# iqbal-lab-org/gramtools

Hardware: AMD Instinct MI355X
Metric: 150bp reads quasimapped/sec (whole node); bit-exact coverage (higher is better)
Workload: dtype u32

## Files before the change

gramtools_amd/csrc/gmx_capi.cpp:

```cpp
#include <atomic>
#include <algorithm>
#include <array>
#include <cmath>
#include <cstdlib>
#include <cstring>
#include <map>
#include <new>
#include <stdexcept>
#include <system_error>
#include <string>
#include <thread>
#include <vector>

#include "gmx_core.h"
#include "gmx_internal.h"

static std::atomic<uint64_t> g_index_serial{1};
struct gmx_index {
  gmx::HostIndex h;
  const uint64_t serial = g_index_serial.fetch_add(1);
};

static thread_local std::string g_error;
void gmx_set_error(const std::string &msg) noexcept {
// ... 250 lines not shown
    ++n;
  }
  return (int64_t)n;
} GMX_GUARD_INT("gmx_index_per_base_layout")

int gmx_index_allele_base_layout(const gmx_index *ix, uint32_t *pb_off, uint32_t *len) try {
  const auto &h = ix->h;
  if (h.is_nested) {
    gmx_set_error("allele_base_non_nested is empty by convention for nested PRGs");
    return GMX_EINVAL;
  }
  for (size_t s = 0; s < h.sites.size(); ++s) {
    const GmxSite &site = h.sites[s];
    const GmxNode &entry = h.nodes[site.entry_node];
    for (uint32_t a = 0; a < site.n_alleles; ++a) {
      uint32_t tgt = h.edges[entry.edge_begin + a];
      uint32_t slot = h.l_allele_off[s] + a;
      if (tgt == site.exit_node) {
        pb_off[slot] = 0;
        len[slot] = 0;
      } else {
        pb_off[slot] = h.l_cov_off[tgt];
        len[slot] = h.nodes[tgt].seq_len;
      }
    }
  }
  return GMX_OK;
} GMX_GUARD_INT("gmx_index_allele_base_layout")

static std::vector<uint32_t> bubble_order(const gmx::HostIndex &h) {
  std::vector<uint32_t> order(h.sites.size());
  for (uint32_t i = 0; i < order.size(); ++i) order[i] = i;
  std::sort(order.begin(), order.end(), [&](uint32_t a, uint32_t b) {
    if (h.site_ref_pos[a] != h.site_ref_pos[b]) return h.site_ref_pos[a] > h.site_ref_pos[b];
    return a > b;
  });
  return order;
}

int gmx_index_bubble_order(const gmx_index *ix, uint32_t *out) try {
  auto o = bubble_order(ix->h);
  for (size_t i = 0; i < o.size(); ++i) out[i] = 5 + 2 * o[i];
  return GMX_OK;
} GMX_GUARD_INT("gmx_index_bubble_order")

int gmx_compute_coverage_depth(const gmx_index *ix, const uint32_t *per_base_raw, const uint32_t *grouped_raw,
                               const uint32_t *glog, uint64_t n_log, gmx_depth_stats *out) try {
  const gmx::HostIndex &h = ix->h;
  std::vector<std::map<int32_t, uint16_t>> hap(h.sites.size());
  std::vector<std::map<std::vector<int32_t>, uint16_t>> logged(h.sites.size());
  for (uint64_t i = 0; i < n_log;) {
    if (glog[i] == 0xFFFFFFFFu) {
      ++i;
      continue;
    }
    if (i + 2 > n_log) break;
    const uint32_t s = glog[i], n = glog[i + 1] & ~GMX_LOG_COUNTED;
    const uint64_t head = (glog[i + 1] & GMX_LOG_COUNTED) ? 4 : 2;
    if (s >= h.sites.size() || i + head + n > n_log) {
      gmx_set_error("corrupt grouped log");
      return GMX_EINVAL;
    }
    const uint64_t count = head == 4 ? ((uint64_t)glog[i + 2] | ((uint64_t)glog[i + 3] << 32)) : 1;
    std::vector<int32_t> ids(glog + i + head, glog + i + head + n);
    logged[s][ids] = (uint16_t)(logged[s][ids] + count);
    i += head + n;
  }
  for (size_t s = 0; s < h.sites.size(); ++s) {
    const GmxSite &site = h.sites[s];
    if (h.l_grouped_off[s] != GMX_GROUPED_LOG) {
      uint32_t nm = (1u << site.n_alleles) - 1u;
      for (uint32_t m = 0; m < nm; ++m) {
        uint32_t tot = grouped_raw[h.l_grouped_off[s] + m];
        if (!tot) continue;
        uint16_t c = (uint16_t)(tot & 0xFFFFu);
        for (uint32_t a = 0; a < site.n_alleles; ++a)
          if (((m + 1) >> a) & 1u) hap[s][(int32_t)a] = (uint16_t)(hap[s][(int32_t)a] + c);
      }
    }
    for (auto &e : logged[s])
      for (auto a : e.first) hap[s][a] = (uint16_t)(hap[s][a] + e.second);
  }
  auto max_hap = [&](size_t s) -> std::pair<int32_t, uint16_t> {
    std::pair<int32_t, uint16_t> best{0, 0};
    bool any = false;
    for (auto &e : hap[s])
      if (!any || e.second > best.second) {
        best = {e.first, e.second};
        any = true;
      }
    return best;
  };
  std::vector<double> coverages;
  double total = 0;
  uint64_t no_cov = 0;
  for (uint32_t s : bubble_order(h)) {
    const GmxSite &site = h.sites[s];
    if (site.parent_site != 0) continue;
    auto mx = max_hap(s);
    uint16_t allele_cov = mx.second;
    double sum = 0;
    uint64_t n_bases = 0;
    uint32_t cur = site.entry_node;
    size_t guard = 0;
    while (cur != site.exit_node) {
      if (++guard > h.nodes.size() + 8) {
        gmx_set_error("coverage graph walk does not terminate");
        return GMX_EINVAL;
      }
      const GmxNode &nd = h.nodes[cur];
      uint32_t ne = h.nodes[cur + 1].edge_begin - nd.edge_begin;
      if (ne > 1 && nd.seq_len == 0) {
        auto m2 = max_hap((nd.site - 5) / 2);
        if (m2.first < 0 || (uint32_t)m2.first >= ne) {
          gmx_set_error("haplogroup out of range");
          return GMX_EINVAL;
        }
        cur = h.edges[nd.edge_begin + (uint32_t)m2.first];
        continue;
      }
      if (nd.seq_len > 0 && nd.cov_off != GMX_NO_COV)
        for (uint32_t i = 0; i < nd.seq_len; ++i) {
          uint32_t v = per_base_raw[h.l_cov_off[cur] + i];
          sum += (double)(v > 65535u ? 65535u : v);
          ++n_bases;
        }
      cur = h.edges[nd.edge_begin];
    }
    double site_cov = n_bases ? sum / (double)n_bases : (double)allele_cov;
    total += site_cov;
    coverages.push_back(site_cov);
    if (allele_cov == 0) no_cov++;
  }
  double mean = total / (double)coverages.size();
  double tv = 0;
  for (double c : coverages) tv += std::pow(c - mean, 2);
  out->mean_cov_depth = mean;
  out->variance_cov_depth = tv / (double)coverages.size();
  out->num_sites_noCov = no_cov;
  out->num_sites_total = coverages.size();
  return GMX_OK;
} GMX_GUARD_INT("gmx_compute_coverage_depth")

int gmx_debug_suffix_array_u16(const uint16_t *text, uint64_t n, uint16_t *out) try {
  try {
    gmx::debug_suffix_array_u16(text, (size_t)n, out);
    return GMX_OK;
  } catch (std::exception const &ex) {
    gmx_set_error(ex.what());
    return GMX_EINVAL;
  }
} GMX_GUARD_INT("gmx_debug_suffix_array_u16")

int gmx_index_copy_sa(const gmx_index *ix, uint32_t *out) try {
  memcpy(out, ix->h.sa.data(), ix->h.sa.size() * 4);
  return GMX_OK;
} GMX_GUARD_INT("gmx_index_copy_sa")
int gmx_index_copy_bwt(const gmx_index *ix, uint32_t *out) try {
  if (ix->h.bwt.empty()) {
    gmx_set_error("this index was built without its introspection tables (GMX_INDEX_INTROSPECTION=1 keeps them)");
    return GMX_EINVAL;
  }
  memcpy(out, ix->h.bwt.data(), ix->h.bwt.size() * 4);
  return GMX_OK;
} GMX_GUARD_INT("gmx_index_copy_bwt")
uint32_t gmx_index_rank(const gmx_index *ix, uint32_t upper, uint32_t base) try {
  if (base < 1 || base > 4) return 0;
  GmxIndexView v = ix->h.view();
  return gmx_rank(v, upper, base);
} GMX_GUARD_ZERO("gmx_index_rank")
int gmx_index_copy_pos_info(const gmx_index *ix, int64_t *out) try {
  const auto &h = ix->h;
  if (h.pos_target.size() != h.prg.size()) {
    gmx_set_error("this index was built without its introspection tables (GMX_INDEX_INTROSPECTION=1 keeps them)");
    return GMX_EINVAL;
  }
  for (size_t p = 0; p < h.prg.size(); ++p) {
    const GmxNode &nd = h.nodes[h.pos_node[p]];
    out[5 * p + 0] = nd.site;
    out[5 * p + 1] = nd.allele;
    out[5 * p + 2] = h.prg[p] <= 4 ? (int64_t)p - nd.first_pos : 0;
    out[5 * p + 3] = h.pos_target[p].first;
    out[5 * p + 4] = h.pos_target[p].second;
  }
  return GMX_OK;
} GMX_GUARD_INT("gmx_index_copy_pos_info")
int64_t gmx_index_copy_target_map(const gmx_index *ix, int64_t *out, uint64_t cap) try {
  std::vector<int64_t> v{(int64_t)ix->h.target_map.size()};
  for (auto &e : ix->h.target_map) {
    v.push_back(e.first);
    v.push_back((int64_t)e.second.size());
    for (auto &t : e.second) {
      v.push_back(t.id);
      v.push_back(t.deletion_allele);
    }
  }
  if (v.size() > cap) return -(int64_t)v.size();
  std::copy(v.begin(), v.end(), out);
  return (int64_t)v.size();
} GMX_GUARD_INT("gmx_index_copy_target_map")
int64_t gmx_index_seed_states(const gmx_index *ix, const uint8_t *kmer, int64_t *out, uint64_t cap) try {
  return gmx_index_seed_states_k(ix, kmer, ix->h.kmer_size, out, cap);
} GMX_GUARD_INT("gmx_index_seed_states")
int64_t gmx_index_seed_states_k(const gmx_index *ix, const uint8_t *kmer, uint32_t len, int64_t *out, uint64_t cap) try {
  const auto &h = ix->h;
  if (len == 0 || (len != h.kmer_size && len != h.kmer_size2)) return GMX_EINVAL;
  uint32_t code = 0;
  for (uint32_t j = 0; j < len; ++j) {
    if (kmer[j] < 1 || kmer[j] > 4) return GMX_EINVAL;
    code |= (uint32_t)(kmer[j] - 1) << (2 * j);
  }
  auto v = gmx::seed_states_of(h, code, len != h.kmer_size);
  if (v.size() > cap) return -(int64_t)v.size();
  std::copy(v.begin(), v.end(), out);
  return (int64_t)v.size();
} GMX_GUARD_INT("gmx_index_seed_states_k")
int64_t gmx_index_jump_states(const gmx_index *ix, uint32_t lo, uint32_t hi, int64_t *out, uint64_t cap) try {
  const auto &h = ix->h;
  GmxIndexView v = h.view();
  ProbeCtx ctx;
  const GmxRankBlock b = v.blocks[lo >> GMX_BLK_SHIFT];
  gmx_marker_pass(v, lo, hi, GMX_NIL, GMX_NIL, b, ctx);
  std::vector<int64_t> r{(int64_t)ctx.n};
  for (uint32_t s = 0; s < ctx.n; ++s) {
    r.push_back(ctx.st[s].lo);
    r.push_back(ctx.st[s].hi);
    std::vector<std::pair<uint32_t, int32_t>> tmp;
    for (uint32_t x = ctx.st[s].tvd; x != GMX_NIL; x = ctx.arena[x].next) tmp.push_back({ctx.arena[x].site, ctx.arena[x].allele});
    r.push_back((int64_t)tmp.size());
    for (size_t i = tmp.size(); i-- > 0;) {
      r.push_back(tmp[i].first);
      r.push_back(tmp[i].second);
    }
    tmp.clear();
    for (uint32_t x = ctx.st[s].tvg; x != GMX_NIL; x = ctx.arena[x].next) tmp.push_back({ctx.arena[x].site, -1});
    r.push_back((int64_t)tmp.size());
    for (size_t i = tmp.size(); i-- > 0;) {
      r.push_back(tmp[i].first);
      r.push_back(-1);
    }
  }
  if (r.size() > cap) return -(int64_t)r.size();
  std::copy(r.begin(), r.end(), out);
  return (int64_t)r.size();
} GMX_GUARD_INT("gmx_index_jump_states")

int gmx_master_seeds(uint32_t master_seed, const uint64_t *reads_per_file, uint64_t n_files, uint32_t *out) try {
  uint32_t mt[624];
  mt[0] = master_seed;
  for (int i = 1; i < 624; ++i) mt[i] = 1812433253u * (mt[i - 1] ^ (mt[i - 1] >> 30)) + (uint32_t)i;
  int idx = 624;
  auto next = [&]() {
    if (idx >= 624) {
      for (int i = 0; i < 624; ++i) {
        uint32_t y = (mt[i] & 0x80000000u) | (mt[(i + 1) % 624] & 0x7fffffffu);
        mt[i] = mt[(i + 397) % 624] ^ (y >> 1) ^ ((y & 1u) ? 0x9908b0dfu : 0u);
      }
      idx = 0;
    }
    uint32_t y = mt[idx++];
    y ^= (y >> 11);
    y ^= (y << 7) & 0x9d2c5680u;
    y ^= (y << 15) & 0xefc60000u;
    y ^= (y >> 18);
    return y;
  };
  uint64_t o = 0;
  for (uint64_t f = 0; f < n_files; ++f)
    for (uint64_t start = 0; start < reads_per_file[f]; start += 5000)
      for (uint64_t i = 0; i < 5000; ++i) {
        uint32_t s = next();
        if (start + i < reads_per_file[f]) out[o++] = s;
      }
  return GMX_OK;
} GMX_GUARD_INT("gmx_master_seeds")

uint64_t gmx_packed_pairs(const uint64_t *offsets, uint32_t uniform_len, uint64_t n_reads) try {
  if (uniform_len) return n_reads * (uint64_t)((uniform_len + 31u) / 32u);
  if (!offsets) return 0;
  return ((offsets[n_reads] >> 5) - (offsets[0] >> 5)) + n_reads;
} GMX_GUARD_ZERO("gmx_packed_pairs")

namespace {
inline void pack8(uint64_t x, uint32_t &lo, uint32_t &hi, uint64_t &bad) {
  const uint64_t y = x - 0x0101010101010101ull;
  bad |= (y & ~x & 0x8080808080808080ull) | (y & 0xFCFCFCFCFCFCFCFCull);
  lo = (uint32_t)(((y & 0x0101010101010101ull) * 0x0102040810204080ull) >> 56);
  hi = (uint32_t)((((y >> 1) & 0x0101010101010101ull) * 0x0102040810204080ull) >> 56);
}
inline bool pack_read(const uint8_t *p, uint32_t len, uint64_t *out) {
  uint64_t bad = 0;
  uint32_t i = 0, pair = 0;
  for (; i + 32 <= len; i += 32, ++pair) {
    uint32_t lo = 0, hi = 0;
    for (int j = 0; j < 4; ++j) {
      uint64_t x;
      memcpy(&x, p + i + 8 * j, 8);
      uint32_t l, h;
      pack8(x, l, h, bad);
      lo |= l << (8 * j);
      hi |= h << (8 * j);
    }
    out[pair] = (uint64_t)lo | ((uint64_t)hi << 32);
  }
  if (i < len) {
    uint32_t lo = 0, hi = 0;
// ... 161 lines not shown
```

gramtools_amd/csrc/gmx_engine_cover_kernels.h:

```cpp
#pragma once
struct CoverAcc {
  uint32_t *acc;
  uint32_t *log;
  uint32_t *log_cursor;
  uint32_t log_cap;
  uint32_t *scratch_big;
  uint32_t n_lanes_big;
  int rng_mode;
  uint32_t max_candidates;
  uint32_t log_sites;
  uint32_t *heap;
  uint64_t heap_words;
  const uint32_t *status;
  uint32_t n_tasks;
  unsigned long long *stats;
  uint32_t rev_off;
  __device__ __forceinline__ uint32_t off_of(uint32_t task) const { return (task & 1u) ? rev_off : 0u; }
};

#define GMX_LOG_PAD 0xFFFFFFFFu
#ifdef GMX_LOOP_STATS
__device__ unsigned long long gmx_cover_stats[6 * 16];
__device__ unsigned long long gmx_coop_stats[6 * 8];
extern "C" int gmx_debug_coop_stats(unsigned long long *out, int reset) {
// ... 825 lines not shown
  if (!done) o.single_rest_list[atomicAdd(&o.counters[GMX_CNT_SINGLE_REST * GMX_CNT_STRIDE], 1u)] = (uint32_t)rec_idx;
}
__global__ void __launch_bounds__(GMX_BLOCK) gmx_cover_single_rest_kernel(GmxIndexView ix, BatchView b, SearchOut o, CoverAcc acc) {
  const uint32_t n = o.counters[GMX_CNT_SINGLE_REST * GMX_CNT_STRIDE];
  for (uint32_t i = blockIdx.x * GMX_BLOCK + threadIdx.x; i < n; i += gridDim.x * GMX_BLOCK)
    gmx_cover_single_rec<false>(ix, o, acc, o.single_rest_list[i], o.cover_general_list, 8u);
}

__global__ void gmx_log_replay_setup_kernel(SearchOut o, const uint32_t *retry_huge_in) {
  uint32_t *c = o.counters;
  const uint32_t n_entries = c[GMX_CNT_LOG_RETRY * GMX_CNT_STRIDE], n_recs = c[GMX_CNT_LOG_RETRY_RECS * GMX_CNT_STRIDE],
                 n_huge = c[GMX_CNT_LOG_RETRY_HUGE * GMX_CNT_STRIDE];
  for (uint32_t i = threadIdx.x; i < n_huge; i += blockDim.x) o.huge_list[i] = retry_huge_in[i];
  __syncthreads();
  if (threadIdx.x == 0) {
    c[4 * GMX_CNT_STRIDE] = n_entries;
    c[GMX_CNT_REPLAY_RECS * GMX_CNT_STRIDE] = n_recs;
    c[11 * GMX_CNT_STRIDE] = n_huge;
    c[15 * GMX_CNT_STRIDE] = 0;
    c[14 * GMX_CNT_STRIDE] = 0;
    c[GMX_CNT_LOG_RETRY * GMX_CNT_STRIDE] = 0;
    c[GMX_CNT_LOG_RETRY_RECS * GMX_CNT_STRIDE] = 0;
    c[GMX_CNT_LOG_RETRY_HUGE * GMX_CNT_STRIDE] = 0;
  }
}
template <bool NESTED>
__global__ void __launch_bounds__(GMX_BLOCK) gmx_cover_single_replay_kernel(GmxIndexView ix, BatchView b, SearchOut o, CoverAcc acc,
                                                                            const uint32_t *recs_in) {
  const uint32_t n = o.counters[GMX_CNT_REPLAY_RECS * GMX_CNT_STRIDE];
  for (uint32_t i = blockIdx.x * GMX_BLOCK + threadIdx.x; i < n; i += gridDim.x * GMX_BLOCK)
    gmx_cover_single_rec<NESTED>(ix, o, acc, recs_in[i], o.cover_overflow_list, 4u);
}

__global__ void gmx_stats_limbs_kernel(unsigned long long *stats, uint32_t *limbs, int recombine) {
  const uint32_t t = threadIdx.x;
  if (!recombine) {
    if (t < 20) limbs[t] = (uint32_t)((stats[t >> 2] >> (16 * (t & 3))) & 0xFFFFull);
    else if (t < 32) limbs[t] = 0;
  } else if (t < 5) {
    unsigned long long v = 0;
    for (int l = 3; l >= 0; --l) v = (v << 16) + limbs[4 * t + l];
    stats[t] = v;
  }
}

#define GMX_PACK_READS 128
#define GMX_PACK_IN_BYTES (24 * 1024)
#define GMX_PACK_OUT_PAIRS (GMX_PACK_IN_BYTES / 32 + GMX_PACK_READS + 8)
typedef uint32_t __attribute__((aligned(1))) gmx_u32_unaligned;
__device__ __forceinline__ void pack4(uint32_t x, uint32_t &lo, uint32_t &hi, uint32_t &bad) {
  uint32_t y = x - 0x01010101u;
  bad |= ((y & ~x & 0x80808080u) | (y & 0xFCFCFCFCu));
  lo = (((y & 0x01010101u) * 0x01020408u) >> 24) & 0xFu;
  hi = ((((y >> 1) & 0x01010101u) * 0x01020408u) >> 24) & 0xFu;
}
__device__ __forceinline__ uint2 pack_tail(const uint8_t *p, uint32_t rem, uint32_t &bad) {
  uint2 out = make_uint2(0, 0);
  for (uint32_t j = 0; j < rem; ++j) {
    uint32_t x = p[j];
    if (x < 1 || x > 4) bad = 1;
    out.x |= ((x - 1u) & 1u) << j;
    out.y |= (((x - 1u) >> 1) & 1u) << j;
  }
  return out;
}
#define GMX_PACK_THREADS (2 * GMX_PACK_READS)
__global__ void __launch_bounds__(GMX_PACK_THREADS) gmx_pack_kernel(BatchView b, uint8_t *skip, uint2 *packed, uint32_t *counters,
                                                                    uint32_t *zero, uint32_t zero_words) {
  __shared__ uint4 in4[GMX_PACK_IN_BYTES / 16 + 2];
  __shared__ uint2 outp[GMX_PACK_OUT_PAIRS];
  if (blockIdx.x == 0)
    for (uint32_t i = threadIdx.x; i < GMX_N_COUNTERS * GMX_CNT_STRIDE; i += GMX_PACK_THREADS) counters[i] = 0;
  for (uint32_t i = blockIdx.x * GMX_PACK_THREADS + threadIdx.x; i < zero_words; i += gridDim.x * GMX_PACK_THREADS) zero[i] = 0;
  const uint32_t r0 = blockIdx.x * GMX_PACK_READS;
  const uint32_t r1 = min(r0 + GMX_PACK_READS, b.n_reads);
  const uint32_t read = r0 + (threadIdx.x >> 1), half = threadIdx.x & 1u;
  const uint64_t s0 = b.offsets[r0], s1 = b.offsets[r1];
  const uintptr_t g0 = reinterpret_cast<uintptr_t>(b.reads + s0);
  const uint32_t shift = (uint32_t)(g0 & 15u);
  const uint64_t span = (s1 - s0) + shift;
  if (span <= GMX_PACK_IN_BYTES) {
    const uint4 *src = reinterpret_cast<const uint4 *>(g0 - shift);
    const uint32_t n16 = (uint32_t)((span + 15) >> 4);
    {
      uint32_t i = threadIdx.x;
      for (; i + 2 * GMX_PACK_THREADS < n16; i += 3 * GMX_PACK_THREADS) {
        const uint4 v0 = src[i], v1 = src[i + GMX_PACK_THREADS], v2 = src[i + 2 * GMX_PACK_THREADS];
        in4[i] = v0;
        in4[i + GMX_PACK_THREADS] = v1;
        in4[i + 2 * GMX_PACK_THREADS] = v2;
      }
      for (; i < n16; i += GMX_PACK_THREADS) in4[i] = src[i];
    }
    const uint64_t po0 = pack_off(b, r0);
    const uint32_t n_out = (uint32_t)(pack_off(b, r1) - po0);
    for (uint32_t i = threadIdx.x; i < n_out; i += GMX_PACK_THREADS) outp[i] = make_uint2(0, 0);
    __syncthreads();
    if (read < r1) {
      const uint64_t s = b.offsets[read];
      const uint32_t len = (uint32_t)(b.offsets[read + 1] - s);
      const uint32_t q = shift + (uint32_t)(s - s0);
      const uint32_t *w = reinterpret_cast<const uint32_t *>(in4);
      const uint8_t *bytes = reinterpret_cast<const uint8_t *>(in4);
      uint2 *out = outp + (uint32_t)(pack_off(b, read) - po0);
      const uint32_t full = len >> 5, first_half = (full + 1u) >> 1;
      const uint32_t c0 = half ? first_half : 0u, c1 = half ? full : first_half;
      uint32_t idx = (q >> 2) + 8u * c0;
      const uint32_t sh = q & 3u;
      uint32_t bad = 0;
      uint32_t carry = w[idx];
      for (uint32_t c = c0; c < c1; ++c) {
        uint2 pair = make_uint2(0, 0);
#pragma unroll
        for (int j = 0; j < 8; ++j) {
          uint32_t nxt = w[++idx], lo, hi;
          pack4(__builtin_amdgcn_alignbyte(nxt, carry, sh), lo, hi, bad);
          pair.x |= lo << (4 * j);
          pair.y |= hi << (4 * j);
          carry = nxt;
        }
        out[c] = pair;
      }
      const uint32_t rem = len & 31u;
      if (half && rem) out[full] = pack_tail(bytes + q + full * 32, rem, bad);
      bad |= (uint32_t)__shfl_xor((int)bad, 1);
      if (!half) skip[read] = bad ? 1 : 0;
    }
    __syncthreads();
    for (uint32_t i = threadIdx.x; i < n_out; i += GMX_PACK_THREADS) packed[po0 + i] = outp[i];
    return;
  }
  if (read >= r1 || half) return;
  uint64_t s = b.offsets[read], e = b.offsets[read + 1];
  uint32_t len = (uint32_t)(e - s);
  const uint8_t *p = b.reads + s;
  uint2 *out = packed + pack_off(b, read);
  uint32_t bad = 0;
  uint32_t full = len >> 5;
  for (uint32_t c = 0; c < full; ++c) {
    uint2 pair = make_uint2(0, 0);
#pragma unroll
    for (int j = 0; j < 8; ++j) {
      uint32_t lo, hi;
      pack4(*reinterpret_cast<const gmx_u32_unaligned *>(p + c * 32 + j * 4), lo, hi, bad);
      pair.x |= lo << (4 * j);
      pair.y |= hi << (4 * j);
    }
    out[c] = pair;
  }
  uint32_t rem = len & 31u;
  if (rem) out[full] = pack_tail(p + full * 32, rem, bad);
  skip[read] = bad ? 1 : 0;
}
```

gramtools_amd/csrc/gmx_engine_debug.h:

```cpp

struct GmxDebugPools {
  GmxFinalState *states = nullptr;
  uint32_t *stack = nullptr;
  GmxPathNode *arena = nullptr;
  uint32_t *result = nullptr;
  uint32_t *in = nullptr;
  uint2 *planes = nullptr;
  uint32_t cap_states = 0, cap_nodes = 0, cap_in = 0, cap_pairs = 0;
};

__global__ void __launch_bounds__(64) gmx_debug_search_kernel(GmxIndexView ix, BatchView b, const uint32_t *in, uint32_t from, uint32_t stop,
                                                              uint32_t mode, uint32_t from_seed_table, BigOut g, uint32_t *result) {
  const bool active = threadIdx.x == 0;
  BigCtx ctx;
  ctx.sp = 0;
  ctx.cap = g.max_states;
  ctx.stack = g.stack;
  ctx.arena = g.arena;
  ctx.arena_n = 0;
  ctx.arena_cap = g.max_path_nodes;
  ctx.status = GMX_TASK_MAPPED;
  ctx.out = g.states;
  ctx.n_out = 0;
  ctx.out_cap = g.max_states;
// ... 17 lines not shown
        const uint32_t lo = p[0], hi = p[1], nt = p[2], ng = p[3];
        p += 4;
        uint32_t tvd = GMX_NIL, tvg = GMX_NIL;
        bool ok = true;
        for (uint32_t j = 0; j < nt; ++j, p += 2)
          if (ok) ok = (tvd = ctx.arena_new(p[0], (int32_t)p[1], tvd)) != GMX_NIL;
        for (uint32_t j = 0; j < ng; ++j, ++p)
          if (ok) ok = (tvg = ctx.arena_new(p[0], -1, tvg)) != GMX_NIL;
        if (!ok || !ctx.push(lo, hi, tvd, tvg, from, mode)) ctx.fail(GMX_TASK_OVERFLOW);
      }
    }
    run = ctx.status == GMX_TASK_MAPPED;
  }
  GmxLane ln;
  dfs_run_wave<2, false>(ix, ctx, r, stop, run, 0, ln);
  if (active) {
    result[0] = ctx.status;
    result[1] = ctx.n_out;
    result[2] = ctx.arena_n;
  }
}

__global__ void gmx_debug_items_kernel(GmxIndexView ix, const GmxFinalState *finals, uint32_t n_final, uint32_t *out, uint32_t cap_items) {
  if (blockIdx.x != 0 || threadIdx.x != 0) return;
  uint32_t n_items = 0, n_nonvar = 0;
  uint32_t *items = out + 2, *nonvar = out + 2 + 6 * (size_t)cap_items;
  const bool ok = gmx_final_items(
      ix, finals, n_final,
      [&](uint32_t lo, uint32_t hi, uint32_t tvd, uint32_t tvg, uint32_t es, int32_t ea) -> bool {
        if (n_items >= cap_items) return false;
        uint32_t *it = items + 6 * (size_t)n_items++;
        it[0] = lo, it[1] = hi, it[2] = tvd, it[3] = tvg, it[4] = es, it[5] = (uint32_t)ea;
        return true;
      },
      [&](uint32_t i, uint32_t) {
        if (n_nonvar < cap_items) nonvar[n_nonvar] = i;
        ++n_nonvar;
      });
  out[0] = ok ? n_items : 0xFFFFFFFFu;
  out[1] = n_nonvar;
}

namespace {

struct DebugWriter {
  uint32_t *out;
  uint64_t cap, n = 0;
  void put(uint32_t w) {
    if (out && n < cap) out[n] = w;
    ++n;
  }
};

int debug_isa(gmx_engine *e) {
  if (!e->debug_isa.empty()) return GMX_OK;
  std::vector<uint32_t> sa(e->dview.n);
  HIP_TRY(hipMemcpy(sa.data(), e->dview.sa, sa.size() * sizeof(uint32_t), hipMemcpyDeviceToHost));
  e->debug_isa.assign(sa.size(), 0u);
  for (size_t i = 0; i < sa.size(); ++i)
    if (sa[i] < sa.size()) e->debug_isa[sa[i]] = (uint32_t)i;
  return GMX_OK;
}

template <class NodeAt>
int debug_put_state(gmx_engine *e, DebugWriter &w, const GmxFinalState &st, NodeAt node) {
  uint32_t lo = st.lo, hi = st.hi;
  if (hi == GMX_TEXT_MARK) {
    if (lo >= e->debug_isa.size()) {
      gmx_set_error("debug states: text-form state outside the PRG");
      return GMX_EREF;
    }
    lo = hi = e->debug_isa[lo];
  }
  std::vector<std::pair<uint32_t, int32_t>> tvd;
  std::vector<uint32_t> tvg;
  for (uint32_t h = st.traversed; h != GMX_NIL;) {
    GmxPathNode nd;
    int rc = node(h, nd);
    if (rc) return rc;
    tvd.emplace_back(nd.site, nd.allele);
    h = nd.next;
    if (tvd.size() > (1u << 20)) {
      gmx_set_error("debug states: path list does not end");
      return GMX_EREF;
    }
  }
  for (uint32_t h = st.traversing; h != GMX_NIL;) {
    if (gmx_h_inline(h)) {
      tvg.push_back(5u + 2u * (h & ~GMX_INLINE_FLAG));
      break;
    }
    GmxPathNode nd;
    int rc = node(h, nd);
    if (rc) return rc;
    tvg.push_back(nd.site);
    h = nd.next;
    if (tvg.size() > (1u << 20)) {
      gmx_set_error("debug states: path list does not end");
      return GMX_EREF;
    }
  }
  w.put(lo);
  w.put(hi);
  w.put((uint32_t)tvd.size());
  w.put((uint32_t)tvg.size());
  for (size_t i = tvd.size(); i-- > 0;) {
    w.put(tvd[i].first);
    w.put((uint32_t)tvd[i].second);
  }
  for (size_t i = tvg.size(); i-- > 0;) w.put(tvg[i]);
  return GMX_OK;
}

int debug_pools(gmx_engine *e, GmxDebugPools &p, uint32_t n_in_words, uint32_t n_pairs) {
  const uint32_t S = std::max<uint32_t>(e->big.max_states, 64u), N = std::max<uint32_t>(e->big.max_path_nodes, 64u);
  int rc;
  if ((rc = e->alloc(&p.states, S, false))) return rc;
  if ((rc = e->alloc(&p.stack, (size_t)S * GMX_STACK_WORDS, false))) return rc;
  if ((rc = e->alloc(&p.arena, N, false))) return rc;
  if ((rc = e->alloc(&p.result, 4, true))) return rc;
  if ((rc = e->alloc(&p.in, std::max<uint32_t>(n_in_words, 1u), false))) return rc;
  if ((rc = e->alloc(&p.planes, n_pairs + 16, true))) return rc;
  p.cap_states = S;
  p.cap_nodes = N;
  return GMX_OK;
}
void debug_pools_free(gmx_engine *e, GmxDebugPools &p) {
  e->release(p.states);
  e->release(p.stack);
  e->release(p.arena);
  e->release(p.result);
  e->release(p.in);
  e->release(p.planes);
}

}

extern "C" {

int gmx_engine_debug_keep_states(gmx_engine *e, int on) try {
  if (!e) {
    gmx_set_error("null engine");
    return GMX_EINVAL;
  }
  e->keep_states = on != 0;
  return GMX_OK;
} GMX_GUARD_INT("gmx_engine_debug_keep_states")

int gmx_debug_final_states(gmx_engine *e, uint64_t task, uint32_t *out, uint64_t cap_words, uint64_t *n_words, int *tier) try {
  if (!e || !n_words) {
    gmx_set_error("gmx_debug_final_states: null argument");
    return GMX_EINVAL;
  }
  if (!e->keep_states || task >= 2 * e->keep_reads) {
    gmx_set_error("gmx_debug_final_states: no such task in the last batch (gmx_engine_debug_keep_states first)");
    return GMX_EINVAL;
  }
  HIP_TRY(hipSetDevice(e->opts.device));
  HIP_TRY(hipDeviceSynchronize());
  int rc = debug_isa(e);
  if (rc) return rc;
  uint32_t raw[GMX_N_COUNTERS * GMX_CNT_STRIDE];
  HIP_TRY(hipMemcpy(raw, e->d_counters, sizeof(raw), hipMemcpyDeviceToHost));
  auto c = [&](int i) { return raw[i * GMX_CNT_STRIDE]; };
  DebugWriter w{out, cap_words};
  {
    const uint32_t n_huge = c(11);
    std::vector<uint32_t> huge(n_huge);
    if (n_huge) HIP_TRY(hipMemcpy(huge.data(), e->d_huge, n_huge * sizeof(uint32_t), hipMemcpyDeviceToHost));
    for (uint32_t t : huge)
      if (t == task) {
        gmx_set_error("gmx_debug_final_states: the task was searched by the last tier, which keeps no states");
        return GMX_ECAP;
      }
  }
  const uint32_t used = (uint32_t)std::min<uint64_t>((uint64_t)c(1) + c(9) + c(29), e->big.max_slots);
  if (used) {
    std::vector<uint32_t> owner(used), nf(used), over(std::min<uint32_t>(c(1), used));
    HIP_TRY(hipMemcpy(owner.data(), e->big.task_of_slot, used * sizeof(uint32_t), hipMemcpyDeviceToHost));
    HIP_TRY(hipMemcpy(nf.data(), e->big.n_final, used * sizeof(uint32_t), hipMemcpyDeviceToHost));
    if (!over.empty()) HIP_TRY(hipMemcpy(over.data(), e->d_overflow, over.size() * sizeof(uint32_t), hipMemcpyDeviceToHost));
    bool in_slots = false;
    for (uint32_t s = used; s-- > 0;) {
      const bool first_q = s < over.size();
      if (first_q && (over[s] & ~GMX_INST_FLAG) != task) continue;
      if (!first_q && owner[s] != task) continue;
      in_slots = true;
      if (first_q && owner[s] != task) continue;
      if (nf[s] == 0) continue;
      const bool inst = first_q && (over[s] & GMX_INST_FLAG) != 0;
      const uint32_t n = nf[s];
      std::vector<GmxFinalState> st(n);
      if (inst) {
        uint32_t first = 0, width = 0;
        HIP_TRY(hipMemcpy(&first, e->d_inst_first + s, 4, hipMemcpyDeviceToHost));
        HIP_TRY(hipMemcpy(&width, e->d_inst_width + s, 4, hipMemcpyDeviceToHost));
        if (n > width * GMX_INST_STATES) continue;
        HIP_TRY(hipMemcpy(st.data(), e->d_inst_states + (size_t)first * GMX_INST_STATES, n * sizeof(GmxFinalState), hipMemcpyDeviceToHost));
        const GmxPathNode *arena = e->d_inst_arena + (size_t)first * GMX_FAST_ARENA;
        w.put(n);
        for (uint32_t i = 0; i < n; ++i) {
          rc = debug_put_state(e, w, st[i], [&](uint32_t h, GmxPathNode &nd) {
            HIP_TRY(hipMemcpy(&nd, arena + h, sizeof(nd), hipMemcpyDeviceToHost));
            return GMX_OK;
          });
          if (rc) return rc;
        }
        if (tier) *tier = 2;
      } else {
        if (n > e->big.max_states) continue;
        HIP_TRY(hipMemcpy(st.data(), e->big.states + (size_t)s * e->big.max_states, n * sizeof(GmxFinalState), hipMemcpyDeviceToHost));
        const GmxPathNode *arena = e->big.arena + (size_t)s * e->big.max_path_nodes;
        w.put(n);
        for (uint32_t i = 0; i < n; ++i) {
          rc = debug_put_state(e, w, st[i], [&](uint32_t h, GmxPathNode &nd) {
            HIP_TRY(hipMemcpy(&nd, arena + h, sizeof(nd), hipMemcpyDeviceToHost));
            return GMX_OK;
          });
          if (rc) return rc;
        }
        if (tier) *tier = 1;
      }
      *n_words = w.n;
      return w.n > cap_words && out ? GMX_ECAP : GMX_OK;
    }
    if (in_slots) {
      w.put(0);
      if (tier) *tier = 1;
      *n_words = w.n;
      return GMX_OK;
    }
  }
  uint32_t packed = 0;
  HIP_TRY(hipMemcpy(&packed, e->d_n_final + task, 4, hipMemcpyDeviceToHost));
  const uint32_t n = std::min<uint32_t>(packed & 0xFFu, GMX_FAST_STATES);
  std::vector<GmxFinalState> st(n);
  if (n) HIP_TRY(hipMemcpy(st.data(), e->d_finals + (size_t)task * GMX_FAST_STATES, n * sizeof(GmxFinalState), hipMemcpyDeviceToHost));
  const GmxPathNode *arena = e->d_arena + task;
  w.put(n);
  for (uint32_t i = 0; i < n; ++i) {
    rc = debug_put_state(e, w, st[i], [&](uint32_t h, GmxPathNode &nd) {
      HIP_TRY(hipMemcpy(&nd, arena + h, sizeof(nd), hipMemcpyDeviceToHost));
      return GMX_OK;
    });
    if (rc) return rc;
  }
  if (tier) *tier = 0;
  *n_words = w.n;
  return w.n > cap_words && out ? GMX_ECAP : GMX_OK;
} GMX_GUARD_INT("gmx_debug_final_states")

int gmx_debug_search(gmx_engine *e, const uint8_t *read, uint32_t read_len, int from_seed_table, const uint32_t *states, uint64_t n_state_words,
                     uint32_t from, uint32_t stop, int lf_only, uint32_t *out, uint64_t cap_words, uint64_t *n_words) try {
  if (!e || !read || !n_words || read_len == 0 || (!from_seed_table && (!states || n_state_words == 0 || from > read_len || stop > from))) {
    gmx_set_error("gmx_debug_search: bad argument");
    return GMX_EINVAL;
  }
  for (uint32_t i = 0; i < read_len; ++i)
    if (read[i] < 1 || read[i] > 4) {
      gmx_set_error("gmx_debug_search: the read must hold bases 1..4");
      return GMX_EINVAL;
    }
  if (from_seed_table && read_len < e->dview.kmer_size) {
    gmx_set_error("gmx_debug_search: read shorter than the k-mer size");
    return GMX_EINVAL;
  }
  HIP_TRY(hipSetDevice(e->opts.device));
  HIP_TRY(hipDeviceSynchronize());
  int rc = debug_isa(e);
  if (rc) return rc;
  const uint32_t n_pairs = (read_len + 31u) / 32u;
  GmxDebugPools p;
  if ((rc = debug_pools(e, p, (uint32_t)n_state_words, n_pairs))) return rc;
  std::vector<uint2> planes(n_pairs + 16, make_uint2(0, 0));
  for (uint32_t i = 0; i < read_len; ++i) {
    const uint32_t code = read[i] - 1u;
    planes[i >> 5].x |= (code & 1u) << (i & 31u);
    planes[i >> 5].y |= (code >> 1) << (i & 31u);
  }
  HIP_TRY(hipMemcpy(p.planes, planes.data(), planes.size() * sizeof(uint2), hipMemcpyHostToDevice));
  if (!from_seed_table) HIP_TRY(hipMemcpy(p.in, states, n_state_words * sizeof(uint32_t), hipMemcpyHostToDevice));
  BatchView b{};
  b.packed = p.planes;
  b.n_reads = 1;
  b.forward_only = 1;
  b.uniform_len = read_len;
  b.pairs_per_read = n_pairs;
  BigOut g{};
  g.states = p.states;
  g.stack = p.stack;
  g.arena = p.arena;
  g.max_states = p.cap_states;
  g.max_path_nodes = p.cap_nodes;
  g.max_slots = 1;
  const size_t big_lds = (size_t)GMX_BIG_LDS_DEPTH * GMX_STACK_WORDS * 64 * sizeof(uint32_t);
  hipLaunchKernelGGL(gmx_debug_search_kernel, dim3(1), dim3(64), big_lds, 0, e->dview, b, p.in, from, stop,
                     lf_only ? GMX_MODE_LF : GMX_MODE_STATE, from_seed_table ? 1u : 0u, g, p.result);
  HIP_TRY(hipGetLastError());
  HIP_TRY(hipDeviceSynchronize());
  uint32_t res[3] = {0, 0, 0};
  HIP_TRY(hipMemcpy(res, p.result, sizeof(res), hipMemcpyDeviceToHost));
  if (res[0] != GMX_TASK_MAPPED) {
    debug_pools_free(e, p);
    gmx_set_error(res[0] == GMX_TASK_OVERFLOW ? "gmx_debug_search: the states exceed the engine's large-capacity pools (gmx_engine_opts.max_states / max_path_nodes)"
                                              : "gmx_debug_search: the search reports a condition on which the reference throws");
    return res[0] == GMX_TASK_OVERFLOW ? GMX_ECAP : GMX_EREF;
  }
  const uint32_t n = res[1];
  std::vector<GmxFinalState> st(n);
  std::vector<GmxPathNode> arena(res[2]);
  if (n) HIP_TRY(hipMemcpy(st.data(), p.states, n * sizeof(GmxFinalState), hipMemcpyDeviceToHost));
  if (res[2]) HIP_TRY(hipMemcpy(arena.data(), p.arena, res[2] * sizeof(GmxPathNode), hipMemcpyDeviceToHost));
  debug_pools_free(e, p);
  DebugWriter w{out, cap_words};
  w.put(n);
  for (uint32_t i = 0; i < n; ++i) {
    rc = debug_put_state(e, w, st[i], [&](uint32_t h, GmxPathNode &nd) {
      if (h >= arena.size()) {
        gmx_set_error("gmx_debug_search: path handle outside the arena");
        return GMX_EREF;
      }
      nd = arena[h];
      return GMX_OK;
    });
    if (rc) return rc;
  }
  *n_words = w.n;
  return w.n > cap_words && out ? GMX_ECAP : GMX_OK;
} GMX_GUARD_INT("gmx_debug_search")

int gmx_debug_encapsulate(gmx_engine *e, const uint32_t *states, uint64_t n_state_words, uint32_t *out, uint64_t cap_words, uint64_t *n_words,
                          uint32_t *nonvariant_sa, uint64_t cap_nonvariant, uint64_t *n_nonvariant) try {
  if (!e || !states || n_state_words == 0 || !n_words || !n_nonvariant) {
    gmx_set_error("gmx_debug_encapsulate: bad argument");
    return GMX_EINVAL;
  }
  HIP_TRY(hipSetDevice(e->opts.device));
  HIP_TRY(hipDeviceSynchronize());
  std::vector<GmxFinalState> st;
  std::vector<GmxPathNode> arena;
  const uint32_t *p = states, *end = states + n_state_words;
  const uint32_t ns = *p++;
  uint64_t positions = 0;
  for (uint32_t s = 0; s < ns; ++s) {
    if (p + 4 > end || p + 4 + 2 * (uint64_t)p[2] + p[3] > end) {
      gmx_set_error("gmx_debug_encapsulate: malformed state words");
      return GMX_EINVAL;
    }
    const uint32_t lo = p[0], hi = p[1], nt = p[2], ng = p[3];
    p += 4;
    if (lo > hi || hi >= e->dview.n) {
      gmx_set_error("gmx_debug_encapsulate: interval outside the suffix array");
      return GMX_EINVAL;
    }
    uint32_t tvd = GMX_NIL, tvg = GMX_NIL;
    for (uint32_t j = 0; j < nt; ++j, p += 2) {
      arena.push_back(GmxPathNode{p[0], (int32_t)p[1], tvd});
      tvd = (uint32_t)arena.size() - 1;
    }
    for (uint32_t j = 0; j < ng; ++j, ++p) {
      arena.push_back(GmxPathNode{p[0], -1, tvg});
      tvg = (uint32_t)arena.size() - 1;
    }
    st.push_back(GmxFinalState{lo, hi, tvd, tvg});
    positions += (uint64_t)hi - lo + 1;
  }
  if (positions > (1u << 24)) {
    gmx_set_error("gmx_debug_encapsulate: more than 2^24 positions");
    return GMX_EINVAL;
  }
  const uint32_t cap_items = (uint32_t)std::max<uint64_t>(positions + ns, 1);
  GmxFinalState *d_st = nullptr;
  uint32_t *d_out = nullptr;
  int rc;
  if ((rc = e->alloc(&d_st, st.size(), false))) return rc;
  if ((rc = e->alloc(&d_out, 2 + 7 * (size_t)cap_items, true))) return rc;
  if (!st.empty()) HIP_TRY(hipMemcpy(d_st, st.data(), st.size() * sizeof(GmxFinalState), hipMemcpyHostToDevice));
  hipLaunchKernelGGL(gmx_debug_items_kernel, dim3(1), dim3(64), 0, 0, e->dview, d_st, (uint32_t)st.size(), d_out, cap_items);
  HIP_TRY(hipGetLastError());
  HIP_TRY(hipDeviceSynchronize());
  std::vector<uint32_t> res(2 + 7 * (size_t)cap_items);
  HIP_TRY(hipMemcpy(res.data(), d_out, res.size() * sizeof(uint32_t), hipMemcpyDeviceToHost));
  e->release(d_st);
  e->release(d_out);
  if (res[0] == 0xFFFFFFFFu || res[1] > cap_items) {
    gmx_set_error("gmx_debug_encapsulate: item buffer exceeded");
    return GMX_EREF;
  }
  DebugWriter w{out, cap_words};
  w.put(res[0]);
  for (uint32_t i = 0; i < res[0]; ++i) {
    const uint32_t *it = res.data() + 2 + 6 * (size_t)i;
    GmxFinalState f{it[0], it[1], it[2], it[3]};
    if (it[4] != 0) {
      w.put(f.lo);
      w.put(f.lo);
      w.put(1);
      w.put(0);
      w.put(it[4]);
      w.put(it[5]);
      continue;
    }
    rc = debug_put_state(e, w, f, [&](uint32_t h, GmxPathNode &nd) {
      if (h >= arena.size()) {
        gmx_set_error("gmx_debug_encapsulate: path handle outside the arena");
        return GMX_EREF;
      }
      nd = arena[h];
      return GMX_OK;
    });
    if (rc) return rc;
  }
  *n_words = w.n;
  *n_nonvariant = res[1];
  for (uint32_t i = 0; i < res[1] && nonvariant_sa && i < cap_nonvariant; ++i) nonvariant_sa[i] = res[2 + 6 * (size_t)cap_items + i];
  return (w.n > cap_words && out) || (nonvariant_sa && res[1] > cap_nonvariant) ? GMX_ECAP : GMX_OK;
} GMX_GUARD_INT("gmx_debug_encapsulate")

}
```

gramtools_amd/csrc/gmx_engine_host.h:

```cpp
#pragma once
#define HIP_TRY(expr)                                                                      \
  do {                                                                                     \
    hipError_t _e = (expr);                                                                \
    if (_e != hipSuccess) {                                                                \
      gmx_set_error(std::string(#expr) + ": " + hipGetErrorString(_e));                    \
      return GMX_EHIP;                                                                     \
    }                                                                                      \
  } while (0)

enum : int { GMX_TK_SEED = 0, GMX_TK_FILTER0, GMX_TK_FILTER1, GMX_TK_SINGLE, GMX_TK_EXTEND2, GMX_TK_UNPACK, GMX_TK_N };
static_assert(GMX_TK_N <= GMX_TIMED_KERNELS, "gmx_timing::kernel_ms holds GMX_TIMED_KERNELS entries");

struct GmxReadLog {
  const uint32_t stride;
  bool on = false;
  uint32_t *d = nullptr;
  uint64_t cap = 0, count = 0;

  uint64_t used() const { return (count * stride + 3) & ~3ull; }

  int reserve(uint64_t n_more) {
    const uint64_t need = (count + n_more) * stride;
    if (need <= cap) return GMX_OK;
    const uint64_t grown = (std::max<uint64_t>(need + need / 2, 1u << 20) + 3) & ~3ull;
    uint32_t *q = nullptr;
    HIP_TRY(hipDeviceSynchronize());
    HIP_TRY(hipMalloc((void **)&q, grown));
    hipError_t err = hipMemset(q, 0, grown);
    if (err == hipSuccess && count) err = hipMemcpy(q, d, used(), hipMemcpyDeviceToDevice);
    if (err != hipSuccess) {
      (void)hipFree(q);
      HIP_TRY(err);
    }
    release();
    d = q;
    cap = grown;
    return GMX_OK;
  }
  int clear(const hipStream_t *stream) {
    if (count) HIP_TRY(stream ? hipMemsetAsync(d, 0, used(), *stream) : hipMemset(d, 0, used()));
    count = 0;
    return GMX_OK;
  }
  uint64_t claim(uint64_t n) {
    const uint64_t base = count;
    count += n;
    return base;
  }
  void release() {
    if (d) (void)hipFree(d);
    d = nullptr;
    cap = 0;
  }
};

struct gmx_engine {
  gmx_engine_opts opts;
  GmxIndexView dview;
  std::vector<void *> allocs;
  uint64_t index_bytes = 0;
  uint32_t *d_fused = nullptr, *d_limbs = nullptr;
  size_t n_fused = 0, n_acc = 0;
  bool record_strands = false;
  uint32_t max_candidates = 0;
  bool recorded = false;
  std::vector<uint32_t> phys_allele, phys_pb, phys_grouped;
  std::vector<uint32_t> hit_fix;
  unsigned long long *d_stats = nullptr;
  uint32_t *d_error = nullptr;
  uint32_t *d_log = nullptr, *d_log_cursor = nullptr;
  uint32_t log_cap = 0;
  uint32_t n_allele = 0, n_pb = 0, n_grouped = 0;
  uint64_t cap_reads = 0;
  uint8_t *d_skip = nullptr;
  uint2 *d_packed = nullptr;
  uint64_t cap_packed = 0;
  uint32_t *d_status = nullptr, *d_n_final = nullptr, *d_mapped = nullptr, *d_overflow = nullptr, *d_counters = nullptr;
  uint32_t *d_general_rest = nullptr;
  uint32_t *d_single_rest = nullptr;
  bool cover_jump = false;
  uint32_t *d_task_lists = nullptr;
  GmxSeed *d_alive_seed = nullptr;
  uint32_t *d_alive = nullptr, *d_dead = nullptr, *d_dead2 = nullptr;
  uint64_t *d_seed_cursor = nullptr;
  bool seed_cursor = false;
  GmxFinalState *d_finals = nullptr;
  GmxPathNode *d_arena = nullptr;
  GmxCoverRec *d_cover_recs = nullptr;
  BigOut big{};
  uint32_t *d_scratch_big = nullptr, *d_cover_overflow = nullptr;
  uint32_t cover_big_lanes = 0;
  uint32_t *d_big_mapped = nullptr, *d_cover_general = nullptr, *d_cover_mid = nullptr, *d_overflow2 = nullptr;
  uint32_t *d_huge = nullptr, *d_cover_huge = nullptr, *d_huge_retry = nullptr;
  uint32_t *d_inst_list = nullptr, *d_inst_sa = nullptr, *d_inst_remaining = nullptr, *d_inst_mapped = nullptr;
  uint32_t inst_cap = 0;
  GmxPathNode *d_inst_arena = nullptr;
  GmxFinalState *d_inst_states = nullptr;
  uint32_t *d_inst_first = nullptr, *d_inst_width = nullptr;
  uint32_t *d_inst_serial = nullptr, *d_general_serial = nullptr, *d_big_serial = nullptr, *d_overflow3 = nullptr;
  bool coop = true;
  uint32_t *d_heap = nullptr;
  uint64_t heap_words = 0;
  bool log_sites = false;
  std::map<std::vector<uint32_t>, std::array<uint64_t, 2>> log_counts;
  uint32_t *h_log_state = nullptr;
  hipEvent_t ev_log_state = nullptr;
  bool log_state_pending = false;
  uint32_t *d_log_retry[2] = {nullptr, nullptr}, *d_log_retry_recs[2] = {nullptr, nullptr}, *d_log_retry_huge[2] = {nullptr, nullptr};
  int log_retry_side = 0;
  BatchView last_b{};
  SearchOut last_o{};
  CoverAcc last_acc{};
  size_t last_big_lds = 0;
  uint64_t log_replays = 0, log_replayed_entries = 0;
  uint64_t log_known = 0;
  uint64_t log_reads_since = 0;
  bool reset_pending = false;
  hipStream_t reset_stream = nullptr;
  hipStream_t side2_stream = nullptr;
  hipEvent_t ev_fork2 = nullptr, ev_side1 = nullptr, ev_filter = nullptr;
  hipStream_t side_stream = nullptr;
  hipEvent_t ev_fork = nullptr, ev_join = nullptr;
  hipEvent_t ev_wait = nullptr;
  struct GmxDeviceIndex *shared_index = nullptr;
  uint32_t filter_lds_words = 0;
  const uint32_t *d_kmer_planar = nullptr;
  const uint32_t *d_absent = nullptr;
  uint32_t n_absent = 0;
  bool use_absent = false;
  uint32_t n_cus = 256;
  uint32_t probe_iters = GMX_PROBE_ITERS;
  uint32_t extend_cap = 0;
  uint32_t extend_budget = 8;
  bool seeds_in_place = false;
  gmx_engine *twin = nullptr;
  gmx_engine *owner = nullptr;
  bool is_twin = false, twin_off = false;
  GmxReadLog outcomes{1}, positions{16};
  uint64_t reset_epoch = 0;
  hipStream_t main_stream = nullptr;
  uint32_t twin_toggle = 0;
  hipEvent_t ev_zeroed = nullptr, ev_twin_done = nullptr;
  uint64_t zero_epoch = 0, seen_zero_epoch = 0;
  bool twin_in_flight = false;
  bool last_on_twin = false;
  uint32_t extend_passes = 1;
  uint32_t extend_budget2[GMX_EXTRA_PASSES] = {24, 96, 0};
  GmxParked *d_park2 = nullptr;
  uint32_t *d_park2_n = nullptr;
  bool keep_states = false;
  uint64_t keep_reads = 0;
  std::vector<uint32_t> debug_isa;
  uint32_t fuse = 1;
  uint8_t *d_reads = nullptr;
  uint64_t *d_offsets = nullptr;
  uint32_t *d_seeds = nullptr;
  uint64_t cap_bases = 0, cap_stage_reads = 0;
  struct StageSlot {
    uint8_t *d_reads = nullptr;
    uint64_t *d_offsets = nullptr, *h_offsets = nullptr;
    uint32_t *d_seeds = nullptr, *h_seeds = nullptr;
    uint64_t cap_bases = 0, cap_reads = 0;
    hipEvent_t copied = nullptr, done = nullptr;
    bool busy = false;
  } stage[2];
  hipStream_t copy_stream = nullptr;
  hipStream_t copy_stream2 = nullptr;
  uint32_t copy_toggle = 0;
  hipStream_t last_stream = nullptr;
  struct PackSlot {
    uint2 *d_planes = nullptr;
    uint64_t *d_offsets = nullptr;
    uint32_t *d_seeds = nullptr;
    uint8_t *d_skip = nullptr;
    uint64_t cap_pairs = 0, cap_reads = 0;
    hipEvent_t copied = nullptr, done = nullptr;
    bool busy = false;
  } pslot[3];
  uint32_t pslot_next = 0;
  void release(void *q) {
    if (!q) return;
    for (size_t i = 0; i < allocs.size(); ++i)
      if (allocs[i] == q) {
        allocs[i] = allocs.back();
        allocs.pop_back();
        (void)hipFree(q);
        return;
      }
  }
  bool timing = false;
  struct EvTriple { hipEvent_t s, a, b, c; uint64_t reads; hipEvent_t k[GMX_TIMED_KERNELS][2]; uint32_t timed; };
  std::vector<EvTriple> pending;
  double search_ms = 0, cover_ms = 0;
  uint64_t search_launches = 0, cover_launches = 0, timed_reads = 0;
  double kernel_ms[GMX_TIMED_KERNELS] = {0};
  uint64_t kernel_launches[GMX_TIMED_KERNELS] = {0};

  template <class T>
  int alloc(T **p, size_t count, bool zero) {
    void *q = nullptr;
    size_t bytes = std::max<size_t>(count, 1) * sizeof(T);
    allocs.reserve(allocs.size() + 1);
    HIP_TRY(hipMalloc(&q, bytes));
    if (zero) HIP_TRY(hipMemset(q, 0, bytes));
    allocs.push_back(q);
    *p = (T *)q;
    return GMX_OK;
  }
  template <class T, class A>
  int upload(const T **dst, const std::vector<T, A> &src) {
    T *q = nullptr;
    int rc = alloc(&q, src.size(), false);
    if (rc) return rc;
    if (!src.empty()) HIP_TRY(hipMemcpy(q, src.data(), src.size() * sizeof(T), hipMemcpyHostToDevice));
    index_bytes += src.size() * sizeof(T);
    *dst = q;
    return GMX_OK;
  }
  int upload(const uint32_t **dst, const gmx::WordBuf &src) {
    uint32_t *q = nullptr;
    int rc = alloc(&q, src.size(), false);
    if (rc) return rc;
    const size_t piece = (size_t)1 << 28;
    for (size_t at = 0; at < src.size(); at += piece)
      HIP_TRY(hipMemcpy(q + at, src.data() + at, std::min(piece, src.size() - at) * sizeof(uint32_t), hipMemcpyHostToDevice));
    index_bytes += src.size() * sizeof(uint32_t);
    *dst = q;
    return GMX_OK;
  }
};

static hipError_t gmx_event_wait(hipEvent_t ev) {
  static const bool spin = getenv("GMX_WAIT_SPIN") != nullptr;
  if (spin) return hipEventSynchronize(ev);
  const auto t0 = std::chrono::steady_clock::now();
  for (bool napping = false;;) {
    const hipError_t q = hipEventQuery(ev);
    if (q != hipErrorNotReady) return q;
    (void)hipGetLastError();
    if (!napping) {
      napping = std::chrono::steady_clock::now() - t0 > std::chrono::microseconds(60);
      continue;
    }
    struct timespec ts = {0, 50 * 1000};
    nanosleep(&ts, nullptr);
  }
}

static int gmx_quiesce(gmx_engine *e) {
  if (!e->ev_wait) HIP_TRY(hipEventCreateWithFlags(&e->ev_wait, hipEventDisableTiming | hipEventBlockingSync));
  hipStream_t streams[5] = {e->last_stream, e->copy_stream, e->side_stream, e->side2_stream, e->copy_stream2};
  for (int i = 0; i < 5; ++i) {
    if (i > 0 && !streams[i]) continue;
    bool seen = false;
    for (int j = 0; j < i; ++j) seen = seen || streams[j] == streams[i];
    if (seen) continue;
    HIP_TRY(hipEventRecord(e->ev_wait, streams[i]));
    HIP_TRY(gmx_event_wait(e->ev_wait));
  }
  return GMX_OK;
}

static int note_zeroed(gmx_engine *e, hipStream_t stream) {
  if (!e->twin) return GMX_OK;
  if (!e->ev_zeroed) HIP_TRY(hipEventCreateWithFlags(&e->ev_zeroed, hipEventDisableTiming));
  HIP_TRY(hipEventRecord(e->ev_zeroed, stream));
  ++e->zero_epoch;
  return GMX_OK;
}
static int twin_join(gmx_engine *e, hipStream_t stream) {
  gmx_engine *tw = e->twin;
  if (!tw || !e->twin_in_flight) return GMX_OK;
  if (!e->ev_twin_done) HIP_TRY(hipEventCreateWithFlags(&e->ev_twin_done, hipEventDisableTiming));
  HIP_TRY(hipEventRecord(e->ev_twin_done, tw->main_stream));
  HIP_TRY(hipStreamWaitEvent(stream, e->ev_twin_done, 0));
  return GMX_OK;
}
static int flush_reset(gmx_engine *e) {
  if (!e->reset_pending) return GMX_OK;
  e->reset_pending = false;
  HIP_TRY(hipMemsetAsync(e->d_fused, 0, (e->n_fused + 32) * 4, e->reset_stream));
  return note_zeroed(e, e->reset_stream);
}

static int log_settle(gmx_engine *e);
static int gmx_log_drain(gmx_engine *e, uint64_t keep_below) {
  int frc = flush_reset(e);
  if (frc) return frc;
  HIP_TRY(hipDeviceSynchronize());
  uint32_t used = 0;
  HIP_TRY(hipMemcpy(&used, e->d_log_cursor, 4, hipMemcpyDeviceToHost));
  used = std::min(used, e->log_cap);
  e->log_reads_since = 0;
  e->log_known = used;
  if (used <= keep_below) return GMX_OK;
  std::vector<uint32_t> w(used);
  HIP_TRY(hipMemcpy(w.data(), e->d_log, (size_t)used * 4, hipMemcpyDeviceToHost));
  std::vector<uint32_t> key;
  for (size_t i = 0; i < w.size();) {
    if (w[i] == GMX_LOG_PAD) {
      ++i;
      continue;
    }
    const size_t n_ids = i + 2 > w.size() ? 0 : (size_t)(w[i + 1] & ~GMX_LOG_REVERSE);
    if (i + 2 > w.size() || i + 2 + n_ids > w.size()) {
      gmx_set_error("grouped-allele-count log: malformed record at word " + std::to_string(i) + " of " + std::to_string(w.size()));
      return GMX_EREF;
    }
    if ((w[i + 1] & GMX_LOG_REVERSE) && !(e->owner ? e->owner : e)->record_strands) {
      gmx_set_error("grouped-allele-count log: a reverse-complement record at word " + std::to_string(i) + " of an engine that does not record per strand");
      return GMX_EREF;
    }
    key.assign(1, w[i]);
    key.insert(key.end(), w.begin() + i + 2, w.begin() + i + 2 + n_ids);
    e->log_counts[key][(w[i + 1] & GMX_LOG_REVERSE) ? 1 : 0] += 1;
    i += 2 + n_ids;
  }
  HIP_TRY(hipMemset(e->d_log_cursor, 0, 4));
  e->log_known = 0;
  return GMX_OK;
}

template <class Env, int LIST>
static void launch_cover_lds(gmx_engine *e, hipStream_t stream, const BatchView &b, const SearchOut &o, const CoverAcc &acc,
                             bool after_coop = false) {
  static const uint32_t lanes_env = getenv("GMX_COVER_LANES") ? (uint32_t)atoi(getenv("GMX_COVER_LANES")) : 0u;
  const uint32_t lanes = lanes_env ? std::min(lanes_env, gmx_cover_lds_lanes<Env>()) : gmx_cover_lds_lanes<Env>();
  const size_t lds = (size_t)GmxScratchFixed<Env>::total * lanes * sizeof(uint32_t);
  const uint32_t per_cu = std::min<uint32_t>((uint32_t)(160 * 1024 / lds), 32u);
  hipLaunchKernelGGL((gmx_cover_kernel<Env, LIST>), dim3(e->n_cus * per_cu), dim3(64), lds, stream, e->dview, b, o, e->big,
                     acc, lanes, after_coop ? 1u : 0u);
}

template <int LIST>
static void launch_cover_coop(gmx_engine *e, hipStream_t stream, const BatchView &b, const SearchOut &o, const CoverAcc &acc) {
  const size_t lds = (size_t)gmx_coop_lds_words<LIST>() * sizeof(uint32_t);
  const uint32_t per_cu = std::min<uint32_t>((uint32_t)(160 * 1024 / lds), 16u);
  hipLaunchKernelGGL((gmx_cover_coop_kernel<LIST>), dim3(e->n_cus * per_cu), dim3(64), lds, stream, e->dview, b, o, e->big, acc);
}

extern "C" {

void gmx_engine_default_opts(gmx_engine_opts *o) try {
  o->device = 0;
  o->rng_mode = GMX_RNG_LEMIRE;
  o->max_states = 1024;
  o->max_path_nodes = 2048;
  o->max_batch_reads = 4u << 20;
  o->forward_only = 0;
  o->huge_heap_bytes = 512ull << 20;
  o->log_cap_words = 0;
} GMX_GUARD_VOID("gmx_engine_default_opts")

static int ensure_batch_capacity(gmx_engine *e, uint64_t n_reads, bool launching = false) {
  if (launching) {
    gmx_engine *own = e->owner ? e->owner : e;
    for (GmxReadLog *log : {&own->outcomes, &own->positions})
      if (log->on) {
        const int lrc = log->reserve(n_reads);
        if (lrc) return lrc;
      }
  }
  if (n_reads <= e->cap_reads) return GMX_OK;
  uint64_t cap = std::max<uint64_t>(e->cap_reads ? n_reads + n_reads / 8 : n_reads, 1024);
  uint64_t n_tasks = cap * 2;
  int rc;
  if ((rc = e->alloc(&e->d_skip, cap, true))) return rc;
  if ((rc = e->alloc(&e->d_status, n_tasks, false))) return rc;
  if ((rc = e->alloc(&e->d_n_final, n_tasks, false))) return rc;
  if ((rc = e->alloc(&e->d_cover_recs, n_tasks * GMX_REGIONS, false))) return rc;
  if ((rc = e->alloc(&e->d_mapped, n_tasks * GMX_REGIONS, false))) return rc;
  if ((rc = e->alloc(&e->d_task_lists, (size_t)GMX_TL_N * n_tasks, false))) return rc;
  e->d_overflow = e->d_task_lists + (size_t)GMX_TL_OVERFLOW * n_tasks;
  e->d_overflow2 = e->d_task_lists + (size_t)GMX_TL_OVERFLOW2 * n_tasks;
  e->d_alive = e->d_task_lists + (size_t)GMX_TL_ALIVE * n_tasks;
  e->d_dead = e->d_task_lists + (size_t)GMX_TL_DEAD * n_tasks;
  e->d_dead2 = e->d_task_lists + (size_t)GMX_TL_DEAD2 * n_tasks;
  e->d_cover_general = e->d_task_lists + (size_t)GMX_TL_GENERAL * n_tasks;
  if ((rc = e->alloc(&e->d_cover_overflow, n_tasks, false))) return rc;
  if ((rc = e->alloc(&e->d_general_rest, n_tasks, false))) return rc;
  if ((rc = e->alloc(&e->d_single_rest, n_tasks, false))) return rc;
  if ((rc = e->alloc(&e->d_park2, (size_t)n_tasks * GMX_STACK_DEPTH, false))) return rc;
  if ((rc = e->alloc(&e->d_park2_n, n_tasks, false))) return rc;
  if (e->log_sites)
    for (int side = 0; side < 2; ++side) {
      if ((rc = e->alloc(&e->d_log_retry[side], n_tasks, false))) return rc;
      if ((rc = e->alloc(&e->d_log_retry_recs[side], n_tasks, false))) return rc;
      if ((rc = e->alloc(&e->d_log_retry_huge[side], n_tasks, false))) return rc;
    }
  if ((rc = e->alloc(&e->d_cover_mid, n_tasks, false))) return rc;
  if ((rc = e->alloc(&e->d_seed_cursor, n_tasks, false))) return rc;
  if ((rc = e->alloc(&e->d_finals, n_tasks * GMX_FAST_STATES, false))) return rc;
  if ((rc = e->alloc(&e->d_arena, n_tasks * GMX_FAST_ARENA, false))) return rc;
  if ((rc = e->alloc(&e->d_alive_seed, n_tasks, false))) return rc;
  if ((rc = e->alloc(&e->d_huge, n_tasks, false))) return rc;
  if ((rc = e->alloc(&e->d_cover_huge, n_tasks, false))) return rc;
  if ((rc = e->alloc(&e->d_huge_retry, 2 * n_tasks, false))) return rc;
  e->big.max_slots = (uint32_t)std::min<uint64_t>(n_tasks, std::min<uint64_t>(std::max<uint64_t>(n_tasks / 16, 4096), 262144));
  if ((rc = e->alloc(&e->big.states, (size_t)e->big.max_slots * e->big.max_states, false))) return rc;
  if ((rc = e->alloc(&e->big.stack, (size_t)e->big.max_slots * e->big.max_states * GMX_STACK_WORDS, false))) return rc;
  if ((rc = e->alloc(&e->big.arena, (size_t)e->big.max_slots * e->big.max_path_nodes, false))) return rc;
  if ((rc = e->alloc(&e->big.n_final, e->big.max_slots, false))) return rc;
  if ((rc = e->alloc(&e->big.task_of_slot, e->big.max_slots, false))) return rc;
  if ((rc = e->alloc(&e->d_big_mapped, e->big.max_slots, false))) return rc;
  e->inst_cap = (uint32_t)std::min<uint64_t>(n_tasks, 1u << 23);
  if ((rc = e->alloc(&e->d_inst_list, e->inst_cap, false))) return rc;
  if ((rc = e->alloc(&e->d_inst_sa, e->inst_cap, false))) return rc;
  if ((rc = e->alloc(&e->d_inst_remaining, e->big.max_slots, false))) return rc;
  if ((rc = e->alloc(&e->d_inst_mapped, e->big.max_slots, false))) return rc;
  if ((rc = e->alloc(&e->d_inst_first, e->big.max_slots, false))) return rc;
  if ((rc = e->alloc(&e->d_inst_width, e->big.max_slots, false))) return rc;
  if ((rc = e->alloc(&e->d_inst_serial, e->big.max_slots, false))) return rc;
  if ((rc = e->alloc(&e->d_general_serial, n_tasks, false))) return rc;
  if ((rc = e->alloc(&e->d_big_serial, e->big.max_slots, false))) return rc;
  if ((rc = e->alloc(&e->d_overflow3, 2 * n_tasks, false))) return rc;
  if ((rc = e->alloc(&e->d_inst_arena, (size_t)e->inst_cap * GMX_FAST_ARENA, false))) return rc;
  if ((rc = e->alloc(&e->d_inst_states, (size_t)e->inst_cap * GMX_INST_STATES, false))) return rc;
  e->cap_reads = cap;
  return GMX_OK;
}

struct GmxDeviceIndex {
  uint64_t serial = 0;
  int device = 0;
  GmxIndexView view{};
  std::vector<void *> allocs;
  uint64_t bytes = 0;
  int refs = 0;
};
static std::mutex g_dev_index_mu;
static std::vector<GmxDeviceIndex *> g_dev_indexes;
static void gmx_dev_index_release(GmxDeviceIndex *d) {
  if (!d) return;
  std::lock_guard<std::mutex> lk(g_dev_index_mu);
  if (--d->refs > 0) return;
  for (void *p : d->allocs) (void)hipFree(p);
  g_dev_indexes.erase(std::remove(g_dev_indexes.begin(), g_dev_indexes.end(), d), g_dev_indexes.end());
  delete d;
}

static int engine_create(const gmx_index *ixh, const gmx_engine_opts *opts_in, gmx_engine *primary, gmx_engine **out);
static int set_record_strands(gmx_engine *e, bool on);
int gmx_engine_create(const gmx_index *ixh, const gmx_engine_opts *opts_in, gmx_engine **out) try {
  int rc = engine_create(ixh, opts_in, nullptr, out);
  if (rc) return rc;
  gmx_engine *e = *out;
  if (const char *ro = getenv("GMX_RECORD_OUTCOMES")) e->outcomes.on = atoi(ro) != 0;
  if (const char *rp = getenv("GMX_RECORD_POSITIONS")) e->positions.on = atoi(rp) != 0;
  const gmx::HostIndex &h = gmx_index_host(ixh);
  const bool can = !e->log_sites && e->shared_index && !getenv("GMX_NO_INDEX_SHARE");
  bool want = can && (h.is_nested || e->index_bytes >= (2ull << 30));
  if (const char *tw = getenv("GMX_TWIN")) want = can && atoi(tw) != 0;
  if (want) {
    gmx_engine *t = nullptr;
    if (engine_create(ixh, &e->opts, e, &t) == GMX_OK) {
      e->twin = t;
      t->owner = e;
    } else {
      (void)hipGetLastError();
    }
  }
  if (const char *rs = getenv("GMX_RECORD_STRANDS"))
    if (atoi(rs) != 0 && (rc = set_record_strands(e, true))) {
      gmx_engine_destroy(e);
      *out = nullptr;
      return rc;
    }
  if (const char *mc = getenv("GMX_MAX_CANDIDATES")) e->max_candidates = (uint32_t)strtoul(mc, nullptr, 10);
  return GMX_OK;
} GMX_GUARD_INT("gmx_engine_create")

static int engine_create(const gmx_index *ixh, const gmx_engine_opts *opts_in, gmx_engine *primary, gmx_engine **out) {
  if (!ixh || !out) {
    gmx_set_error("gmx_engine_create: null argument");
    return GMX_EINVAL;
  }
  gmx_engine_opts opts;
  if (opts_in)
    opts = *opts_in;
  else
    gmx_engine_default_opts(&opts);
  if (opts.max_states == 0) opts.max_states = 1024;
  if (opts.max_path_nodes == 0) opts.max_path_nodes = 2048;
  if (opts.max_batch_reads == 0) opts.max_batch_reads = 4u << 20;
  if (opts.huge_heap_bytes == 0) opts.huge_heap_bytes = 512ull << 20;
  if (const char *hb = getenv("GMX_HUGE_HEAP_BYTES")) opts.huge_heap_bytes = strtoull(hb, nullptr, 10);
  opts.huge_heap_bytes = std::max<uint64_t>(opts.huge_heap_bytes, 64 * 1024);
  int ndev = 0;
  if (hipGetDeviceCount(&ndev) != hipSuccess || ndev <= 0) {
    gmx_set_error("no HIP device available: the quasimap engine has no CPU fallback");
    return GMX_ENODEV;
  }
  if (opts.device < 0 || opts.device >= ndev) {
    gmx_set_error("device ordinal out of range");
    return GMX_ENODEV;
  }
  HIP_TRY(hipSetDevice(opts.device));
  const gmx::HostIndex &h = gmx_index_host(ixh);
  if (h.kmer_size == 0) {
    gmx_set_error("the index was built without a k-mer seed table (kmer_size = 0)");
    return GMX_EINVAL;
  }
  gmx_engine *e = new gmx_engine();
  e->opts = opts;
  GmxIndexView v = h.view();
  int rc = 0;
  {
// ... 100 lines not shown
      e->n_cus = (uint32_t)prop.multiProcessorCount;
    const size_t words = h.kmer_bitmap.size();
    if (!getenv("GMX_FORCE_ABSENT_FILTER") && words >= 4 && words % 4 == 0 && words * 4 <= 128 * 1024 &&
        hipFuncSetAttribute(reinterpret_cast<const void *>(gmx_filter_lds_kernel), hipFuncAttributeMaxDynamicSharedMemorySize,
                            (int)(words * 4)) == hipSuccess)
      e->filter_lds_words = (uint32_t)words;
    (void)hipGetLastError();
    if (primary) {
      e->filter_lds_words = primary->filter_lds_words;
      e->d_kmer_planar = primary->d_kmer_planar;
      e->d_absent = primary->d_absent;
      e->n_absent = primary->n_absent;
      e->use_absent = primary->use_absent;
    } else if (e->filter_lds_words) {
      const uint32_t k = h.kmer_size;
      std::vector<uint32_t> planar(words, 0);
      for (uint64_t code = 0; code < (1ull << (2 * k)); ++code) {
        if (!((h.kmer_bitmap[code >> 5] >> (code & 31)) & 1u)) continue;
        uint32_t lo = 0, hi = 0;
        for (uint32_t j = 0; j < k; ++j) {
          const uint32_t base = (uint32_t)(code >> (2 * j)) & 3u;
          lo |= (base & 1u) << j;
          hi |= (base >> 1) << j;
        }
        const uint32_t p = (hi << k) | lo;
        planar[p >> 5] |= 1u << (p & 31);
      }
      rc |= e->upload(&e->d_kmer_planar, planar);
    } else if (!getenv("GMX_NO_ABSENT_FILTER")) {
      const uint64_t n_k = 1ull << (2 * h.kmer_size);
      if (n_k - std::min<uint64_t>(n_k, h.n_seed_kmers_present) <= GMX_ABSENT_MAX) {
        std::vector<uint32_t> absent;
        for (size_t w = 0; w < words && absent.size() <= GMX_ABSENT_MAX; ++w) {
          uint32_t zeros = ~h.kmer_bitmap[w];
          while (zeros) {
            const uint64_t code = (uint64_t)w * 32 + (uint32_t)__builtin_ctz(zeros);
            zeros &= zeros - 1;
            if (code < n_k) absent.push_back((uint32_t)code);
          }
        }
        if (absent.size() <= GMX_ABSENT_MAX) {
          e->n_absent = (uint32_t)absent.size();
          e->use_absent = true;
          if (absent.empty()) absent.push_back(0);
          rc |= e->upload(&e->d_absent, absent);
        }
      }
    }
  }
  if (const char *pi = getenv("GMX_PROBE_ITERS")) e->probe_iters = (uint32_t)std::max(0, atoi(pi));
  if (getenv("GMX_NO_FUSE")) e->fuse = 0;
  if (const char *eb = getenv("GMX_EXTEND_BUDGET")) e->extend_budget = (uint32_t)std::max(0, atoi(eb));
  e->extend_cap = 0u;
  if (const char *ec = getenv("GMX_EXTEND_CAP")) e->extend_cap = (uint32_t)std::max(0, atoi(ec));
  e->extend_passes = 1u;
  e->extend_budget2[0] = 24;
  e->extend_budget2[1] = 96;
  if (const char *ep = getenv("GMX_EXTEND_PASSES")) {
    e->extend_passes = 1;
    for (const char *q = ep; *q && e->extend_passes < GMX_EXTRA_PASSES;) {
      e->extend_budget2[e->extend_passes - 1] = (uint32_t)std::max(1l, strtol(q, const_cast<char **>(&q), 10));
      ++e->extend_passes;
      if (*q == ',') ++q; else break;
    }
  }
  if (getenv("GMX_NO_COOP")) e->coop = false;
  e->seed_cursor = h.n_seed_states_large * 10 > h.n_seed_states;
  if (const char *sc = getenv("GMX_SEED_CURSOR")) e->seed_cursor = atoi(sc) != 0;
  if (primary) {
    e->seed_cursor = primary->seed_cursor;
    e->dview.sa_ctx = primary->dview.sa_ctx;
    e->dview.seed_side = primary->dview.seed_side;
  }
  if (!primary && e->seed_cursor && !rc && !getenv("GMX_NO_SA_CTX")) {
    uint32_t *sc = nullptr;
    if (e->alloc(&sc, h.sa.size(), false) == GMX_OK) {
      hipLaunchKernelGGL(gmx_sa_ctx_kernel, dim3(8192), dim3(256), 0, nullptr, e->dview.sa, e->dview.text, (uint64_t)h.sa.size(), sc);
      if (hipDeviceSynchronize() == hipSuccess) {
        e->dview.sa_ctx = sc;
        e->index_bytes += h.sa.size() * sizeof(uint32_t);
      }
    } else {
      (void)hipGetLastError();
    }
  }
  if (!primary && e->seed_cursor && !rc && !getenv("GMX_NO_SEED_SIDE") && h.seed_words.size() > 1) {
    uint32_t *side = nullptr;
    const size_t n_side = h.seed_words.size() / 4 + 2;
    if (e->alloc(&side, n_side, false) == GMX_OK) {
      hipLaunchKernelGGL(gmx_seed_side_kernel, dim3(8192), dim3(256), 0, nullptr, e->dview.seeds, (uint64_t)h.seeds.size(), e->dview.seed_words,
                         e->dview.seed_shift, side);
      if (h.kmer_size2)
        hipLaunchKernelGGL(gmx_seed_side_kernel, dim3(8192), dim3(256), 0, nullptr, e->dview.seeds2, (uint64_t)h.seeds2.size(), e->dview.seed_words,
                           e->dview.seed_shift, side);
      if (hipDeviceSynchronize() == hipSuccess) {
        e->dview.seed_side = side;
        e->index_bytes += n_side * sizeof(uint32_t);
      }
    } else {
      (void)hipGetLastError();
    }
  }
  auto make_stream = [&](hipStream_t *st) -> bool {
    int least = 0, greatest = 0;
    bool want_prio = h.is_nested;
    if (const char *tp = getenv("GMX_TWIN_PRIORITY")) want_prio = atoi(tp) != 0;
    const bool prio = primary && want_prio && hipDeviceGetStreamPriorityRange(&least, &greatest) == hipSuccess && least != greatest;
    (void)hipGetLastError();
    return (prio ? hipStreamCreateWithPriority(st, hipStreamNonBlocking, greatest) : hipStreamCreateWithFlags(st, hipStreamNonBlocking)) == hipSuccess;
  };
  rc |= !make_stream(&e->side_stream);
  rc |= !make_stream(&e->side2_stream);
  rc |= hipEventCreateWithFlags(&e->ev_fork2, hipEventDisableTiming) != hipSuccess;
  rc |= hipEventCreateWithFlags(&e->ev_side1, hipEventDisableTiming) != hipSuccess;
  rc |= hipEventCreateWithFlags(&e->ev_filter, hipEventDisableTiming) != hipSuccess;
  rc |= hipEventCreateWithFlags(&e->ev_fork, hipEventDisableTiming) != hipSuccess;
  rc |= hipEventCreateWithFlags(&e->ev_join, hipEventDisableTiming) != hipSuccess;
  e->cover_big_lanes = 64 * 32;
  rc |= e->alloc(&e->d_scratch_big, (size_t)GmxScratchFixed<CoverEnvBig>::total * e->cover_big_lanes, false);
  if (primary) {
    e->is_twin = true;
    rc |= !make_stream(&e->main_stream);
    e->last_stream = e->main_stream;
  }
  if (rc) {
    gmx_engine_destroy(e);
    return GMX_EHIP;
  }
  *out = e;
  return GMX_OK;
}

void gmx_engine_destroy(gmx_engine *e) try {
  if (!e) return;
  (void)hipSetDevice(e->opts.device);
  (void)hipDeviceSynchronize();
  if (e->twin) gmx_engine_destroy(e->twin);
  e->twin = nullptr;
  if (e->main_stream) (void)hipStreamDestroy(e->main_stream);
  if (e->ev_zeroed) (void)hipEventDestroy(e->ev_zeroed);
  if (e->ev_twin_done) (void)hipEventDestroy(e->ev_twin_done);
  if (e->side_stream) (void)hipStreamDestroy(e->side_stream);
  if (e->side2_stream) (void)hipStreamDestroy(e->side2_stream);
  if (e->ev_fork2) (void)hipEventDestroy(e->ev_fork2);
  if (e->ev_side1) (void)hipEventDestroy(e->ev_side1);
  if (e->ev_filter) (void)hipEventDestroy(e->ev_filter);
  if (e->ev_fork) (void)hipEventDestroy(e->ev_fork);
  if (e->ev_join) (void)hipEventDestroy(e->ev_join);
  if (e->ev_wait) (void)hipEventDestroy(e->ev_wait);
  if (e->copy_stream) (void)hipStreamDestroy(e->copy_stream);
  if (e->copy_stream2) (void)hipStreamDestroy(e->copy_stream2);
  if (e->h_log_state) (void)hipHostFree(e->h_log_state);
  if (e->ev_log_state) (void)hipEventDestroy(e->ev_log_state);
  for (auto &sl : e->pslot) {
    if (sl.copied) (void)hipEventDestroy(sl.copied);
    if (sl.done) (void)hipEventDestroy(sl.done);
  }
  for (auto &sl : e->stage) {
    if (sl.copied) (void)hipEventDestroy(sl.copied);
    if (sl.done) (void)hipEventDestroy(sl.done);
    if (sl.h_offsets) (void)hipHostFree(sl.h_offsets);
    if (sl.h_seeds) (void)hipHostFree(sl.h_seeds);
  }
  for (void *p : e->allocs) (void)hipFree(p);
  e->outcomes.release();
  e->positions.release();
  gmx_dev_index_release(e->shared_index);
  delete e;
} GMX_GUARD_VOID("gmx_engine_destroy")

int gmx_engine_reset(gmx_engine *e) try {
  HIP_TRY(hipSetDevice(e->opts.device));
  e->reset_pending = false;
  HIP_TRY(hipDeviceSynchronize());
  HIP_TRY(hipMemset(e->d_fused, 0, (e->n_fused + 32) * 4));
  HIP_TRY(hipMemset(e->d_error, 0, 8));
  HIP_TRY(hipMemset(e->d_counters, 0, GMX_N_COUNTERS * GMX_CNT_STRIDE * 4));
  if (e->twin) {
    HIP_TRY(hipMemset(e->twin->d_error, 0, 8));
    HIP_TRY(hipMemset(e->twin->d_counters, 0, GMX_N_COUNTERS * GMX_CNT_STRIDE * 4));
    e->twin_in_flight = false;
  }
  int lrc = e->outcomes.clear(nullptr);
  if (lrc || (lrc = e->positions.clear(nullptr))) return lrc;
  ++e->reset_epoch;
  e->log_counts.clear();
  e->log_known = e->log_reads_since = 0;
  e->log_state_pending = false;
  e->recorded = false;
  return GMX_OK;
} GMX_GUARD_INT("gmx_engine_reset")

int gmx_engine_reset_async(gmx_engine *e, void *hip_stream) try {
  HIP_TRY(hipSetDevice(e->opts.device));
  hipStream_t st = (hipStream_t)hip_stream;
  int frc = flush_reset(e);
  if (frc) return frc;
  if ((frc = twin_join(e, st))) return frc;
  e->twin_in_flight = false;
  if ((frc = e->outcomes.clear(&st)) || (frc = e->positions.clear(&st))) return frc;
  ++e->reset_epoch;
  e->reset_pending = true;
  e->reset_stream = st;
  e->log_counts.clear();
  e->log_known = e->log_reads_since = 0;
  e->log_state_pending = false;
  e->recorded = false;
  return GMX_OK;
} GMX_GUARD_INT("gmx_engine_reset_async")

static bool gmx_ab_no_filter() {
  static const bool off = getenv("GMX_AB_NO_FILTER") != nullptr;
  return off;
}
static void launch_filter(gmx_engine *e, hipStream_t st, dim3 task_grid, const BatchView &b, const SearchOut &o, int pass,
                          hipEvent_t t0 = nullptr, hipEvent_t t1 = nullptr) {
  if (gmx_ab_no_filter()) return;
  if (e->filter_lds_words)
    hipExtLaunchKernelGGL(gmx_filter_lds_kernel, dim3(e->n_cus), dim3(GMX_FILTER_LDS_THREADS), e->filter_lds_words * 4,
                          st, t0, t1, 0u, e->dview, b, o, e->d_kmer_planar, e->filter_lds_words, pass);
  else if (e->use_absent)
    hipExtLaunchKernelGGL(gmx_filter_absent_kernel, task_grid, dim3(GMX_BLOCK), 0, st, t0, t1, 0u, e->dview, b, o, e->d_absent, e->n_absent, pass);
  else
    hipExtLaunchKernelGGL(gmx_filter_kernel, task_grid, dim3(GMX_BLOCK), 0, st, t0, t1, 0u, e->dview, b, o, pass);
}

static int log_state_enqueue(gmx_engine *e, hipStream_t stream) {
  if (!e->h_log_state) {
    HIP_TRY(hipHostMalloc(reinterpret_cast<void **>(&e->h_log_state), 4 * sizeof(uint32_t), hipHostMallocDefault));
    HIP_TRY(hipEventCreateWithFlags(&e->ev_log_state, hipEventDisableTiming));
  }
  HIP_TRY(hipMemcpyAsync(e->h_log_state + 0, e->d_log_cursor, 4, hipMemcpyDeviceToHost, stream));
  HIP_TRY(hipMemcpyAsync(e->h_log_state + 1, e->d_counters + GMX_CNT_LOG_RETRY * GMX_CNT_STRIDE, 4, hipMemcpyDeviceToHost, stream));
  HIP_TRY(hipMemcpyAsync(e->h_log_state + 2, e->d_counters + GMX_CNT_LOG_RETRY_RECS * GMX_CNT_STRIDE, 4, hipMemcpyDeviceToHost, stream));
  HIP_TRY(hipMemcpyAsync(e->h_log_state + 3, e->d_counters + GMX_CNT_LOG_RETRY_HUGE * GMX_CNT_STRIDE, 4, hipMemcpyDeviceToHost, stream));
  HIP_TRY(hipEventRecord(e->ev_log_state, stream));
  e->log_state_pending = true;
  return GMX_OK;
}

static int launch_log_replay(gmx_engine *e, hipStream_t stream) {
  const int in = e->log_retry_side, out = in ^ 1;
  SearchOut o = e->last_o;
  o.log_retry_list = e->d_log_retry[out];
  o.log_retry_recs = e->d_log_retry_recs[out];
  o.log_retry_huge = e->d_log_retry_huge[out];
  o.cover_overflow_list = e->d_log_retry[in];
  hipLaunchKernelGGL(gmx_log_replay_setup_kernel, dim3(1), dim3(1024), 0, stream, o, e->d_log_retry_huge[in]);
  if (e->dview.is_nested)
    hipLaunchKernelGGL(gmx_cover_single_replay_kernel<true>, dim3(e->n_cus * 4), dim3(GMX_BLOCK), 0, stream, e->dview, e->last_b, o, e->last_acc,
                     e->d_log_retry_recs[in]);
  else
    hipLaunchKernelGGL(gmx_cover_single_replay_kernel<false>, dim3(e->n_cus * 4), dim3(GMX_BLOCK), 0, stream, e->dview, e->last_b, o, e->last_acc,
                     e->d_log_retry_recs[in]);
  hipLaunchKernelGGL((gmx_cover_kernel<CoverEnvBig, 1>), dim3(e->cover_big_lanes / 64), dim3(64), e->last_big_lds, stream, e->dview,
                     e->last_b, o, e->big, e->last_acc, 64u, 0u);
  HIP_TRY(hipGetLastError());
  e->log_retry_side = out;
  e->last_o.log_retry_list = o.log_retry_list;
  e->last_o.log_retry_recs = o.log_retry_recs;
  e->last_o.log_retry_huge = o.log_retry_huge;
  return log_state_enqueue(e, stream);
}

static int log_settle(gmx_engine *e) {
  if (!e->log_state_pending) return GMX_OK;
  uint64_t before = ~0ull;
  for (int round = 0;; ++round) {
    HIP_TRY(hipEventSynchronize(e->ev_log_state));
    e->log_state_pending = false;
    const uint32_t used = std::min(e->h_log_state[0], e->log_cap);
    const uint64_t retries = (uint64_t)e->h_log_state[1] + e->h_log_state[2] + e->h_log_state[3];
    if (retries == 0) {
      if (used > e->log_cap / 2) return gmx_log_drain(e, 0);
      e->log_known = used;
      return GMX_OK;
    }
    if (round > 0 && retries >= before) {
      HIP_TRY(hipDeviceSynchronize());
      const uint32_t err[2] = {GMX_TASK_LOGFULL, 0};
      HIP_TRY(hipMemcpy(e->d_error, err, 8, hipMemcpyHostToDevice));
      return GMX_OK;
    }
    before = retries;
    int rc = gmx_log_drain(e, 0);
    if (rc) return rc;
    e->log_replays++;
    e->log_replayed_entries += retries;
    if ((rc = launch_log_replay(e, e->last_stream))) return rc;
  }
}

struct BatchInput {
  const uint8_t *d_reads = nullptr;
  const uint64_t *d_offsets = nullptr;
  const uint32_t *d_seeds = nullptr;
  const uint2 *d_planes = nullptr;
  const uint8_t *d_skip = nullptr;
  const uint32_t *d_twobit = nullptr;
  uint32_t twobit_base0 = 0;
  uint32_t uniform_len = 0;
  uint64_t n_reads = 0, total_bases = 0;
};

__global__ void gmx_batch_begin_kernel(uint32_t *counters, uint32_t *zero, uint32_t zero_words) {
  if (blockIdx.x == 0)
    for (uint32_t i = threadIdx.x; i < GMX_N_COUNTERS * GMX_CNT_STRIDE; i += blockDim.x) counters[i] = 0;
  for (uint32_t i = blockIdx.x * blockDim.x + threadIdx.x; i < zero_words; i += gridDim.x * blockDim.x) zero[i] = 0;
}

__device__ __forceinline__ uint32_t gmx_even_bits(unsigned long long x) {
  x &= 0x5555555555555555ull;
  x = (x | (x >> 1)) & 0x3333333333333333ull;
  x = (x | (x >> 2)) & 0x0F0F0F0F0F0F0F0Full;
  x = (x | (x >> 4)) & 0x00FF00FF00FF00FFull;
  x = (x | (x >> 8)) & 0x0000FFFF0000FFFFull;
  x = (x | (x >> 16)) & 0x00000000FFFFFFFFull;
  return (uint32_t)x;
}
__global__ void __launch_bounds__(256) gmx_unpack2_kernel(BatchView b, const uint32_t *stream, uint32_t base0, uint2 *packed) {
  const uint32_t ppr_uniform = b.pairs_per_read;
  for (uint64_t t = blockIdx.x * (uint64_t)blockDim.x + threadIdx.x;; t += (uint64_t)gridDim.x * blockDim.x) {
    uint32_t read, pair;
    uint64_t first_base;
    uint32_t len;
    if (b.uniform_len) {
      read = (uint32_t)(t / ppr_uniform);
      if (read >= b.n_reads) break;
      pair = (uint32_t)(t - (uint64_t)read * ppr_uniform);
      first_base = (uint64_t)read * b.uniform_len;
      len = b.uniform_len;
    } else {
      read = (uint32_t)t;
      if (read >= b.n_reads) break;
      pair = 0;
      first_base = b.offsets[read] - b.offsets[0];
      len = (uint32_t)(b.offsets[read + 1] - b.offsets[read]);
    }
    uint2 *out = packed + pack_off(b, read);
    const uint32_t n_pairs = b.uniform_len ? pair + 1 : (len + 31u) / 32u;
    for (uint32_t p = pair; p < n_pairs; ++p) {
      const uint64_t j = base0 + first_base + 32ull * p;
      const uint64_t w = j >> 4;
      const uint32_t sh = (uint32_t)(j & 15u) * 2u;
      const uint32_t w0 = stream[w], w1 = stream[w + 1], w2 = stream[w + 2];
      const unsigned long long bits = (unsigned long long)__builtin_amdgcn_alignbit(w1, w0, sh) |
                                      ((unsigned long long)__builtin_amdgcn_alignbit(w2, w1, sh) << 32);
      out[p] = make_uint2(gmx_even_bits(bits), gmx_even_bits(bits >> 1));
    }
  }
}

static int launch_batch(gmx_engine *e, const BatchInput &in, hipStream_t stream) {
  const uint64_t n_reads = in.n_reads, total_bases = in.total_bases;
  if (n_reads == 0) return GMX_OK;
  if (n_reads > (0x7fffffffull / GMX_FAST_ARENA) / 2) {
    gmx_set_error("batch too large: at most 44 M reads per launch (lower gmx_engine_opts.max_batch_reads)");
    return GMX_EINVAL;
  }
  int rc = e->log_sites ? log_settle(e) : GMX_OK;
  if (rc) return rc;
  if ((rc = ensure_batch_capacity(e, n_reads, true))) return rc;
  const bool fold_reset = e->reset_pending && e->reset_stream == stream;
  if (e->reset_pending && !fold_reset && (rc = flush_reset(e))) return rc;
  e->reset_pending = false;
  if (!in.d_planes) {
    uint64_t need = total_bases / 32 + n_reads + 16;
    if (need > e->cap_packed) {
      rc = e->alloc(&e->d_packed, need, false);
      if (rc) return rc;
      e->cap_packed = need;
    }
  }
  BatchView b{in.d_reads, in.d_offsets, in.d_seeds, (in.d_planes || in.d_twobit) ? in.d_skip : e->d_skip, in.d_planes ? in.d_planes : e->d_packed,
              (uint32_t)n_reads, (uint32_t)(e->opts.forward_only ? 1 : 0), in.uniform_len, (in.uniform_len + 31u) / 32u,
              e->keep_states ? 1u : 0u};
  const uint32_t region_inv = (uint32_t)std::min<uint64_t>(0xFFFFFFFFull, (((uint64_t)GMX_REGIONS << 32) + e->dview.n_prg - 1) / std::max<uint32_t>(e->dview.n_prg, 1u));
  SearchOut o{};
  o.status = e->d_status;
  o.n_final = e->d_n_final;
  o.finals = e->d_finals;
  o.arena = e->d_arena;
  o.cover_recs = e->d_cover_recs;
  o.cover_rec_task = e->d_mapped;
  o.region_cap = (uint32_t)(e->cap_reads * 2);
  o.region_inv = region_inv;
  o.task_lists = e->d_task_lists;
  o.list_stride = (uint32_t)(e->cap_reads * 2);
  o.overflow_list = e->d_overflow;
  o.overflow2_list = e->d_overflow2;
  o.cover_overflow_list = e->d_cover_overflow;
  o.big_mapped_list = e->d_big_mapped;
  o.cover_mid_list = e->d_cover_mid;
  o.cover_general_list = e->d_cover_general;
  o.alive_list = e->d_alive;
  o.dead_list = e->d_dead;
  o.dead2_list = e->d_dead2;
  o.seed_cursor = e->d_seed_cursor;
  o.error = e->d_error;
  o.counters = e->d_counters;
  o.alive_seed = e->d_alive_seed;
  o.huge_list = e->d_huge;
  o.cover_huge_list = e->d_cover_huge;
  o.huge_retry = e->d_huge_retry;
  o.arena_stride = (uint32_t)(e->cap_reads * 2);
  o.inst_list = e->d_inst_list;
  o.inst_sa = e->d_inst_sa;
  o.inst_remaining = e->d_inst_remaining;
  o.inst_cap = e->inst_cap;
  o.inst_slots = !getenv("GMX_NO_INST") ? e->big.max_slots : 0u;
  o.slot_n_final = e->big.n_final;
  o.slot_task = e->big.task_of_slot;
  o.inst_mapped_list = e->d_inst_mapped;
  o.inst_arena = e->d_inst_arena;
  o.inst_states = e->d_inst_states;
  o.inst_first = e->d_inst_first;
  o.inst_remaining_width = e->d_inst_width;
  o.inst_serial_list = e->d_inst_serial;
  o.general_serial_list = e->d_general_serial;
  o.big_serial_list = e->d_big_serial;
  o.overflow3_list = e->d_overflow3;
  o.split_twice = getenv("GMX_NO_SPLIT2") ? 0u : 1u;
  o.general_rest_list = e->d_general_rest;
  o.single_rest_list = e->d_single_rest;
  o.park2 = e->d_park2;
  o.park2_n = e->d_park2_n;
  o.log_retry_list = e->d_log_retry[e->log_retry_side];
  o.log_retry_recs = e->d_log_retry_recs[e->log_retry_side];
  o.log_retry_huge = e->d_log_retry_huge[e->log_retry_side];
  o.stats = e->d_stats;
  {
    gmx_engine *own = e->owner ? e->owner : e;
    own->recorded = true;
    if (own->outcomes.on) {
      o.outcomes = own->outcomes.d;
      o.outcome_base = own->outcomes.claim(n_reads);
    }
    if (own->positions.on) {
      o.positions = reinterpret_cast<uint2 *>(own->positions.d);
      o.position_base = own->positions.claim(n_reads);
    }
  }
  uint32_t n_tasks = (uint32_t)n_reads * 2;
  if (e->keep_states) {
    HIP_TRY(hipMemsetAsync(e->d_n_final, 0, (size_t)n_tasks * sizeof(uint32_t), stream));
    e->keep_reads = n_reads;
  }
  gmx_engine::EvTriple ev{};
  if (e->timing) {
    HIP_TRY(hipEventCreate(&ev.s));
    HIP_TRY(hipEventCreate(&ev.a));
    HIP_TRY(hipEventCreate(&ev.b));
    HIP_TRY(hipEventCreate(&ev.c));
    for (int k = 0; k < GMX_TK_N; ++k) {
      HIP_TRY(hipEventCreate(&ev.k[k][0]));
      HIP_TRY(hipEventCreate(&ev.k[k][1]));
    }
    ev.reads = n_reads;
    HIP_TRY(hipEventRecord(ev.s, stream));
  }
  auto t_ev = [&](int k, int side) -> hipEvent_t {
    if (!e->timing) return nullptr;
    ev.timed |= 1u << k;
    return ev.k[k][side];
  };
  if (in.d_planes || in.d_twobit) {
    hipLaunchKernelGGL(gmx_batch_begin_kernel, dim3(fold_reset ? 256 : 1), dim3(1024), 0, stream, e->d_counters,
                       fold_reset ? e->d_fused : nullptr, fold_reset ? (uint32_t)(e->n_fused + 32) : 0u);
    if (in.d_twobit) {
      const uint64_t threads = in.uniform_len ? n_reads * ((in.uniform_len + 31u) / 32u) : n_reads;
      hipExtLaunchKernelGGL(gmx_unpack2_kernel, dim3((unsigned)std::min<uint64_t>((threads + 255) / 256, 1u << 20)), dim3(256), 0, stream,
                            t_ev(GMX_TK_UNPACK, 0), t_ev(GMX_TK_UNPACK, 1), 0u, b, in.d_twobit, in.twobit_base0, e->d_packed);
    }
  } else
    hipLaunchKernelGGL(gmx_pack_kernel, dim3((unsigned)((n_reads + GMX_PACK_READS - 1) / GMX_PACK_READS)), dim3(GMX_PACK_THREADS), 0, stream, b,
                       e->d_skip, e->d_packed, e->d_counters, fold_reset ? e->d_fused : nullptr, fold_reset ? (uint32_t)(e->n_fused + 32) : 0u);
  if (fold_reset && (rc = note_zeroed(e, stream))) return rc;
  size_t lds = (size_t)GMX_STACK_DEPTH * GMX_STACK_WORDS * GMX_BLOCK * sizeof(uint32_t);
  const size_t big_lds = (size_t)GMX_BIG_LDS_DEPTH * GMX_STACK_WORDS * 64 * sizeof(uint32_t);
  dim3 task_grid((n_tasks + GMX_BLOCK - 1) / GMX_BLOCK);
  const bool seeded = e->dview.kmer_size2 != 0 && !getenv("GMX_NO_SEEDED");
  if (seeded)
    hipExtLaunchKernelGGL(gmx_seed_kernel, dim3((n_tasks + GMX_SEED_THREADS * GMX_SEED_CHUNKS - 1) / (GMX_SEED_THREADS * GMX_SEED_CHUNKS)), dim3(GMX_SEED_THREADS), 0, stream,
                          t_ev(GMX_TK_SEED, 0), t_ev(GMX_TK_SEED, 1), 0u, e->dview, b, o);
  else if (e->seed_cursor)
    hipExtLaunchKernelGGL(gmx_probe_kernel<true>, task_grid, dim3(GMX_BLOCK), (uint32_t)lds, stream, t_ev(GMX_TK_SEED, 0), t_ev(GMX_TK_SEED, 1), 0u, e->dview, b, o,
                          e->probe_iters);
  else
    hipExtLaunchKernelGGL(gmx_probe_kernel<false>, task_grid, dim3(GMX_BLOCK), (uint32_t)lds, stream, t_ev(GMX_TK_SEED, 0), t_ev(GMX_TK_SEED, 1), 0u, e->dview, b, o,
                          e->probe_iters);
  HIP_TRY(hipEventRecord(e->ev_fork, stream));
  HIP_TRY(hipStreamWaitEvent(e->side_stream, e->ev_fork, 0));
  CoverAcc acc{e->d_fused, e->d_log, e->d_log_cursor, e->log_cap, e->d_scratch_big, e->cover_big_lanes, e->opts.rng_mode,
               (e->owner ? e->owner : e)->max_candidates, e->log_sites ? 1u : 0u, e->d_heap, e->heap_words, e->d_status, (uint32_t)n_reads * 2u, e->d_stats,
               (e->owner ? e->owner : e)->record_strands ? (uint32_t)e->n_acc : 0u};
  if (seeded) {
    HIP_TRY(hipStreamWaitEvent(e->side2_stream, e->ev_fork, 0));
    const InstPools pools{0};
    hipLaunchKernelGGL(gmx_extend_inst_kernel, dim3(e->n_cus * 2), dim3(GMX_BLOCK), lds, e->side2_stream, e->dview, b, o, pools);
    if (e->coop) launch_cover_coop<5>(e, e->side2_stream, b, o, acc);
    launch_cover_lds<CoverEnvMid, 5>(e, e->side2_stream, b, o, acc, e->coop);
    hipLaunchKernelGGL(gmx_search_split_kernel, dim3(4096), dim3(64), big_lds, e->side2_stream, e->dview, b, o, e->big, 0);
    launch_cover_lds<CoverEnvMid, 4>(e, e->side2_stream, b, o, acc);
  } else {
    hipLaunchKernelGGL(gmx_search_big_kernel, dim3(1024), dim3(64), big_lds, e->side_stream, e->dview, b, o, e->big, 0);
  }
  HIP_TRY(hipEventRecord(e->ev_side1, e->side_stream));
  if (!gmx_ab_no_filter()) launch_filter(e, e->side_stream, task_grid, b, o, 0, t_ev(GMX_TK_FILTER0, 0), t_ev(GMX_TK_FILTER0, 1));
  hipEvent_t k0 = e->timing ? ev.a : nullptr, k1 = e->timing ? ev.b : nullptr;
  const uint32_t budget = e->extend_budget;
  if (seeded && e->seed_cursor)
    hipExtLaunchKernelGGL((gmx_extend_kernel<true, 1>), task_grid, dim3(GMX_BLOCK), (uint32_t)lds, stream, k0, k1, 0u, e->dview, b, o, e->fuse, budget, 0u);
  else if (seeded)
    hipExtLaunchKernelGGL((gmx_extend_kernel<false, 1>), task_grid, dim3(GMX_BLOCK), (uint32_t)lds, stream, k0, k1, 0u, e->dview, b, o, e->fuse, budget, 0u);
  else if (e->seed_cursor)
    hipExtLaunchKernelGGL((gmx_extend_kernel<true, 0>), task_grid, dim3(GMX_BLOCK), (uint32_t)lds, stream, k0, k1, 0u, e->dview, b, o, e->fuse, budget, 0u);
  else
    hipExtLaunchKernelGGL((gmx_extend_kernel<false, 0>), task_grid, dim3(GMX_BLOCK), (uint32_t)lds, stream, k0, k1, 0u, e->dview, b, o, e->fuse, budget, 0u);
  if (budget) {
    for (uint32_t pass = 0; pass < e->extend_passes; ++pass) {
      const bool last = pass + 1 >= e->extend_passes;
      const uint32_t budget2 = last ? e->extend_cap : e->extend_budget2[pass];
      const uint32_t pass_arg = pass | (last && e->extend_cap ? 0x80000000u : 0u);
      hipEvent_t p0 = pass == 0 ? t_ev(GMX_TK_EXTEND2, 0) : nullptr, p1 = pass == 0 ? t_ev(GMX_TK_EXTEND2, 1) : nullptr;
      if (e->seed_cursor)
        hipExtLaunchKernelGGL((gmx_extend_kernel<true, 2>), task_grid, dim3(GMX_BLOCK), (uint32_t)lds, stream, p0, p1, 0u, e->dview, b, o, e->fuse, budget2, pass_arg);
      else
        hipExtLaunchKernelGGL((gmx_extend_kernel<false, 2>), task_grid, dim3(GMX_BLOCK), (uint32_t)lds, stream, p0, p1, 0u, e->dview, b, o, e->fuse, budget2, pass_arg);
    }
  }
  HIP_TRY(hipEventRecord(e->ev_fork2, stream));
  HIP_TRY(hipStreamWaitEvent(e->side2_stream, e->ev_fork2, 0));
  HIP_TRY(hipStreamWaitEvent(e->side2_stream, e->ev_side1, 0));
  if (!gmx_ab_no_filter()) launch_filter(e, e->side2_stream, task_grid, b, o, 1, t_ev(GMX_TK_FILTER1, 0), t_ev(GMX_TK_FILTER1, 1));
  static const bool split2 = getenv("GMX_NO_SPLIT2") == nullptr;
  if (split2) hipLaunchKernelGGL(gmx_search_split_kernel, dim3(1024), dim3(64), big_lds, e->side2_stream, e->dview, b, o, e->big, 1);
  hipLaunchKernelGGL(gmx_search_big_kernel, dim3(1024), dim3(64), big_lds, e->side2_stream, e->dview, b, o, e->big, split2 ? 2 : 1);
  if (e->coop) launch_cover_coop<2>(e, e->side2_stream, b, o, acc);
  launch_cover_lds<CoverEnvMid, 2>(e, e->side2_stream, b, o, acc, e->coop);
  const bool general_on_side = !e->dview.is_nested;
  HIP_TRY(hipStreamWaitEvent(e->side_stream, e->ev_fork2, 0));
  const size_t one_lds = (size_t)4 * GMX_WIDE_LOCI * GMX_ONE_THREADS * sizeof(uint32_t);
  const bool one = !getenv("GMX_NO_COVER_ONE");
  auto launch_one = [&](hipStream_t st) {
    hipLaunchKernelGGL(gmx_cover_one_kernel, dim3(e->n_cus * 4), dim3(GMX_ONE_THREADS), one_lds, st, e->dview, b, o, e->big, acc, one ? 1u : 0u);
  };
  if (general_on_side) {
    launch_one(e->side_stream);
    if (e->coop) launch_cover_coop<3>(e, e->side_stream, b, o, acc);
    launch_cover_lds<CoverEnvLds, 3>(e, e->side_stream, b, o, acc, e->coop);
    launch_cover_lds<CoverEnv, 0>(e, e->side_stream, b, o, acc);
  }
  HIP_TRY(hipEventRecord(e->ev_filter, e->side_stream));
  if (e->dview.is_nested) {
    hipExtLaunchKernelGGL(gmx_cover_single_kernel<true>, dim3(task_grid.x * GMX_REGIONS), dim3(GMX_BLOCK), 0, stream, t_ev(GMX_TK_SINGLE, 0), t_ev(GMX_TK_SINGLE, 1), 0u,
                          e->dview, b, o, acc);
  } else if (e->cover_jump) {
    hipExtLaunchKernelGGL(gmx_cover_jump_kernel, dim3(task_grid.x * GMX_REGIONS), dim3(GMX_BLOCK), (uint32_t)(GMX_STAGE_MAX * GMX_BLOCK * sizeof(uint32_t)), stream,
                          t_ev(GMX_TK_SINGLE, 0), t_ev(GMX_TK_SINGLE, 1), 0u, e->dview, b, o, acc);
    hipLaunchKernelGGL(gmx_cover_single_rest_kernel, dim3(e->n_cus * 2), dim3(GMX_BLOCK), 0, stream, e->dview, b, o, acc);
  } else {
    hipExtLaunchKernelGGL(gmx_cover_single_kernel<false>, dim3(task_grid.x * GMX_REGIONS), dim3(GMX_BLOCK), 0, stream, t_ev(GMX_TK_SINGLE, 0), t_ev(GMX_TK_SINGLE, 1), 0u,
                          e->dview, b, o, acc);
  }
  hipStream_t last = general_on_side ? e->side2_stream : stream;
  if (!general_on_side) {
    launch_one(stream);
    if (e->coop) launch_cover_coop<3>(e, stream, b, o, acc);
    launch_cover_lds<CoverEnvLds, 3>(e, stream, b, o, acc, e->coop);
    launch_cover_lds<CoverEnv, 0>(e, stream, b, o, acc);
    HIP_TRY(hipEventRecord(e->ev_join, e->side2_stream));
    HIP_TRY(hipStreamWaitEvent(stream, e->ev_join, 0));
  }
  HIP_TRY(hipStreamWaitEvent(last, e->ev_filter, 0));
  hipLaunchKernelGGL((gmx_cover_kernel<CoverEnvBig, 1>), dim3(e->cover_big_lanes / 64), dim3(64), big_lds, last, e->dview,
                     b, o, e->big, acc, 64u, 0u);
  if (general_on_side) {
    HIP_TRY(hipEventRecord(e->ev_join, e->side2_stream));
    HIP_TRY(hipStreamWaitEvent(stream, e->ev_join, 0));
  }
  if (e->timing) {
    HIP_TRY(hipEventRecord(ev.c, stream));
    e->pending.push_back(ev);
  }
  HIP_TRY(hipGetLastError());
  e->last_stream = stream;
  if (e->log_sites) {
    e->last_b = b;
    e->last_o = o;
    e->last_acc = acc;
    e->last_big_lds = big_lds;
    if ((rc = log_state_enqueue(e, stream))) return rc;
  }
  return GMX_OK;
}

int gmx_map_reads_device(gmx_engine *e, const uint8_t *d_reads, const uint64_t *d_offsets, const uint32_t *d_seeds,
                         uint64_t n_reads, uint64_t total_bases, void *hip_stream) try {
  if (!e) {
    gmx_set_error("null engine");
    return GMX_EINVAL;
  }
  HIP_TRY(hipSetDevice(e->opts.device));
  hipStream_t stream = (hipStream_t)hip_stream;
  uint64_t done = 0;
  while (done < n_reads) {
    uint64_t n = std::min<uint64_t>(e->opts.max_batch_reads, n_reads - done);
    BatchInput in;
    in.d_reads = d_reads;
    in.d_offsets = d_offsets + done;
    in.d_seeds = d_seeds + done;
    in.n_reads = n;
    in.total_bases = total_bases;
    int rc = launch_batch(e, in, stream);
    if (rc) return rc;
    done += n;
  }
  if (e->log_sites) return log_settle(e);
  return GMX_OK;
} GMX_GUARD_INT("gmx_map_reads_device")

static bool gmx_is_pinned(const void *p) {
  hipPointerAttribute_t at;
  if (hipPointerGetAttributes(&at, p) != hipSuccess) {
    (void)hipGetLastError();
    return false;
  }
  return at.type == hipMemoryTypeHost;
}

static int map_reads_host_pipelined(gmx_engine *e, const uint8_t *reads, const uint64_t *offsets, const uint32_t *seeds,
                                    uint64_t n_reads, uint64_t chunk) {
  if (!e->copy_stream) HIP_TRY(hipStreamCreateWithFlags(&e->copy_stream, hipStreamNonBlocking));
  const uint64_t first = offsets[0], total = offsets[n_reads] - first;
  const bool registered = !gmx_is_pinned(reads + first) &&
                          hipHostRegister(const_cast<uint8_t *>(reads + first), total, hipHostRegisterDefault) == hipSuccess;
  (void)hipGetLastError();
  int rc = GMX_OK;
  auto hip_ok = [&](hipError_t err, const char *what) {
    if (err == hipSuccess) return true;
    gmx_set_error(std::string(what) + ": " + hipGetErrorString(err));
    rc = GMX_EHIP;
    return false;
  };
  uint64_t done = 0;
  try {
  for (uint32_t i = 0; done < n_reads && rc == GMX_OK; ++i) {
    gmx_engine::StageSlot &sl = e->stage[i & 1];
    const uint64_t n = std::min<uint64_t>(chunk, n_reads - done);
    const uint64_t b0 = offsets[done], bases = offsets[done + n] - b0;
    if (sl.busy) {
      if (!hip_ok(gmx_event_wait(sl.done), "hipEventSynchronize")) break;
      sl.busy = false;
    }
    if (!sl.copied) {
      if (!hip_ok(hipEventCreateWithFlags(&sl.copied, hipEventDisableTiming | hipEventBlockingSync), "hipEventCreate") ||
          !hip_ok(hipEventCreateWithFlags(&sl.done, hipEventDisableTiming | hipEventBlockingSync), "hipEventCreate"))
        break;
    }
    if (bases > sl.cap_bases) {
      const uint64_t cb = std::max<uint64_t>(bases + bases / 8, 1 << 16);
      e->release(sl.d_reads);
      sl.d_reads = nullptr;
      sl.cap_bases = 0;
      if ((rc = e->alloc(&sl.d_reads, cb + 16, false))) break;
      sl.cap_bases = cb;
    }
    if (n > sl.cap_reads) {
      const uint64_t cr = std::max<uint64_t>(n, 1024);
      e->release(sl.d_offsets);
      e->release(sl.d_seeds);
      sl.d_offsets = nullptr;
      sl.d_seeds = nullptr;
      sl.cap_reads = 0;
      if ((rc = e->alloc(&sl.d_offsets, cr + 1, false)) || (rc = e->alloc(&sl.d_seeds, cr, false))) break;
      if (sl.h_offsets) (void)hipHostFree(sl.h_offsets);
      if (sl.h_seeds) (void)hipHostFree(sl.h_seeds);
      sl.h_offsets = nullptr;
      sl.h_seeds = nullptr;
      if (!hip_ok(hipHostMalloc(reinterpret_cast<void **>(&sl.h_offsets), (cr + 1) * sizeof(uint64_t), hipHostMallocDefault), "hipHostMalloc") ||
          !hip_ok(hipHostMalloc(reinterpret_cast<void **>(&sl.h_seeds), cr * sizeof(uint32_t), hipHostMallocDefault), "hipHostMalloc"))
        break;
      sl.cap_reads = cr;
    }
    for (uint64_t j = 0; j <= n; ++j) sl.h_offsets[j] = offsets[done + j] - b0;
    memcpy(sl.h_seeds, seeds + done, n * sizeof(uint32_t));
    if (!hip_ok(hipMemcpyAsync(sl.d_reads, reads + b0, bases, hipMemcpyHostToDevice, e->copy_stream), "hipMemcpyAsync(reads)") ||
        !hip_ok(hipMemcpyAsync(sl.d_offsets, sl.h_offsets, (n + 1) * sizeof(uint64_t), hipMemcpyHostToDevice, e->copy_stream), "hipMemcpyAsync(offsets)") ||
        !hip_ok(hipMemcpyAsync(sl.d_seeds, sl.h_seeds, n * sizeof(uint32_t), hipMemcpyHostToDevice, e->copy_stream), "hipMemcpyAsync(seeds)") ||
        !hip_ok(hipEventRecord(sl.copied, e->copy_stream), "hipEventRecord") ||
        !hip_ok(hipStreamWaitEvent(nullptr, sl.copied, 0), "hipStreamWaitEvent"))
      break;
    {
      BatchInput in;
      in.d_reads = sl.d_reads;
      in.d_offsets = sl.d_offsets;
      in.d_seeds = sl.d_seeds;
      in.n_reads = n;
      in.total_bases = bases;
      rc = launch_batch(e, in, nullptr);
    }
    if (rc) break;
    if (!hip_ok(hipEventRecord(sl.done, nullptr), "hipEventRecord")) break;
    sl.busy = true;
    done += n;
  }
  } catch (...) {
    rc = gmx_guard_catch("gmx_map_reads_host");
  }
  (void)hipStreamSynchronize(e->copy_stream);
  (void)hipDeviceSynchronize();
  e->stage[0].busy = e->stage[1].busy = false;
  if (registered) (void)hipHostUnregister(const_cast<uint8_t *>(reads + first));
  (void)hipGetLastError();
  return rc ? rc : gmx_engine_sync(e);
}

static uint64_t gmx_feed_chunk(const gmx_engine *e);
int gmx_map_reads_host(gmx_engine *e, const uint8_t *reads, const uint64_t *offsets, const uint32_t *seeds,
                       uint64_t n_reads) try {
  if (!e) {
    gmx_set_error("null engine");
    return GMX_EINVAL;
  }
  if (n_reads == 0) return GMX_OK;
  HIP_TRY(hipSetDevice(e->opts.device));
  {
    const uint64_t chunk = gmx_feed_chunk(e);
    if (n_reads > chunk && !getenv("GMX_HOST_SERIAL")) return map_reads_host_pipelined(e, reads, offsets, seeds, n_reads, chunk);
  }
  uint64_t done = 0;
  while (done < n_reads) {
    uint64_t n = std::min<uint64_t>(e->opts.max_batch_reads, n_reads - done);
    uint64_t b0 = offsets[done], b1 = offsets[done + n];
    uint64_t bases = b1 - b0;
    if (bases > e->cap_bases) {
      uint64_t cb = std::max<uint64_t>(bases, 1 << 16);
      int rc = e->alloc(&e->d_reads, cb + 16, false);
      if (rc) return rc;
      e->cap_bases = cb;
    }
    if (n > e->cap_stage_reads) {
      uint64_t cr = std::max<uint64_t>(n, 1024);
      int rc = e->alloc(&e->d_offsets, cr + 1, false);
      if (rc) return rc;
      rc = e->alloc(&e->d_seeds, cr, false);
      if (rc) return rc;
      e->cap_stage_reads = cr;
    }
    std::vector<uint64_t> rel(n + 1);
    for (uint64_t i = 0; i <= n; ++i) rel[i] = offsets[done + i] - b0;
    HIP_TRY(hipMemcpy(e->d_reads, reads + b0, bases, hipMemcpyHostToDevice));
    HIP_TRY(hipMemcpy(e->d_offsets, rel.data(), (n + 1) * sizeof(uint64_t), hipMemcpyHostToDevice));
    HIP_TRY(hipMemcpy(e->d_seeds, seeds + done, n * sizeof(uint32_t), hipMemcpyHostToDevice));
    BatchInput in;
    in.d_reads = e->d_reads;
    in.d_offsets = e->d_offsets;
    in.d_seeds = e->d_seeds;
    in.n_reads = n;
    in.total_bases = bases;
    int rc = launch_batch(e, in, nullptr);
    if (rc) return rc;
    HIP_TRY(hipStreamSynchronize(nullptr));
    if (e->log_sites && (rc = log_settle(e))) return rc;
    done += n;
  }
  return gmx_engine_sync(e);
} GMX_GUARD_INT("gmx_map_reads_host")

struct BatchTarget {
  gmx_engine *eng;
  hipStream_t stream;
};
static int pick_target(gmx_engine *e, BatchTarget *out) {
  out->eng = e;
  out->stream = nullptr;
  e->last_on_twin = false;
  gmx_engine *tw = e->twin;
  if (!tw || e->twin_off || e->keep_states) return GMX_OK;
  if (e->reset_pending) {
    e->twin_toggle = 1;
    return GMX_OK;
  }
  if ((e->twin_toggle++ & 1u) == 0) return GMX_OK;
  if (tw->seen_zero_epoch != e->zero_epoch) {
    HIP_TRY(hipStreamWaitEvent(tw->main_stream, e->ev_zeroed, 0));
    tw->seen_zero_epoch = e->zero_epoch;
  }
  tw->timing = e->timing;
  out->eng = tw;
  out->stream = tw->main_stream;
  e->twin_in_flight = true;
  e->last_on_twin = true;
  return GMX_OK;
}

static int map_reads_packed_impl(gmx_engine *e, const uint64_t *planes, bool twobit, const uint64_t *offsets, uint32_t uniform_len,
                                 const uint32_t *seeds, const uint8_t *skip, uint64_t n_reads) {
  if (!e || !planes || !seeds || (!offsets && !uniform_len)) {
    gmx_set_error("gmx_map_reads_packed_host / gmx_map_reads_2bit_host: null argument (offsets may be null only with uniform_len)");
    return GMX_EINVAL;
  }
  if (n_reads == 0) return GMX_OK;
  HIP_TRY(hipSetDevice(e->opts.device));
  if (!e->copy_stream) HIP_TRY(hipStreamCreateWithFlags(&e->copy_stream, hipStreamNonBlocking));
  static const bool two_copy_streams = getenv("GMX_TWO_COPY_STREAMS") != nullptr;
  if (two_copy_streams && !e->copy_stream2) HIP_TRY(hipStreamCreateWithFlags(&e->copy_stream2, hipStreamNonBlocking));
  const uint32_t ppr = (uniform_len + 31u) / 32u;
  auto base_at = [&](uint64_t r) -> uint64_t { return uniform_len ? r * uniform_len : offsets[r] - offsets[0]; };
  auto pair_at = [&](uint64_t r) -> uint64_t {
    if (twobit) return (base_at(r) + 31) >> 5;
    return uniform_len ? r * ppr : ((offsets[r] >> 5) - (offsets[0] >> 5)) + r;
  };
  struct Reg { const void *p; bool on; };
  Reg regs[4] = {{planes, false}, {offsets, false}, {seeds, false}, {skip, false}};
  const uint64_t reg_bytes[4] = {pair_at(n_reads) * 8, (n_reads + 1) * 8, n_reads * 4, n_reads};
  bool all_pinned = true;
  for (int i = 0; i < 4; ++i) {
    if (!regs[i].p || gmx_is_pinned(regs[i].p)) continue;
    regs[i].on = hipHostRegister(const_cast<void *>(regs[i].p), reg_bytes[i], hipHostRegisterDefault) == hipSuccess;
    (void)hipGetLastError();
    all_pinned = false;
  }
  const uint32_t *d_seeds_host = nullptr;
  if (e->seeds_in_place && gmx_is_pinned(seeds)) {
    void *dp = nullptr;
    if (hipHostGetDevicePointer(&dp, const_cast<uint32_t *>(seeds), 0) == hipSuccess && dp) d_seeds_host = static_cast<const uint32_t *>(dp);
    else (void)hipGetLastError();
  }
  const uint64_t chunk = gmx_feed_chunk(e);
  int rc = GMX_OK;
  auto hip_ok = [&](hipError_t err, const char *what) {
    if (err == hipSuccess) return true;
    gmx_set_error(std::string(what) + ": " + hipGetErrorString(err));
    rc = GMX_EHIP;
    return false;
  };
  try {
  for (uint64_t done = 0; done < n_reads && rc == GMX_OK;) {
    gmx_engine::PackSlot &sl = e->pslot[e->pslot_next];
    e->pslot_next = (e->pslot_next + 1) % 3;
    const uint64_t n = std::min<uint64_t>(chunk, n_reads - done);
    uint64_t p0 = pair_at(done), pairs = pair_at(done + n) - p0;
    uint32_t twobit_base0 = 0;
    if (twobit) {
      const uint64_t b0 = base_at(done), b1 = base_at(done + n);
      p0 = b0 >> 5;
      pairs = ((b1 + 31) >> 5) - p0;
      twobit_base0 = (uint32_t)(b0 & 31u);
    }
    if (sl.busy) {
      if (!hip_ok(gmx_event_wait(sl.done), "hipEventSynchronize")) break;
      sl.busy = false;
    }
    if (!sl.copied) {
      if (!hip_ok(hipEventCreateWithFlags(&sl.copied, hipEventDisableTiming | hipEventBlockingSync), "hipEventCreate") ||
          !hip_ok(hipEventCreateWithFlags(&sl.done, hipEventDisableTiming | hipEventBlockingSync), "hipEventCreate"))
        break;
    }
    if (pairs + 16 > sl.cap_pairs) {
      const uint64_t cp = pairs + pairs / 8 + 64;
      e->release(sl.d_planes);
      sl.d_planes = nullptr;
      sl.cap_pairs = 0;
      if ((rc = e->alloc(&sl.d_planes, cp, false))) break;
      sl.cap_pairs = cp;
    }
    if (n > sl.cap_reads) {
      const uint64_t cr = std::max<uint64_t>(n, 1024);
      e->release(sl.d_offsets);
      e->release(sl.d_seeds);
      e->release(sl.d_skip);
      sl.d_offsets = nullptr;
      sl.d_seeds = nullptr;
      sl.d_skip = nullptr;
      sl.cap_reads = 0;
      if ((rc = e->alloc(&sl.d_offsets, cr + 1, false)) || (rc = e->alloc(&sl.d_seeds, cr, false)) || (rc = e->alloc(&sl.d_skip, cr, false))) break;
      sl.cap_reads = cr;
    }
    const hipStream_t cs = two_copy_streams && ((e->copy_toggle++) & 1u) ? e->copy_stream2 : e->copy_stream;
    if (!hip_ok(hipMemcpyAsync(sl.d_planes, planes + p0, pairs * 8, hipMemcpyHostToDevice, cs), "hipMemcpyAsync(planes)")) break;
    if (!uniform_len &&
        !hip_ok(hipMemcpyAsync(sl.d_offsets, offsets + done, (n + 1) * 8, hipMemcpyHostToDevice, cs), "hipMemcpyAsync(offsets)"))
      break;
    if (!d_seeds_host &&
        !hip_ok(hipMemcpyAsync(sl.d_seeds, seeds + done, n * 4, hipMemcpyHostToDevice, cs), "hipMemcpyAsync(seeds)"))
      break;
    if (skip && !hip_ok(hipMemcpyAsync(sl.d_skip, skip + done, n, hipMemcpyHostToDevice, cs), "hipMemcpyAsync(skip)")) break;
    BatchTarget tg;
    if ((rc = pick_target(e, &tg))) break;
    if (!hip_ok(hipEventRecord(sl.copied, cs), "hipEventRecord") ||
        !hip_ok(hipStreamWaitEvent(tg.stream, sl.copied, 0), "hipStreamWaitEvent"))
      break;
    BatchInput in;
    in.d_offsets = uniform_len ? nullptr : sl.d_offsets;
    in.d_seeds = d_seeds_host ? d_seeds_host + done : sl.d_seeds;
    in.d_planes = twobit ? nullptr : sl.d_planes;
    in.d_twobit = twobit ? reinterpret_cast<const uint32_t *>(sl.d_planes) : nullptr;
    in.twobit_base0 = twobit_base0;
    in.d_skip = skip ? sl.d_skip : nullptr;
    in.uniform_len = uniform_len;
    in.n_reads = n;
    in.total_bases = uniform_len ? n * (uint64_t)uniform_len : offsets[done + n] - offsets[done];
    if ((rc = launch_batch(tg.eng, in, tg.stream))) break;
    if (!hip_ok(hipEventRecord(sl.done, tg.stream), "hipEventRecord")) break;
    sl.busy = true;
    done += n;
  }
  } catch (...) {
    rc = gmx_guard_catch(twobit ? "gmx_map_reads_2bit_host" : "gmx_map_reads_packed_host");
  }
  if (rc != GMX_OK || !all_pinned) {
    (void)hipStreamSynchronize(e->copy_stream);
    if (e->copy_stream2) (void)hipStreamSynchronize(e->copy_stream2);
    if (rc != GMX_OK) {
      (void)hipDeviceSynchronize();
      for (auto &sl : e->pslot) sl.busy = false;
    }
  }
  for (int i = 0; i < 4; ++i)
    if (regs[i].on) (void)hipHostUnregister(const_cast<void *>(regs[i].p));
  (void)hipGetLastError();
  return rc;
}

int gmx_map_reads_packed_host(gmx_engine *e, const uint64_t *planes, const uint64_t *offsets, uint32_t uniform_len,
                              const uint32_t *seeds, const uint8_t *skip, uint64_t n_reads) try {
  return map_reads_packed_impl(e, planes, false, offsets, uniform_len, seeds, skip, n_reads);
} GMX_GUARD_INT("gmx_map_reads_packed_host")

static uint64_t gmx_feed_chunk(const gmx_engine *e) {
  static const char *env = getenv("GMX_FEED_CHUNK");
  if (env) return std::max<uint64_t>(1, std::min<uint64_t>(e->opts.max_batch_reads, strtoull(env, nullptr, 10)));
  return e->opts.max_batch_reads;
}

int gmx_map_reads_packed_device(gmx_engine *e, const uint64_t *d_planes, const uint64_t *d_offsets, uint32_t uniform_len,
                                const uint32_t *seeds, const uint8_t *d_skip, uint64_t n_reads) try {
  if (!e || !d_planes || !seeds || (!d_offsets && !uniform_len)) {
    gmx_set_error("gmx_map_reads_packed_device: null argument (d_offsets may be null only with uniform_len)");
    return GMX_EINVAL;
  }
  if (n_reads == 0) return GMX_OK;
  HIP_TRY(hipSetDevice(e->opts.device));
  const uint32_t *d_seeds = seeds;
  if (gmx_is_pinned(seeds)) {
    void *dp = nullptr;
    if (hipHostGetDevicePointer(&dp, const_cast<uint32_t *>(seeds), 0) != hipSuccess || !dp) {
      (void)hipGetLastError();
      gmx_set_error("gmx_map_reads_packed_device: the page-locked seeds have no device address");
      return GMX_EHIP;
    }
    d_seeds = static_cast<const uint32_t *>(dp);
  }
  const uint64_t chunk = gmx_feed_chunk(e);
  if (!uniform_len && n_reads > chunk) {
    gmx_set_error("gmx_map_reads_packed_device: with d_offsets a call takes at most 2^20 reads (and at most max_batch_reads)");
    return GMX_EINVAL;
  }
  const uint64_t ppr = (uniform_len + 31u) / 32u;
  for (uint64_t done = 0; done < n_reads;) {
    const uint64_t n = std::min<uint64_t>(chunk, n_reads - done);
    BatchInput in;
    in.d_planes = reinterpret_cast<const uint2 *>(d_planes + done * ppr);
    in.d_offsets = uniform_len ? nullptr : d_offsets;
    in.d_seeds = d_seeds + done;
    in.d_skip = d_skip ? d_skip + done : nullptr;
    in.uniform_len = uniform_len;
    in.n_reads = n;
    in.total_bases = uniform_len ? n * (uint64_t)uniform_len : 0;
    BatchTarget tg;
    int rc = pick_target(e, &tg);
    if (rc) return rc;
    if ((rc = launch_batch(tg.eng, in, tg.stream))) return rc;
    done += n;
  }
  return GMX_OK;
} GMX_GUARD_INT("gmx_map_reads_packed_device")

int gmx_map_reads_2bit_host(gmx_engine *e, const uint64_t *stream, const uint64_t *offsets, uint32_t uniform_len, const uint32_t *seeds,
                            const uint8_t *skip, uint64_t n_reads) try {
  return map_reads_packed_impl(e, stream, true, offsets, uniform_len, seeds, skip, n_reads);
} GMX_GUARD_INT("gmx_map_reads_2bit_host")

void *gmx_engine_second_stream(gmx_engine *e) { return e && e->twin ? (void *)e->twin->main_stream : nullptr; }

int gmx_engine_seeds_in_place(gmx_engine *e, int on) try {
  if (!e) {
    gmx_set_error("null engine");
    return GMX_EINVAL;
  }
  e->seeds_in_place = on != 0;
  return GMX_OK;
} GMX_GUARD_INT("gmx_engine_seeds_in_place")

int gmx_engine_sync_uploads(gmx_engine *e) try {
  if (!e) {
    gmx_set_error("null engine");
    return GMX_EINVAL;
  }
  HIP_TRY(hipSetDevice(e->opts.device));
  if (e->copy_stream) {
    if (!e->ev_wait) HIP_TRY(hipEventCreateWithFlags(&e->ev_wait, hipEventDisableTiming | hipEventBlockingSync));
    HIP_TRY(hipEventRecord(e->ev_wait, e->copy_stream));
    HIP_TRY(gmx_event_wait(e->ev_wait));
  }
  if (e->copy_stream2) {
    if (!e->ev_wait) HIP_TRY(hipEventCreateWithFlags(&e->ev_wait, hipEventDisableTiming | hipEventBlockingSync));
    HIP_TRY(hipEventRecord(e->ev_wait, e->copy_stream2));
    HIP_TRY(gmx_event_wait(e->ev_wait));
  }
  return GMX_OK;
} GMX_GUARD_INT("gmx_engine_sync_uploads")

static std::mutex g_host_mu;
struct HostBlock {
  uint64_t bytes;
  bool pinned;
};
static std::map<void *, HostBlock> g_host_live;
static std::vector<std::pair<void *, uint64_t>> g_host_spare;
void *gmx_host_alloc(uint64_t bytes) try {
  bytes = std::max<uint64_t>(bytes, 1);
  {
    std::lock_guard<std::mutex> lk(g_host_mu);
    size_t best = g_host_spare.size();
    for (size_t i = 0; i < g_host_spare.size(); ++i)
      if (g_host_spare[i].second >= bytes && g_host_spare[i].second <= 2 * bytes + (1u << 20) &&
          (best == g_host_spare.size() || g_host_spare[i].second < g_host_spare[best].second))
        best = i;
    if (best != g_host_spare.size()) {
      void *p = g_host_spare[best].first;
      g_host_live[p] = HostBlock{g_host_spare[best].second, true};
      g_host_spare.erase(g_host_spare.begin() + (long)best);
      return p;
    }
  }
  void *p = nullptr;
  static const unsigned alloc_flags = getenv("GMX_HOST_ALLOC_FLAGS") ? (unsigned)strtoul(getenv("GMX_HOST_ALLOC_FLAGS"), nullptr, 0) : hipHostMallocDefault;
  bool pinned = hipHostMalloc(&p, bytes, alloc_flags) == hipSuccess && p;
  if (!pinned) {
    (void)hipGetLastError();
    p = malloc(bytes);
  }
  if (p) {
    std::lock_guard<std::mutex> lk(g_host_mu);
    g_host_live[p] = HostBlock{bytes, pinned};
  }
  return p;
} GMX_GUARD_PTR("gmx_host_alloc")
void gmx_host_free(void *p) try {
  if (!p) return;
  HostBlock blk{0, false};
  {
    std::lock_guard<std::mutex> lk(g_host_mu);
    auto it = g_host_live.find(p);
    if (it == g_host_live.end()) return;
    blk = it->second;
    g_host_live.erase(it);
    if (blk.pinned && blk.bytes >= (1u << 20) && g_host_spare.size() < 16) {
      g_host_spare.emplace_back(p, blk.bytes);
      return;
    }
  }
  if (blk.pinned)
    (void)hipHostFree(p);
  else
    free(p);
} GMX_GUARD_VOID("gmx_host_free")

int gmx_engine_reserve(gmx_engine *e, uint64_t n_reads, uint64_t n_bases) try {
  if (!e) {
    gmx_set_error("null engine");
    return GMX_EINVAL;
  }
  HIP_TRY(hipSetDevice(e->opts.device));
  n_reads = std::min<uint64_t>(n_reads, e->opts.max_batch_reads);
  int rc = ensure_batch_capacity(e, n_reads);
  if (rc) return rc;
  const uint64_t need = n_bases / 32 + n_reads + 16;
  if (need > e->cap_packed) {
    if ((rc = e->alloc(&e->d_packed, need, false))) return rc;
    e->cap_packed = need;
  }
  if (n_bases > e->cap_bases) {
    if ((rc = e->alloc(&e->d_reads, n_bases + 16, false))) return rc;
    e->cap_bases = n_bases;
  }
  if (n_reads > e->cap_stage_reads) {
    if ((rc = e->alloc(&e->d_offsets, n_reads + 1, false)) || (rc = e->alloc(&e->d_seeds, n_reads, false))) return rc;
    e->cap_stage_reads = n_reads;
  }
  return GMX_OK;
} GMX_GUARD_INT("gmx_engine_reserve")

int gmx_engine_reserve_packed(gmx_engine *e, uint64_t n_reads, uint64_t n_pairs) try {
  if (!e) {
    gmx_set_error("null engine");
    return GMX_EINVAL;
  }
  HIP_TRY(hipSetDevice(e->opts.device));
  n_reads = std::min<uint64_t>(n_reads, gmx_feed_chunk(e));
  int rc = ensure_batch_capacity(e, n_reads);
  if (rc) return rc;
  if (e->twin && (rc = ensure_batch_capacity(e->twin, n_reads))) return rc;
  if (!e->copy_stream) HIP_TRY(hipStreamCreateWithFlags(&e->copy_stream, hipStreamNonBlocking));
  for (auto &sl : e->pslot) {
    if (sl.busy) continue;
    if (!sl.copied) {
      HIP_TRY(hipEventCreateWithFlags(&sl.copied, hipEventDisableTiming | hipEventBlockingSync));
      HIP_TRY(hipEventCreateWithFlags(&sl.done, hipEventDisableTiming | hipEventBlockingSync));
    }
    if (n_pairs + 16 > sl.cap_pairs) {
      e->release(sl.d_planes);
      sl.d_planes = nullptr;
      sl.cap_pairs = 0;
      if ((rc = e->alloc(&sl.d_planes, n_pairs + 64, false))) return rc;
      sl.cap_pairs = n_pairs + 64;
    }
    if (n_reads > sl.cap_reads) {
      e->release(sl.d_offsets);
      e->release(sl.d_seeds);
      e->release(sl.d_skip);
      sl.d_offsets = nullptr;
      sl.d_seeds = nullptr;
      sl.d_skip = nullptr;
      sl.cap_reads = 0;
      if ((rc = e->alloc(&sl.d_offsets, n_reads + 1, false)) || (rc = e->alloc(&sl.d_seeds, n_reads, false)) ||
          (rc = e->alloc(&sl.d_skip, n_reads, false)))
        return rc;
      sl.cap_reads = n_reads;
    }
  }
  return GMX_OK;
} GMX_GUARD_INT("gmx_engine_reserve_packed")

int gmx_engine_sync(gmx_engine *e) try {
  HIP_TRY(hipSetDevice(e->opts.device));
  {
    int frc = flush_reset(e);
    if (frc) return frc;
    if ((frc = log_settle(e))) return frc;
  }
  {
    int qrc = gmx_quiesce(e);
    if (qrc) return qrc;
    if (e->twin && (qrc = gmx_quiesce(e->twin))) return qrc;
    e->twin_in_flight = false;
  }
  HIP_TRY(hipStreamSynchronize(e->last_stream));
  HIP_TRY(hipDeviceSynchronize());
  uint32_t c[4] = {0, 0, 0, 0};
  HIP_TRY(hipMemcpy(c + 2, e->d_error, 8, hipMemcpyDeviceToHost));
  if (c[2] == 0 && e->twin) {
    HIP_TRY(hipMemcpy(c + 2, e->twin->d_error, 8, hipMemcpyDeviceToHost));
    if (c[2] != 0) HIP_TRY(hipMemset(e->twin->d_error, 0, 8));
  }
  if (c[2] != 0) {
    HIP_TRY(hipMemset(e->d_error, 0, 8));
    char msg[256];
    if (c[2] == GMX_TASK_LOGFULL) {
      snprintf(msg, sizeof(msg),
               "a read's records exceed the whole grouped-allele-count log (sites without dense group counters; %u words): "
               "nothing of it was recorded: raise gmx_engine_opts.log_cap_words",
               e->log_cap);
      gmx_set_error(msg);
      return GMX_ECAP;
    }
    if (c[2] == GMX_TASK_OVERFLOW) {
      snprintf(msg, sizeof(msg),
               "read %u (orientation %u) needs more memory for its search states or its mapping instances than the whole "
               "last-tier heap holds (%llu bytes); nothing of this read was recorded: raise gmx_engine_opts.huge_heap_bytes "
               "(GMX_HUGE_HEAP_BYTES)",
               c[3] >> 1, c[3] & 1, (unsigned long long)e->heap_words * 4);
      gmx_set_error(msg);
      return GMX_ECAP;
    }
    snprintf(msg, sizeof(msg),
             "read %u (orientation %u): inconsistent variant path (the reference throws/asserts here: a site "
             "traversed twice or an exit that does not match the entered site)",
             c[3] >> 1, c[3] & 1);
    gmx_set_error(msg);
    return GMX_EREF;
  }
  return GMX_OK;
} GMX_GUARD_INT("gmx_engine_sync")

int gmx_engine_enable_timing(gmx_engine *e, int on) try {
  e->timing = on != 0;
  if (e->twin) e->twin->timing = e->timing;
  return GMX_OK;
} GMX_GUARD_INT("gmx_engine_enable_timing")

int gmx_engine_timing(gmx_engine *e, gmx_timing *out) try {
  HIP_TRY(hipSetDevice(e->opts.device));
  if (e->twin) {
    e->pending.insert(e->pending.end(), e->twin->pending.begin(), e->twin->pending.end());
    e->twin->pending.clear();
  }
  for (auto &ev : e->pending) {
    HIP_TRY(hipEventSynchronize(ev.c));
    float ms0 = 0, ms1 = 0, ms2 = 0;
    HIP_TRY(hipEventElapsedTime(&ms0, ev.s, ev.a));
    HIP_TRY(hipEventElapsedTime(&ms1, ev.a, ev.b));
    HIP_TRY(hipEventElapsedTime(&ms2, ev.b, ev.c));
    e->search_ms += ms1;
    e->cover_ms += ms0 + ms2;
    e->search_launches++;
    e->cover_launches++;
    e->timed_reads += ev.reads;
    for (int k = 0; k < GMX_TK_N; ++k) {
      if (ev.timed & (1u << k)) {
        float ms = 0;
        HIP_TRY(hipEventSynchronize(ev.k[k][1]));
        HIP_TRY(hipEventElapsedTime(&ms, ev.k[k][0], ev.k[k][1]));
        e->kernel_ms[k] += ms;
        e->kernel_launches[k]++;
      }
      (void)hipEventDestroy(ev.k[k][0]);
      (void)hipEventDestroy(ev.k[k][1]);
    }
    (void)hipEventDestroy(ev.s);
    (void)hipEventDestroy(ev.a);
    (void)hipEventDestroy(ev.b);
    (void)hipEventDestroy(ev.c);
  }
  e->pending.clear();
  out->search_ms = e->search_ms;
  out->search_launches = e->search_launches;
  out->cover_ms = e->cover_ms;
  out->cover_launches = e->cover_launches;
  out->reads = e->timed_reads;
  for (int k = 0; k < GMX_TIMED_KERNELS; ++k) {
    out->kernel_ms[k] = e->kernel_ms[k];
    out->kernel_launches[k] = e->kernel_launches[k];
    e->kernel_ms[k] = 0;
    e->kernel_launches[k] = 0;
  }
  e->search_ms = e->cover_ms = 0;
  e->search_launches = e->cover_launches = e->timed_reads = 0;
  return GMX_OK;
} GMX_GUARD_INT("gmx_engine_timing")

int gmx_engine_queue_counts(gmx_engine *e, gmx_queue_counts *out) try {
  HIP_TRY(hipSetDevice(e->opts.device));
  HIP_TRY(hipDeviceSynchronize());
  uint32_t raw[GMX_N_COUNTERS * GMX_CNT_STRIDE];
  HIP_TRY(hipMemcpy(raw, (e->twin && e->last_on_twin ? e->twin : e)->d_counters, sizeof(raw), hipMemcpyDeviceToHost));
  auto c = [&](int i) { return (uint64_t)raw[i * GMX_CNT_STRIDE]; };
  out->mapped = 0;
  for (int r = 0; r < GMX_REGIONS; ++r) out->mapped += c(16 + r);
  out->mapped += c(8);
  out->alive = c(5);
  out->dead = c(6) + c(12);
  out->overflow_probe = c(1);
  out->overflow_extend = c(9);
  out->big_mapped = c(7);
  out->cover_general = c(8);
  out->cover_mid = c(13);
  out->cover_overflow = c(4);
  out->seed_cursor = e->seed_cursor ? 1 : 0;
  out->inst_mapped = c(25);
  out->huge_search = c(11);
  out->huge_cover = c(15);
  out->log_replays = e->log_replays;
  out->log_replayed_entries = e->log_replayed_entries;
  out->overflow_split = c(29);
  return GMX_OK;
} GMX_GUARD_INT("gmx_engine_queue_counts")

int gmx_coverage_device(gmx_engine *e, gmx_device_coverage *out) try {
  {
    int frc = flush_reset(e);
    if (frc) return frc;
  }
  if (e->twin && e->twin_in_flight) {
    int qrc = gmx_quiesce(e->twin);
    if (qrc) return qrc;
    e->twin_in_flight = false;
  }
  out->allele_sum = out->per_base = out->grouped = nullptr;
  out->n_allele_sum = e->n_allele;
  out->n_per_base = e->n_pb;
  out->n_grouped = e->n_grouped;
  out->stats = e->d_stats;
  out->n_stats = 5;
  out->fused = e->d_fused;
  out->n_fused = e->n_fused;
  return GMX_OK;
} GMX_GUARD_INT("gmx_coverage_device")

int gmx_coverage_reduce_begin(gmx_engine *e, void *hip_stream) try {
  if (!e) {
    gmx_set_error("null engine");
    return GMX_EINVAL;
  }
  {
    int frc = flush_reset(e);
    if (frc) return frc;
    if ((frc = log_settle(e))) return frc;
  }
  HIP_TRY(hipSetDevice(e->opts.device));
  {
    int trc = twin_join(e, (hipStream_t)hip_stream);
    if (trc) return trc;
  }
  e->recorded = true;
  hipLaunchKernelGGL(gmx_stats_limbs_kernel, dim3(1), dim3(64), 0, (hipStream_t)hip_stream, e->d_stats, e->d_limbs, 0);
  HIP_TRY(hipGetLastError());
  return GMX_OK;
} GMX_GUARD_INT("gmx_coverage_reduce_begin")

int gmx_coverage_reduce_end(gmx_engine *e, void *hip_stream) try {
  if (!e) {
    gmx_set_error("null engine");
    return GMX_EINVAL;
  }
  {
    int frc = flush_reset(e);
    if (frc) return frc;
  }
  HIP_TRY(hipSetDevice(e->opts.device));
  hipLaunchKernelGGL(gmx_stats_limbs_kernel, dim3(1), dim3(64), 0, (hipStream_t)hip_stream, e->d_stats, e->d_limbs, 1);
  HIP_TRY(hipGetLastError());
  return GMX_OK;
} GMX_GUARD_INT("gmx_coverage_reduce_end")

static void gather_block(const gmx_engine *e, const uint32_t *block, uint32_t *allele_sum, uint32_t *per_base, uint32_t *grouped) {
  if (allele_sum) for (size_t i = 0; i < e->phys_allele.size(); ++i) allele_sum[i] += block[e->phys_allele[i]];
  if (per_base) for (size_t i = 0; i < e->phys_pb.size(); ++i) per_base[i] += block[e->phys_pb[i]];
  if (grouped) for (size_t i = 0; i < e->phys_grouped.size(); ++i) grouped[i] += block[e->phys_grouped[i]];
  for (size_t i = 0; i + 3 < e->hit_fix.size(); i += 4) {
    const uint32_t hits = block[e->hit_fix[i]];
    if (allele_sum) allele_sum[e->hit_fix[i + 1]] += hits;
    if (grouped) grouped[e->hit_fix[i + 2]] += hits;
    if (per_base) per_base[e->hit_fix[i + 3]] += hits;
  }
}
static int fetch_blocks(gmx_engine *e, size_t first, size_t count, uint32_t *allele_sum, uint32_t *per_base, uint32_t *grouped) {
  {
    int frc = flush_reset(e);
    if (frc) return frc;
    if ((frc = log_settle(e))) return frc;
  }
  HIP_TRY(hipSetDevice(e->opts.device));
  HIP_TRY(hipDeviceSynchronize());
  if (!allele_sum && !per_base && !grouped) return GMX_OK;
  std::vector<uint32_t> block(std::max<size_t>(e->n_acc * count, 1));
  if (e->n_acc) HIP_TRY(hipMemcpy(block.data(), e->d_fused + first * e->n_acc, e->n_acc * count * 4, hipMemcpyDeviceToHost));
  if (allele_sum) std::fill(allele_sum, allele_sum + e->phys_allele.size(), 0u);
  if (per_base) std::fill(per_base, per_base + e->phys_pb.size(), 0u);
  if (grouped) std::fill(grouped, grouped + e->phys_grouped.size(), 0u);
  for (size_t k = 0; k < count; ++k) gather_block(e, block.data() + k * e->n_acc, allele_sum, per_base, grouped);
  return GMX_OK;
}

int gmx_coverage_fetch(gmx_engine *e, uint32_t *allele_sum, uint32_t *per_base, uint32_t *grouped, gmx_stats *stats) try {
  if (!e) {
    gmx_set_error("null engine");
    return GMX_EINVAL;
  }
  {
    int rc = fetch_blocks(e, 0, e->record_strands ? 2 : 1, allele_sum, per_base, grouped);
    if (rc) return rc;
  }
  if (stats) {
    unsigned long long s[5];
    HIP_TRY(hipMemcpy(s, e->d_stats, sizeof(s), hipMemcpyDeviceToHost));
    stats->all_reads_count = s[0];
    stats->skipped_reads_count = s[1];
    stats->missing_kmer_reads_count = s[2];
    stats->no_extension_reads_count = s[3];
    stats->exact_mapped_reads_count = s[4];
  }
  return GMX_OK;
} GMX_GUARD_INT("gmx_coverage_fetch")

int gmx_coverage_fetch_strand(gmx_engine *e, int strand, uint32_t *allele_sum, uint32_t *per_base, uint32_t *grouped_dense) try {
  if (!e) {
    gmx_set_error("null engine");
    return GMX_EINVAL;
  }
  if (!e->record_strands) {
    gmx_set_error("gmx_coverage_fetch_strand: the engine does not record per strand (gmx_engine_record_strands)");
    return GMX_EINVAL;
  }
  if (strand != 0 && strand != 1) {
    gmx_set_error("gmx_coverage_fetch_strand: strand is 0 (forward) or 1 (reverse complement)");
    return GMX_EINVAL;
  }
  return fetch_blocks(e, (size_t)strand, 1, allele_sum, per_base, grouped_dense);
} GMX_GUARD_INT("gmx_coverage_fetch_strand")

static int set_record_strands(gmx_engine *e, bool on) {
  if (e->record_strands == on) return GMX_OK;
  const size_t n_fused = (on ? 2 : 1) * e->n_acc + 32;
  if (n_fused + 32 > 0xFFFFFFFFull) {
    gmx_set_error("gmx_engine_record_strands: two accumulator blocks of this index exceed 2^32 words");
    return GMX_EINVAL;
  }
  uint32_t *old = e->d_fused, *q = nullptr;
  int rc = e->alloc(&q, n_fused + 32, true);
  if (rc) return rc;
  e->release(old);
  e->record_strands = on;
  e->reset_pending = false;
  for (gmx_engine *w : {e, e->twin}) {
    if (!w) continue;
    w->d_fused = q;
    w->n_fused = n_fused;
    w->d_limbs = q + n_fused - 32;
    w->d_stats = reinterpret_cast<unsigned long long *>(q + n_fused);
    w->d_log_cursor = q + n_fused + 16;
  }
  return GMX_OK;
}

int gmx_engine_record_strands(gmx_engine *e, int on) try {
  if (!e) {
    gmx_set_error("null engine");
    return GMX_EINVAL;
  }
  if (e->recorded) {
    gmx_set_error("gmx_engine_record_strands: coverage has been recorded since the last reset (call gmx_engine_reset first)");
    return GMX_EINVAL;
  }
  HIP_TRY(hipSetDevice(e->opts.device));
  HIP_TRY(hipDeviceSynchronize());
  return set_record_strands(e, on != 0);
} GMX_GUARD_INT("gmx_engine_record_strands")

int gmx_engine_set_max_candidates(gmx_engine *e, uint32_t limit) try {
  if (!e) {
    gmx_set_error("null engine");
    return GMX_EINVAL;
  }
  if (e->recorded) {
    gmx_set_error("gmx_engine_set_max_candidates: coverage has been recorded since the last reset (call gmx_engine_reset first)");
    return GMX_EINVAL;
  }
  e->max_candidates = limit;
  return GMX_OK;
} GMX_GUARD_INT("gmx_engine_set_max_candidates")

uint32_t gmx_engine_max_candidates(gmx_engine *e) try {
  return e ? e->max_candidates : 0u;
} GMX_GUARD_ZERO("gmx_engine_max_candidates")

static int read_log_record(gmx_engine *e, GmxReadLog gmx_engine::*log, int on) {
  if (!e) {
    gmx_set_error("null engine");
    return GMX_EINVAL;
  }
  (e->*log).on = on != 0;
  return GMX_OK;
}

static int64_t read_log_count(gmx_engine *e, GmxReadLog gmx_engine::*log) {
  if (!e) {
    gmx_set_error("null engine");
    return GMX_EINVAL;
  }
  return (int64_t)(e->*log).count;
}

static int read_log_fetch(gmx_engine *e, GmxReadLog gmx_engine::*which, uint64_t first, uint64_t n, void *out, const char *name) {
  if (!e || (n && !out)) {
    gmx_set_error(std::string(name) + ": null argument");
    return GMX_EINVAL;
  }
  const GmxReadLog &log = e->*which;
  if (first > log.count || n > log.count - first) {
    gmx_set_error(std::string(name) + ": reads " + std::to_string(first) + " .. " + std::to_string(first + n) + " of " +
                  std::to_string(log.count) + " recorded");
    return GMX_EINVAL;
  }
  {
    int frc = flush_reset(e);
    if (frc) return frc;
    if ((frc = log_settle(e))) return frc;
  }
  HIP_TRY(hipSetDevice(e->opts.device));
  HIP_TRY(hipDeviceSynchronize());
  if (n) HIP_TRY(hipMemcpy(out, reinterpret_cast<const uint8_t *>(log.d) + first * log.stride, n * log.stride, hipMemcpyDeviceToHost));
  return GMX_OK;
}

int gmx_engine_record_outcomes(gmx_engine *e, int on) try {
  return read_log_record(e, &gmx_engine::outcomes, on);
} GMX_GUARD_INT("gmx_engine_record_outcomes")

int64_t gmx_engine_outcome_count(gmx_engine *e) try {
  return read_log_count(e, &gmx_engine::outcomes);
} GMX_GUARD_INT("gmx_engine_outcome_count")

int gmx_engine_fetch_outcomes(gmx_engine *e, uint64_t first, uint64_t n, uint8_t *out) try {
  return read_log_fetch(e, &gmx_engine::outcomes, first, n, out, "gmx_engine_fetch_outcomes");
} GMX_GUARD_INT("gmx_engine_fetch_outcomes")

enum LogForm { LOG_FORWARD = 0, LOG_REVERSE_ONLY = 1, LOG_TOTALS = 2, LOG_EXCHANGE = 3 };
static LogForm exchange_form(const gmx_engine *e) { return e->record_strands ? LOG_EXCHANGE : LOG_TOTALS; }
static uint64_t emit_log_counts(const gmx_engine *e, LogForm which, uint32_t *out, uint64_t cap_words) {
  uint64_t n = 0;
  for (auto const &kv : e->log_counts) {
    const uint64_t words = 4 + (kv.first.size() - 1);
    for (int s = 0; s < (which == LOG_EXCHANGE ? 2 : 1); ++s) {
      const uint64_t count = which == LOG_TOTALS ? kv.second[0] + kv.second[1] : kv.second[which == LOG_EXCHANGE ? s : which];
      if (!count) continue;
      if (out && n + words <= cap_words) {
        out[n] = kv.first[0];
        out[n + 1] = (uint32_t)(kv.first.size() - 1) | GMX_LOG_COUNTED | (which == LOG_EXCHANGE && s ? GMX_LOG_REVERSE : 0u);
        out[n + 2] = (uint32_t)count;
        out[n + 3] = (uint32_t)(count >> 32);
        for (size_t j = 1; j < kv.first.size(); ++j) out[n + 3 + j] = kv.first[j];
      }
      n += words;
    }
  }
  return n;
}

int gmx_engine_record_positions(gmx_engine *e, int on) try {
  return read_log_record(e, &gmx_engine::positions, on);
} GMX_GUARD_INT("gmx_engine_record_positions")

int64_t gmx_engine_position_count(gmx_engine *e) try {
  return read_log_count(e, &gmx_engine::positions);
} GMX_GUARD_INT("gmx_engine_position_count")

int gmx_engine_fetch_positions(gmx_engine *e, uint64_t first, uint64_t n, uint32_t *out) try {
  return read_log_fetch(e, &gmx_engine::positions, first, n, out, "gmx_engine_fetch_positions");
} GMX_GUARD_INT("gmx_engine_fetch_positions")

int64_t gmx_coverage_fetch_grouped_log(gmx_engine *e, uint32_t *out, uint64_t cap_words) try {
  if (!e) return GMX_EINVAL;
  if (hipSetDevice(e->opts.device) != hipSuccess) return GMX_EHIP;
  if (log_settle(e)) return GMX_EHIP;
  if (gmx_log_drain(e, 0)) return GMX_EHIP;
  return (int64_t)emit_log_counts(e, LOG_TOTALS, out, cap_words);
} GMX_GUARD_INT("gmx_coverage_fetch_grouped_log")

int64_t gmx_coverage_fetch_grouped_log_strand(gmx_engine *e, int strand, uint32_t *out, uint64_t cap_words) try {
  if (!e) {
    gmx_set_error("null engine");
    return GMX_EINVAL;
  }
  if (!e->record_strands) {
    gmx_set_error("gmx_coverage_fetch_grouped_log_strand: the engine does not record per strand (gmx_engine_record_strands)");
    return GMX_EINVAL;
  }
  if (strand != 0 && strand != 1) {
    gmx_set_error("gmx_coverage_fetch_grouped_log_strand: strand is 0 (forward) or 1 (reverse complement)");
    return GMX_EINVAL;
  }
  if (hipSetDevice(e->opts.device) != hipSuccess) return GMX_EHIP;
  if (log_settle(e)) return GMX_EHIP;
  if (gmx_log_drain(e, 0)) return GMX_EHIP;
  return (int64_t)emit_log_counts(e, strand ? LOG_REVERSE_ONLY : LOG_FORWARD, out, cap_words);
} GMX_GUARD_INT("gmx_coverage_fetch_grouped_log_strand")

int64_t gmx_coverage_export_grouped_log(gmx_engine *e, uint32_t *out, uint64_t cap_words) try {
  if (!e) {
    gmx_set_error("null engine");
    return GMX_EINVAL;
  }
  if (hipSetDevice(e->opts.device) != hipSuccess) return GMX_EHIP;
  if (log_settle(e)) return GMX_EHIP;
  if (gmx_log_drain(e, 0)) return GMX_EHIP;
  return (int64_t)emit_log_counts(e, exchange_form(e), out, cap_words);
} GMX_GUARD_INT("gmx_coverage_export_grouped_log")

int gmx_coverage_import_grouped_log(gmx_engine *e, const uint32_t *records, uint64_t n_words, int replace) try {
  if (!e || (!records && n_words)) {
    gmx_set_error("gmx_coverage_import_grouped_log: null argument");
    return GMX_EINVAL;
  }
  {
    int frc = flush_reset(e);
    if (frc) return frc;
  }
  HIP_TRY(hipSetDevice(e->opts.device));
  return gmx_engine_log_import(e, records, (size_t)n_words, replace != 0);
} GMX_GUARD_INT("gmx_coverage_import_grouped_log")

}

uint64_t gmx_engine_reset_epoch(const gmx_engine *e) { return e->reset_epoch; }

void gmx_engine_raw(gmx_engine *e, GmxEngineRaw *out) {
  (void)flush_reset(e);
  out->device = e->opts.device;
  out->d_fused = e->d_fused;
  out->n_fused = e->n_fused;
  out->log_sites = e->log_sites;
  out->record_strands = e->record_strands;
}

int gmx_engine_log_export(gmx_engine *e, std::vector<uint32_t> &out) {
  {
    int frc = flush_reset(e);
    if (frc) return frc;
    if ((frc = log_settle(e))) return frc;
  }
  HIP_TRY(hipSetDevice(e->opts.device));
  {
    int rc = gmx_log_drain(e, 0);
    if (rc) return rc;
  }
  const LogForm which = exchange_form(e);
  out.assign((size_t)emit_log_counts(e, which, nullptr, 0), 0);
  emit_log_counts(e, which, out.data(), out.size());
  return GMX_OK;
}

int gmx_engine_log_import(gmx_engine *e, const uint32_t *w, size_t n_words, bool replace) {
  {
    int frc = flush_reset(e);
    if (frc) return frc;
  }
  const uint32_t flags = GMX_LOG_COUNTED | GMX_LOG_REVERSE;
  for (size_t i = 0; i < n_words;) {
    if (w[i] == GMX_LOG_PAD) {
      ++i;
      continue;
    }
    if (i + 2 > n_words) break;
    const uint32_t n = w[i + 1] & ~flags;
    const size_t head = (w[i + 1] & GMX_LOG_COUNTED) ? 4 : 2;
    if (i + head + n > n_words) {
      gmx_set_error("corrupt grouped log");
      return GMX_EINVAL;
    }
    if ((w[i + 1] & GMX_LOG_REVERSE) && !e->record_strands) {
      gmx_set_error("grouped log: a reverse-complement record (GMX_LOG_REVERSE) for an engine that does not record per strand");
      return GMX_EINVAL;
    }
    i += head + n;
  }
  if (replace) {
    int rc = gmx_log_drain(e, 0);
    if (rc) return rc;
    e->log_counts.clear();
  }
  std::vector<uint32_t> key;
  for (size_t i = 0; i < n_words;) {
    if (w[i] == GMX_LOG_PAD) {
      ++i;
      continue;
    }
    if (i + 2 > n_words) break;
    const uint32_t n = w[i + 1] & ~flags;
    const size_t head = (w[i + 1] & GMX_LOG_COUNTED) ? 4 : 2;
    const uint64_t count = head == 4 ? ((uint64_t)w[i + 2] | ((uint64_t)w[i + 3] << 32)) : 1;
    key.assign(1, w[i]);
    key.insert(key.end(), w + i + head, w + i + head + n);
    e->log_counts[key][(w[i + 1] & GMX_LOG_REVERSE) ? 1 : 0] += count;
    i += head + n;
  }
  return GMX_OK;
}

#include "gmx_engine_debug.h"
```

gramtools_amd/csrc/gmx_index.h:

```cpp
#pragma once
#include <sys/mman.h>

#include <algorithm>
#include <chrono>
#include <cstdint>
#include <cstdlib>
#include <new>
#include <string>
#include <utility>
#include <vector>

#include "gmx_types.h"

namespace gmx {

inline bool gmx_huge_pages_pay() {
  static const bool ok = [] {
    if (const char *e = getenv("GMX_HUGEPAGES")) return atoi(e) != 0;
    const size_t bytes = (size_t)16 << 20, huge = (size_t)2 << 20;
    auto touch = [&](bool advise) -> double {
      void *p = aligned_alloc(huge, bytes);
      if (!p) return 1e9;
      if (advise && madvise(p, bytes, MADV_HUGEPAGE) != 0) {
        free(p);
// ... 1 lines not shown
      }
      const auto t0 = std::chrono::steady_clock::now();
      for (size_t i = 0; i < bytes; i += 4096) static_cast<volatile char *>(p)[i] = 1;
      const double dt = std::chrono::duration<double>(std::chrono::steady_clock::now() - t0).count();
      free(p);
      return dt;
    };
    const double plain = touch(false), advised = touch(true);
    return advised < plain;
  }();
  return ok;
}

template <class T>
struct BigAlloc {
  typedef T value_type;
  BigAlloc() = default;
  template <class U>
  BigAlloc(const BigAlloc<U> &) {}
  T *allocate(size_t n) {
    size_t bytes = n ? n * sizeof(T) : 1;
    void *p;
    const size_t huge = (size_t)2 << 20;
    if (bytes >= ((size_t)64 << 20) && gmx_huge_pages_pay()) {
      bytes = (bytes + huge - 1) / huge * huge;
      p = aligned_alloc(huge, bytes);
      if (p) madvise(p, bytes, MADV_HUGEPAGE);
    } else {
      p = malloc(bytes);
    }
    if (!p) throw std::bad_alloc();
    return static_cast<T *>(p);
  }
  void deallocate(T *p, size_t) { free(p); }
  template <class U>
  void construct(U *p) { ::new ((void *)p) U; }
  template <class U, class A0, class... A>
  void construct(U *p, A0 &&a0, A &&...a) { ::new ((void *)p) U(std::forward<A0>(a0), std::forward<A>(a)...); }
  bool operator==(const BigAlloc &) const { return true; }
  bool operator!=(const BigAlloc &) const { return false; }
};
typedef std::vector<GmxSeed, BigAlloc<GmxSeed>> SeedTable;

class WordBuf {
 public:
  WordBuf() = default;
  WordBuf(const WordBuf &) = delete;
  WordBuf &operator=(const WordBuf &) = delete;
  WordBuf(WordBuf &&o) noexcept : p_(o.p_), n_(o.n_), cap_(o.cap_) { o.p_ = nullptr, o.n_ = o.cap_ = 0; }
  WordBuf &operator=(WordBuf &&o) noexcept {
    if (this != &o) {
      release();
      p_ = o.p_, n_ = o.n_, cap_ = o.cap_;
      o.p_ = nullptr, o.n_ = o.cap_ = 0;
    }
    return *this;
  }
  ~WordBuf() { release(); }
  uint32_t *data() { return p_; }
  const uint32_t *data() const { return p_; }
  size_t size() const { return n_; }
  bool empty() const { return n_ == 0; }
  uint32_t &operator[](size_t i) { return p_[i]; }
  const uint32_t &operator[](size_t i) const { return p_[i]; }
  void reserve(size_t words) {
    if (words <= cap_) return;
    const size_t page = (size_t)2 << 20;
    const size_t bytes = (words * sizeof(uint32_t) + page - 1) / page * page;
    void *q = p_ ? mremap(p_, cap_ * sizeof(uint32_t), bytes, MREMAP_MAYMOVE)
                 : mmap(nullptr, bytes, PROT_READ | PROT_WRITE, MAP_PRIVATE | MAP_ANONYMOUS | MAP_NORESERVE, -1, 0);
    if (q == MAP_FAILED) throw std::bad_alloc();
    if (bytes >= ((size_t)64 << 20) && gmx_huge_pages_pay()) madvise(q, bytes, MADV_HUGEPAGE);
    p_ = static_cast<uint32_t *>(q);
    cap_ = bytes / sizeof(uint32_t);
  }
  void resize(size_t words) {
    if (words > cap_) reserve(std::max(words, cap_ + cap_ / 4));
    n_ = words;
  }
  void clear() { n_ = 0; }
  void release() {
    if (p_) munmap(p_, cap_ * sizeof(uint32_t));
    p_ = nullptr;
    n_ = cap_ = 0;
  }
  uint32_t *grow(size_t words) {
    const size_t at = n_;
    resize(n_ + words);
    return p_ + at;
  }

 private:
  uint32_t *p_ = nullptr;
  size_t n_ = 0, cap_ = 0;
};

struct TargetedMarker {
  uint32_t id;
  int32_t deletion_allele;
};

struct HostIndex {
  std::vector<uint32_t> prg;
  uint32_t kmer_size = 0;
  uint32_t sentinel_pos = 0;
  uint32_t C[8] = {0};
  bool is_nested = false;

  std::vector<GmxRankBlock> blocks;
  std::vector<uint32_t> sa;
  std::vector<GmxHit> hits;
  std::vector<uint32_t> hit_perm, hit_prog;
  std::vector<GmxTextRec> text;
  std::vector<uint32_t> prog;
  std::vector<uint32_t> pos_node;
  std::vector<GmxNode> nodes;
  std::vector<uint32_t> edges;
  std::vector<GmxSite> sites;
  std::vector<GmxSiteGeo> site_geo;
  SeedTable seeds;
  uint32_t kmer_size2 = 0;
  SeedTable seeds2;
  WordBuf seed_words;
  uint32_t seed_shift = 0;
  std::vector<uint32_t> kmer_bitmap;
  uint32_t n_allele_slots = 0, n_pb_slots = 0, n_grouped_slots = 0;
  uint32_t n_acc_slots = 0;
  std::vector<uint32_t> l_allele_off, l_grouped_off;
  std::vector<uint32_t> l_cov_off;
  std::vector<uint32_t> phys_allele, phys_pb, phys_grouped;
  std::vector<uint32_t> hit_fix;
  std::vector<uint32_t> site_ref_pos;

  std::vector<uint32_t> bwt;
  std::vector<std::pair<uint32_t, std::vector<TargetedMarker>>> target_map;
  std::vector<std::pair<uint32_t, int32_t>> pos_target;
  uint64_t n_seed_kmers_present = 0;
  uint64_t n_seed_states = 0, n_seed_states_large = 0;

  GmxIndexView view() const;
};

void build_suffix_array(const std::vector<uint32_t> &text, std::vector<uint32_t> &sa, int threads = 1);
void debug_suffix_array_u16(const uint16_t *text, size_t n, uint16_t *sa);

void build_index(const std::vector<uint32_t> &prg, uint32_t kmer_size, HostIndex &out, int threads = 0, int seed_k2 = -1);
void build_index(std::vector<uint32_t> &&prg, uint32_t kmer_size, HostIndex &out, int threads = 0, int seed_k2 = -1);

void save_index(const HostIndex &h, const std::string &path);
void load_index(const std::string &path, const std::vector<uint32_t> &prg, uint32_t kmer_size, HostIndex &out);

std::vector<uint32_t> read_prg_file(const std::string &path);

struct WalkState {
  uint32_t lo, hi, tvd, tvg;
};
struct WalkNode {
  std::vector<WalkState> list;
  std::vector<GmxPathNode> arena;
};
struct SeedEntryRef {
  uint32_t code, table;
  uint64_t off;
};
struct SeedPart {
  std::vector<uint32_t> words;
  uint64_t word_base = 0, n_words = 0;
  std::vector<SeedEntryRef> complex;
  uint64_t n_present[2] = {0, 0}, n_states_all[2] = {0, 0}, n_states_large[2] = {0, 0};
};
typedef bool (*DeviceSeedWalk)(const HostIndex &ix, uint32_t k, uint32_t k2, uint32_t depth0, std::vector<WalkNode> &roots,
                               GmxSeed *table, GmxSeed *table2, uint32_t *bitmap, std::vector<SeedPart> &parts, WordBuf &words);
extern DeviceSeedWalk g_device_seed_walk;

typedef bool (*DeviceSuffixPresort)(const uint32_t *text, size_t n, uint32_t *sa, std::vector<uint32_t> &tie_mask);
extern DeviceSuffixPresort g_device_suffix_presort;

std::vector<int64_t> seed_states_of(const HostIndex &ix, uint32_t kmer_code, bool longer_table = false);

}
```

Measured before the change: 1.453 billion.

## Gather coverage on device and skip idle syncs in engine sync

Coverage fetch now runs a device gather kernel over precomputed source and hit tables. It copies back only the compact per-slot sums plus a tail of stats, error and log-cursor words through a pinned buffer and an event wait, instead of a full device sync, a full accumulator memcpy and a host-side gather. A busy/shared flag lets gmx_engine_sync return early when nothing ran since the last fetch, and grouped-log fetches skip draining when log sites are disabled. In exchange, busy-state tracking has to be maintained at every entry point, and a host fallback remains for large tables or when GMX_FETCH_HOST is set.

Measured after the change: 1.452 billion. No clear change (-0.1%).

```diff
diff --git a/gramtools_amd/csrc/gmx_capi.cpp b/gramtools_amd/csrc/gmx_capi.cpp
--- a/gramtools_amd/csrc/gmx_capi.cpp
+++ b/gramtools_amd/csrc/gmx_capi.cpp
@@ -426,6 +426,25 @@
   }
 } GMX_GUARD_INT("gmx_debug_suffix_array_u16")
 
+extern "C" int64_t gmx_debug_fetch_tables(const uint32_t *phys_allele, uint64_t n_allele, const uint32_t *phys_pb, uint64_t n_pb,
+                                          const uint32_t *phys_grouped, uint64_t n_grouped, const uint32_t *hit_fix, uint64_t n_hit_words,
+                                          uint64_t n_acc, uint32_t *src, uint32_t *hit) try {
+  std::vector<uint32_t> s, h;
+  if (!gmx::build_fetch_tables(phys_allele, n_allele, phys_pb, n_pb, phys_grouped, n_grouped, hit_fix, n_hit_words, n_acc,
+                               src ? &s : nullptr, hit ? &h : nullptr))
+    return -1;
+  if (src && !s.empty()) memcpy(src, s.data(), s.size() * 4);
+  if (hit && !h.empty()) memcpy(hit, h.data(), h.size() * 4);
+  return (int64_t)(n_allele + n_pb + n_grouped);
+} GMX_GUARD_INT("gmx_debug_fetch_tables")
+
+extern "C" int64_t gmx_debug_index_fetch_tables(const gmx_index *ix, uint32_t *src, uint32_t *hit) try {
+  if (!ix) return GMX_EINVAL;
+  const gmx::HostIndex &h = ix->h;
+  return gmx_debug_fetch_tables(h.phys_allele.data(), h.phys_allele.size(), h.phys_pb.data(), h.phys_pb.size(), h.phys_grouped.data(),
+                                h.phys_grouped.size(), h.hit_fix.data(), h.hit_fix.size(), ((uint64_t)h.n_acc_slots + 63) / 64 * 64, src, hit);
+} GMX_GUARD_INT("gmx_debug_index_fetch_tables")
+
 int gmx_index_copy_sa(const gmx_index *ix, uint32_t *out) try {
   memcpy(out, ix->h.sa.data(), ix->h.sa.size() * 4);
   return GMX_OK;
diff --git a/gramtools_amd/csrc/gmx_engine_cover_kernels.h b/gramtools_amd/csrc/gmx_engine_cover_kernels.h
--- a/gramtools_amd/csrc/gmx_engine_cover_kernels.h
+++ b/gramtools_amd/csrc/gmx_engine_cover_kernels.h
@@ -1001,3 +1001,34 @@
   if (rem) out[full] = pack_tail(p + full * 32, rem, bad);
   skip[read] = bad ? 1 : 0;
 }
+
+#define GMX_FETCH_TAIL 16
+struct FetchTailSrc {
+  const uint32_t *stats;
+  const uint32_t *log_cursor;
+  const uint32_t *error;
+  const uint32_t *twin_error;
+};
+__global__ void __launch_bounds__(256) gmx_cover_gather_kernel(const uint32_t *__restrict__ block, size_t stride, uint32_t count,
+                                                               const uint32_t *__restrict__ src, const uint32_t *__restrict__ hit,
+                                                               uint32_t begin, uint32_t end, uint32_t *__restrict__ out, FetchTailSrc tail) {
+  for (uint32_t i = begin + blockIdx.x * blockDim.x + threadIdx.x; i < end; i += gridDim.x * blockDim.x) {
+    const uint32_t s = src[i], h = hit[i];
+    uint32_t v = 0;
+    for (uint32_t k = 0; k < count; ++k) {
+      const uint32_t *b = block + (size_t)k * stride;
+      v += b[s];
+      if (h != gmx::GMX_FETCH_NO_HIT) v += b[h];
+    }
+    out[i] = v;
+  }
+  if (blockIdx.x == 0 && threadIdx.x < GMX_FETCH_TAIL) {
+    const uint32_t t = threadIdx.x;
+    uint32_t v = 0;
+    if (t < 10) v = tail.stats[t];
+    else if (t == 10) v = tail.log_cursor[0];
+    else if (t < 13) v = tail.error[t - 11];
+    else if (t < 15 && tail.twin_error) v = tail.twin_error[t - 13];
+    out[end + t] = v;
+  }
+}
diff --git a/gramtools_amd/csrc/gmx_engine_debug.h b/gramtools_amd/csrc/gmx_engine_debug.h
--- a/gramtools_amd/csrc/gmx_engine_debug.h
+++ b/gramtools_amd/csrc/gmx_engine_debug.h
@@ -193,6 +193,7 @@
     gmx_set_error("gmx_debug_final_states: null argument");
     return GMX_EINVAL;
   }
+  gmx_busy(e);
   if (!e->keep_states || task >= 2 * e->keep_reads) {
     gmx_set_error("gmx_debug_final_states: no such task in the last batch (gmx_engine_debug_keep_states first)");
     return GMX_EINVAL;
@@ -297,6 +298,7 @@
     gmx_set_error("gmx_debug_search: bad argument");
     return GMX_EINVAL;
   }
+  gmx_busy(e);
   for (uint32_t i = 0; i < read_len; ++i)
     if (read[i] < 1 || read[i] > 4) {
       gmx_set_error("gmx_debug_search: the read must hold bases 1..4");
@@ -376,6 +378,7 @@
     gmx_set_error("gmx_debug_encapsulate: bad argument");
     return GMX_EINVAL;
   }
+  gmx_busy(e);
   HIP_TRY(hipSetDevice(e->opts.device));
   HIP_TRY(hipDeviceSynchronize());
   std::vector<GmxFinalState> st;
diff --git a/gramtools_amd/csrc/gmx_engine_host.h b/gramtools_amd/csrc/gmx_engine_host.h
--- a/gramtools_amd/csrc/gmx_engine_host.h
+++ b/gramtools_amd/csrc/gmx_engine_host.h
@@ -66,6 +66,13 @@
   bool recorded = false;
   std::vector<uint32_t> phys_allele, phys_pb, phys_grouped;
   std::vector<uint32_t> hit_fix;
+  int fetch_state = 0;
+  uint32_t *d_fetch_src = nullptr, *d_fetch_hit = nullptr, *d_fetch_out = nullptr;
+  uint32_t *h_fetch = nullptr;
+  size_t h_fetch_words = 0;
+  hipEvent_t ev_fetch = nullptr;
+  bool busy = true, shared = false, stream_changed = false;
+  uint32_t idle_tail[16] = {0};
   unsigned long long *d_stats = nullptr;
   uint32_t *d_error = nullptr;
   uint32_t *d_log = nullptr, *d_log_cursor = nullptr;
@@ -247,6 +254,14 @@
   }
 }
 
+static inline void gmx_busy(gmx_engine *e) {
+  if (e) (e->owner ? e->owner : e)->busy = true;
+}
+static inline bool fetch_host_forced() {
+  const char *v = getenv("GMX_FETCH_HOST");
+  return v && atoi(v) != 0;
+}
+
 static int gmx_quiesce(gmx_engine *e) {
   if (!e->ev_wait) HIP_TRY(hipEventCreateWithFlags(&e->ev_wait, hipEventDisableTiming | hipEventBlockingSync));
   hipStream_t streams[5] = {e->last_stream, e->copy_stream, e->side_stream, e->side2_stream, e->copy_stream2};
@@ -279,6 +294,7 @@
 static int flush_reset(gmx_engine *e) {
   if (!e->reset_pending) return GMX_OK;
   e->reset_pending = false;
+  gmx_busy(e);
   HIP_TRY(hipMemsetAsync(e->d_fused, 0, (e->n_fused + 32) * 4, e->reset_stream));
   return note_zeroed(e, e->reset_stream);
 }
@@ -287,6 +303,7 @@
 static int gmx_log_drain(gmx_engine *e, uint64_t keep_below) {
   int frc = flush_reset(e);
   if (frc) return frc;
+  gmx_busy(e);
   HIP_TRY(hipDeviceSynchronize());
   uint32_t used = 0;
   HIP_TRY(hipMemcpy(&used, e->d_log_cursor, 4, hipMemcpyDeviceToHost));
@@ -353,6 +370,7 @@
 } GMX_GUARD_VOID("gmx_engine_default_opts")
 
 static int ensure_batch_capacity(gmx_engine *e, uint64_t n_reads, bool launching = false) {
+  gmx_busy(e);
   if (launching) {
     gmx_engine *own = e->owner ? e->owner : e;
     for (GmxReadLog *log : {&own->outcomes, &own->positions})
@@ -759,6 +777,10 @@
   if (e->copy_stream2) (void)hipStreamDestroy(e->copy_stream2);
   if (e->h_log_state) (void)hipHostFree(e->h_log_state);
   if (e->ev_log_state) (void)hipEventDestroy(e->ev_log_state);
+  if (e->h_fetch) (void)hipHostFree(e->h_fetch);
+  if (e->ev_fetch) (void)hipEventDestroy(e->ev_fetch);
+  for (uint32_t *q : {e->d_fetch_src, e->d_fetch_hit, e->d_fetch_out})
+    if (q) (void)hipFree(q);
   for (auto &sl : e->pslot) {
     if (sl.copied) (void)hipEventDestroy(sl.copied);
     if (sl.done) (void)hipEventDestroy(sl.done);
@@ -779,6 +801,7 @@
 int gmx_engine_reset(gmx_engine *e) try {
   HIP_TRY(hipSetDevice(e->opts.device));
   e->reset_pending = false;
+  gmx_busy(e);
   HIP_TRY(hipDeviceSynchronize());
   HIP_TRY(hipMemset(e->d_fused, 0, (e->n_fused + 32) * 4));
   HIP_TRY(hipMemset(e->d_error, 0, 8));
@@ -801,6 +824,7 @@
 int gmx_engine_reset_async(gmx_engine *e, void *hip_stream) try {
   HIP_TRY(hipSetDevice(e->opts.device));
   hipStream_t st = (hipStream_t)hip_stream;
+  gmx_busy(e);
   int frc = flush_reset(e);
   if (frc) return frc;
   if ((frc = twin_join(e, st))) return frc;
@@ -833,6 +857,7 @@
 }
 
 static int log_state_enqueue(gmx_engine *e, hipStream_t stream) {
+  gmx_busy(e);
   if (!e->h_log_state) {
     HIP_TRY(hipHostMalloc(reinterpret_cast<void **>(&e->h_log_state), 4 * sizeof(uint32_t), hipHostMallocDefault));
     HIP_TRY(hipEventCreateWithFlags(&e->ev_log_state, hipEventDisableTiming));
@@ -848,6 +873,7 @@
 
 static int launch_log_replay(gmx_engine *e, hipStream_t stream) {
   const int in = e->log_retry_side, out = in ^ 1;
+  gmx_busy(e);
   SearchOut o = e->last_o;
   o.log_retry_list = e->d_log_retry[out];
   o.log_retry_recs = e->d_log_retry_recs[out];
@@ -872,6 +898,7 @@
 
 static int log_settle(gmx_engine *e) {
   if (!e->log_state_pending) return GMX_OK;
+  gmx_busy(e);
   uint64_t before = ~0ull;
   for (int round = 0;; ++round) {
     HIP_TRY(hipEventSynchronize(e->ev_log_state));
@@ -960,6 +987,8 @@
 
 static int launch_batch(gmx_engine *e, const BatchInput &in, hipStream_t stream) {
   const uint64_t n_reads = in.n_reads, total_bases = in.total_bases;
+  gmx_busy(e);
+  if (!e->is_twin && stream != e->last_stream) e->stream_changed = true;
   if (n_reads == 0) return GMX_OK;
   if (n_reads > (0x7fffffffull / GMX_FAST_ARENA) / 2) {
     gmx_set_error("batch too large: at most 44 M reads per launch (lower gmx_engine_opts.max_batch_reads)");
@@ -1238,6 +1267,7 @@
 
 static int map_reads_host_pipelined(gmx_engine *e, const uint8_t *reads, const uint64_t *offsets, const uint32_t *seeds,
                                     uint64_t n_reads, uint64_t chunk) {
+  gmx_busy(e);
   if (!e->copy_stream) HIP_TRY(hipStreamCreateWithFlags(&e->copy_stream, hipStreamNonBlocking));
   const uint64_t first = offsets[0], total = offsets[n_reads] - first;
   const bool registered = !gmx_is_pinned(reads + first) &&
@@ -1331,6 +1361,7 @@
     return GMX_EINVAL;
   }
   if (n_reads == 0) return GMX_OK;
+  gmx_busy(e);
   HIP_TRY(hipSetDevice(e->opts.device));
   {
     const uint64_t chunk = gmx_feed_chunk(e);
@@ -1409,6 +1440,7 @@
     return GMX_EINVAL;
   }
   if (n_reads == 0) return GMX_OK;
+  gmx_busy(e);
   HIP_TRY(hipSetDevice(e->opts.device));
   if (!e->copy_stream) HIP_TRY(hipStreamCreateWithFlags(&e->copy_stream, hipStreamNonBlocking));
   static const bool two_copy_streams = getenv("GMX_TWO_COPY_STREAMS") != nullptr;
@@ -1590,7 +1622,7 @@
   return map_reads_packed_impl(e, stream, true, offsets, uniform_len, seeds, skip, n_reads);
 } GMX_GUARD_INT("gmx_map_reads_2bit_host")
 
-void *gmx_engine_second_stream(gmx_engine *e) { return e && e->twin ? (void *)e->twin->main_stream : nullptr; }
+void *gmx_engine_second_stream(gmx_engine *e) { return e && e->twin ? (e->shared = true, (void *)e->twin->main_stream) : nullptr; }
 
 int gmx_engine_seeds_in_place(gmx_engine *e, int on) try {
   if (!e) {
@@ -1744,6 +1776,10 @@
 
 int gmx_engine_sync(gmx_engine *e) try {
   HIP_TRY(hipSetDevice(e->opts.device));
+  if (!e->busy && !e->shared && !e->reset_pending && !e->log_state_pending && e->idle_tail[11] == 0 && e->idle_tail[13] == 0 &&
+      !fetch_host_forced())
+    return GMX_OK;
+  gmx_busy(e);
   {
     int frc = flush_reset(e);
     if (frc) return frc;
@@ -1877,6 +1913,8 @@
 } GMX_GUARD_INT("gmx_engine_queue_counts")
 
 int gmx_coverage_device(gmx_engine *e, gmx_device_coverage *out) try {
+  e->shared = true;
+  gmx_busy(e);
   {
     int frc = flush_reset(e);
     if (frc) return frc;
@@ -1913,6 +1951,8 @@
     if (trc) return trc;
   }
   e->recorded = true;
+  e->shared = true;
+  gmx_busy(e);
   hipLaunchKernelGGL(gmx_stats_limbs_kernel, dim3(1), dim3(64), 0, (hipStream_t)hip_stream, e->d_stats, e->d_limbs, 0);
   HIP_TRY(hipGetLastError());
   return GMX_OK;
@@ -1928,6 +1968,8 @@
     if (frc) return frc;
   }
   HIP_TRY(hipSetDevice(e->opts.device));
+  e->shared = true;
+  gmx_busy(e);
   hipLaunchKernelGGL(gmx_stats_limbs_kernel, dim3(1), dim3(64), 0, (hipStream_t)hip_stream, e->d_stats, e->d_limbs, 1);
   HIP_TRY(hipGetLastError());
   return GMX_OK;
@@ -1944,22 +1986,120 @@
     if (per_base) per_base[e->hit_fix[i + 3]] += hits;
   }
 }
-static int fetch_blocks(gmx_engine *e, size_t first, size_t count, uint32_t *allele_sum, uint32_t *per_base, uint32_t *grouped) {
+static int fetch_blocks_host(gmx_engine *e, size_t first, size_t count, uint32_t *allele_sum, uint32_t *per_base, uint32_t *grouped,
+                             unsigned long long *stats) {
+  gmx_busy(e);
+  HIP_TRY(hipDeviceSynchronize());
+  if (allele_sum || per_base || grouped) {
+    std::vector<uint32_t> block(std::max<size_t>(e->n_acc * count, 1));
+    if (e->n_acc) HIP_TRY(hipMemcpy(block.data(), e->d_fused + first * e->n_acc, e->n_acc * count * 4, hipMemcpyDeviceToHost));
+    if (allele_sum) std::fill(allele_sum, allele_sum + e->phys_allele.size(), 0u);
+    if (per_base) std::fill(per_base, per_base + e->phys_pb.size(), 0u);
+    if (grouped) std::fill(grouped, grouped + e->phys_grouped.size(), 0u);
+    for (size_t k = 0; k < count; ++k) gather_block(e, block.data() + k * e->n_acc, allele_sum, per_base, grouped);
+  }
+  if (stats) HIP_TRY(hipMemcpy(stats, e->d_stats, 5 * sizeof(unsigned long long), hipMemcpyDeviceToHost));
+  return GMX_OK;
+}
+
+static bool fetch_device_setup(gmx_engine *e) {
+  if (e->fetch_state) return e->fetch_state > 0;
+  std::vector<uint32_t> src, hit;
+  const bool ok = gmx::build_fetch_tables(e->phys_allele.data(), e->phys_allele.size(), e->phys_pb.data(), e->phys_pb.size(),
+                                          e->phys_grouped.data(), e->phys_grouped.size(), e->hit_fix.data(), e->hit_fix.size(),
+                                          e->n_acc, &src, &hit);
+  e->fetch_state = -1;
+  if (!ok) return false;
+  const size_t total = src.size(), bytes = std::max<size_t>(total, 1) * 4;
+  bool good = hipMalloc((void **)&e->d_fetch_src, bytes) == hipSuccess && hipMalloc((void **)&e->d_fetch_hit, bytes) == hipSuccess &&
+              hipMalloc((void **)&e->d_fetch_out, (total + GMX_FETCH_TAIL) * 4) == hipSuccess &&
+              hipEventCreateWithFlags(&e->ev_fetch, hipEventDisableTiming) == hipSuccess;
+  if (good && total)
+    good = hipMemcpy(e->d_fetch_src, src.data(), total * 4, hipMemcpyHostToDevice) == hipSuccess &&
+           hipMemcpy(e->d_fetch_hit, hit.data(), total * 4, hipMemcpyHostToDevice) == hipSuccess;
+  if (!good) {
+    (void)hipGetLastError();
+    if (e->d_fetch_src) (void)hipFree(e->d_fetch_src);
+    if (e->d_fetch_hit) (void)hipFree(e->d_fetch_hit);
+    if (e->d_fetch_out) (void)hipFree(e->d_fetch_out);
+    e->d_fetch_src = e->d_fetch_hit = e->d_fetch_out = nullptr;
+    return false;
+  }
+  e->fetch_state = 1;
+  return true;
+}
+
+static int fetch_blocks_device(gmx_engine *e, size_t first, size_t count, uint32_t *allele_sum, uint32_t *per_base, uint32_t *grouped,
+                               unsigned long long *stats, bool *served) {
+  *served = false;
+  const size_t n_a = e->phys_allele.size(), n_p = e->phys_pb.size(), n_g = e->phys_grouped.size();
+  if (fetch_host_forced() || n_a + n_p + n_g > gmx::GMX_FETCH_MAX_SLOTS || !fetch_device_setup(e)) return GMX_OK;
+  size_t lo = 0, hi = 0;
+  if (allele_sum || per_base || grouped) {
+    lo = allele_sum ? 0 : per_base ? n_a : n_a + n_p;
+    hi = grouped ? n_a + n_p + n_g : per_base ? n_a + n_p : n_a;
+  }
+  const size_t words = hi - lo + GMX_FETCH_TAIL;
+  if (words > e->h_fetch_words) {
+    if (e->h_fetch) (void)hipHostFree(e->h_fetch);
+    e->h_fetch = nullptr;
+    e->h_fetch_words = 0;
+    const size_t grown = std::max<size_t>(words, n_a + n_p + n_g + GMX_FETCH_TAIL);
+    if (hipHostMalloc(reinterpret_cast<void **>(&e->h_fetch), grown * 4, hipHostMallocDefault) != hipSuccess) {
+      (void)hipGetLastError();
+      e->h_fetch = nullptr;
+      e->fetch_state = -1;
+      return GMX_OK;
+    }
+    e->h_fetch_words = grown;
+  }
+  struct Part { uint32_t *dst; size_t at, n; };
+  std::vector<Part> parts;
+  if (lo != hi) parts.reserve(3);
+  if (allele_sum) parts.push_back({allele_sum, 0 - lo, n_a});
+  if (per_base) parts.push_back({per_base, n_a - lo, n_p});
+  if (grouped) parts.push_back({grouped, n_a + n_p - lo, n_g});
+  gmx_busy(e);
+  if (e->shared || e->stream_changed) {
+    HIP_TRY(hipDeviceSynchronize());
+    e->stream_changed = false;
+  }
+  const hipStream_t stream = e->last_stream;
+  {
+    int trc = twin_join(e, stream);
+    if (trc) return trc;
+  }
+  const FetchTailSrc tail{reinterpret_cast<const uint32_t *>(e->d_stats), e->d_log_cursor, e->d_error, e->twin ? e->twin->d_error : nullptr};
+  const unsigned blocks = (unsigned)std::min<size_t>(std::max<size_t>((hi - lo + 255) / 256, 1), (size_t)e->n_cus * 8);
+  hipLaunchKernelGGL(gmx_cover_gather_kernel, dim3(blocks), dim3(256), 0, stream, e->d_fused + first * e->n_acc, e->n_acc, (uint32_t)count,
+                     e->d_fetch_src, e->d_fetch_hit, (uint32_t)lo, (uint32_t)hi, e->d_fetch_out, tail);
+  HIP_TRY(hipGetLastError());
+  HIP_TRY(hipMemcpyAsync(e->h_fetch, e->d_fetch_out + lo, words * 4, hipMemcpyDeviceToHost, stream));
+  HIP_TRY(hipEventRecord(e->ev_fetch, stream));
+  HIP_TRY(gmx_event_wait(e->ev_fetch));
+  *served = true;
+  const uint32_t *h = e->h_fetch;
+  for (const Part &p : parts) memcpy(p.dst, h + p.at, p.n * 4);
+  const uint32_t *t = h + (hi - lo);
+  if (stats) memcpy(stats, t, 5 * sizeof(unsigned long long));
+  memcpy(e->idle_tail, t, sizeof(e->idle_tail));
+  e->twin_in_flight = false;
+  e->busy = false;
+  return GMX_OK;
+}
+
+static int fetch_blocks(gmx_engine *e, size_t first, size_t count, uint32_t *allele_sum, uint32_t *per_base, uint32_t *grouped,
+                        unsigned long long *stats = nullptr) {
   {
     int frc = flush_reset(e);
     if (frc) return frc;
     if ((frc = log_settle(e))) return frc;
   }
   HIP_TRY(hipSetDevice(e->opts.device));
-  HIP_TRY(hipDeviceSynchronize());
-  if (!allele_sum && !per_base && !grouped) return GMX_OK;
-  std::vector<uint32_t> block(std::max<size_t>(e->n_acc * count, 1));
-  if (e->n_acc) HIP_TRY(hipMemcpy(block.data(), e->d_fused + first * e->n_acc, e->n_acc * count * 4, hipMemcpyDeviceToHost));
-  if (allele_sum) std::fill(allele_sum, allele_sum + e->phys_allele.size(), 0u);
-  if (per_base) std::fill(per_base, per_base + e->phys_pb.size(), 0u);
-  if (grouped) std::fill(grouped, grouped + e->phys_grouped.size(), 0u);
-  for (size_t k = 0; k < count; ++k) gather_block(e, block.data() + k * e->n_acc, allele_sum, per_base, grouped);
-  return GMX_OK;
+  bool served = false;
+  int rc = fetch_blocks_device(e, first, count, allele_sum, per_base, grouped, stats, &served);
+  if (rc || served) return rc;
+  return fetch_blocks_host(e, first, count, allele_sum, per_base, grouped, stats);
 }
 
 int gmx_coverage_fetch(gmx_engine *e, uint32_t *allele_sum, uint32_t *per_base, uint32_t *grouped, gmx_stats *stats) try {
@@ -1967,13 +2107,12 @@
     gmx_set_error("null engine");
     return GMX_EINVAL;
   }
+  unsigned long long s[5] = {0, 0, 0, 0, 0};
   {
-    int rc = fetch_blocks(e, 0, e->record_strands ? 2 : 1, allele_sum, per_base, grouped);
+    int rc = fetch_blocks(e, 0, e->record_strands ? 2 : 1, allele_sum, per_base, grouped, stats ? s : nullptr);
     if (rc) return rc;
   }
   if (stats) {
-    unsigned long long s[5];
-    HIP_TRY(hipMemcpy(s, e->d_stats, sizeof(s), hipMemcpyDeviceToHost));
     stats->all_reads_count = s[0];
     stats->skipped_reads_count = s[1];
     stats->missing_kmer_reads_count = s[2];
@@ -1999,7 +2138,12 @@
   return fetch_blocks(e, (size_t)strand, 1, allele_sum, per_base, grouped_dense);
 } GMX_GUARD_INT("gmx_coverage_fetch_strand")
 
+int gmx_debug_fetch_state(gmx_engine *e) try {
+  return e ? e->fetch_state : GMX_EINVAL;
+} GMX_GUARD_INT("gmx_debug_fetch_state")
+
 static int set_record_strands(gmx_engine *e, bool on) {
+  gmx_busy(e);
   if (e->record_strands == on) return GMX_OK;
   const size_t n_fused = (on ? 2 : 1) * e->n_acc + 32;
   if (n_fused + 32 > 0xFFFFFFFFull) {
@@ -2141,6 +2285,7 @@
 
 int64_t gmx_coverage_fetch_grouped_log(gmx_engine *e, uint32_t *out, uint64_t cap_words) try {
   if (!e) return GMX_EINVAL;
+  if (!e->log_sites && !fetch_host_forced()) return (int64_t)emit_log_counts(e, LOG_TOTALS, out, cap_words);
   if (hipSetDevice(e->opts.device) != hipSuccess) return GMX_EHIP;
   if (log_settle(e)) return GMX_EHIP;
   if (gmx_log_drain(e, 0)) return GMX_EHIP;
@@ -2160,6 +2305,7 @@
     gmx_set_error("gmx_coverage_fetch_grouped_log_strand: strand is 0 (forward) or 1 (reverse complement)");
     return GMX_EINVAL;
   }
+  if (!e->log_sites && !fetch_host_forced()) return (int64_t)emit_log_counts(e, strand ? LOG_REVERSE_ONLY : LOG_FORWARD, out, cap_words);
   if (hipSetDevice(e->opts.device) != hipSuccess) return GMX_EHIP;
   if (log_settle(e)) return GMX_EHIP;
   if (gmx_log_drain(e, 0)) return GMX_EHIP;
@@ -2195,6 +2341,8 @@
 uint64_t gmx_engine_reset_epoch(const gmx_engine *e) { return e->reset_epoch; }
 
 void gmx_engine_raw(gmx_engine *e, GmxEngineRaw *out) {
+  e->shared = true;
+  gmx_busy(e);
   (void)flush_reset(e);
   out->device = e->opts.device;
   out->d_fused = e->d_fused;
diff --git a/gramtools_amd/csrc/gmx_index.h b/gramtools_amd/csrc/gmx_index.h
--- a/gramtools_amd/csrc/gmx_index.h
+++ b/gramtools_amd/csrc/gmx_index.h
@@ -177,6 +177,37 @@
 
 std::vector<uint32_t> read_prg_file(const std::string &path);
 
+constexpr uint64_t GMX_FETCH_MAX_SLOTS = 32ull << 20;
+constexpr uint32_t GMX_FETCH_NO_HIT = 0xFFFFFFFFu;
+inline bool build_fetch_tables(const uint32_t *phys_allele, uint64_t n_allele, const uint32_t *phys_pb, uint64_t n_pb,
+                               const uint32_t *phys_grouped, uint64_t n_grouped, const uint32_t *hit_fix, uint64_t n_hit_words,
+                               uint64_t n_acc, std::vector<uint32_t> *src, std::vector<uint32_t> *hit) {
+  if (n_allele > GMX_FETCH_MAX_SLOTS || n_pb > GMX_FETCH_MAX_SLOTS || n_grouped > GMX_FETCH_MAX_SLOTS) return false;
+  const uint64_t total = n_allele + n_pb + n_grouped;
+  if (total > GMX_FETCH_MAX_SLOTS || n_hit_words % 4 != 0 || n_acc >= GMX_FETCH_NO_HIT) return false;
+  std::vector<uint32_t> s(total), h(total, GMX_FETCH_NO_HIT);
+  const uint32_t *phys[3] = {phys_allele, phys_pb, phys_grouped};
+  const uint64_t len[3] = {n_allele, n_pb, n_grouped}, base[3] = {0, n_allele, n_allele + n_pb};
+  for (int a = 0; a < 3; ++a)
+    for (uint64_t i = 0; i < len[a]; ++i) {
+      if (phys[a][i] >= n_acc) return false;
+      s[base[a] + i] = phys[a][i];
+    }
+  for (uint64_t i = 0; i < n_hit_words; i += 4) {
+    if (hit_fix[i] >= n_acc) return false;
+    const uint64_t logical[3] = {hit_fix[i + 1], hit_fix[i + 3], hit_fix[i + 2]};
+    for (int a = 0; a < 3; ++a) {
+      if (logical[a] >= len[a]) return false;
+      uint32_t &slot = h[base[a] + logical[a]];
+      if (slot != GMX_FETCH_NO_HIT) return false;
+      slot = hit_fix[i];
+    }
+  }
+  if (src) src->swap(s);
+  if (hit) hit->swap(h);
+  return true;
+}
+
 struct WalkState {
   uint32_t lo, hi, tvd, tvg;
 };
```
